# lthero-big/A-watermark-for-Diffusion-Models

Measured on AMD Instinct MI355X. Metric: watermarked images/sec (embed+extract, 512x512 SD2.1) + lossless bit-accuracy, higher is better.
Workload: dtype f16; 1 GPU; e2e: gsw_embed -> 50-step DDIM sampling (CFG 7.5, 2B-row UNet) -> 50-step DDIM inversion -> fused last step + 256-bit vote; SD2.1-base-shaped UNet (865.9 M params, synthetic weights; convolutions on the hand-written MFMA implicit GEMM), image stages per image: VAE decode -> uint8 -> ToTensor -> VAE encode (timed; synthetic VAE, inversion consumes the latent); batch_per_gpu=64, global_batch=64, message_bits=256, ddim_steps=50, parallelism=dp1 (images sharded, UNet replicated, no data-path collective)

## Files before the change

a-watermark-for-diffusion-models_amd/_native.py:

```python
from __future__ import annotations

import ctypes as C
import os

_HERE = os.path.dirname(os.path.abspath(__file__))
LIB_PATH = os.environ.get("GSWM_LIB", os.path.join(_HERE, "libgswm.so"))

GSW_F32, GSW_F16, GSW_BF16, GSW_F64 = 0, 1, 2, 3
GSW_OK, GSW_ERR_BAD_ARG, GSW_ERR_UNSUPPORTED, GSW_ERR_RAGGED, GSW_ERR_HIP, GSW_WARN_NO_RECORDS = 0, 1, 2, 3, 4, 5
GSW_EMBED_EXACT_F64, GSW_EMBED_FAST_F32 = 0, 1
GSW_MM_GN_ONLY = 1
GSW_FLAG_SATURATED, GSW_FLAG_NAN = 1, 2
GSW_MSG_INLINE_MAX = 256
GSW_IMG_U8_HWC, GSW_IMG_F16_CHW, GSW_IMG_F32_CHW = 0, 1, 2
GSW_PW_BRIGHTNESS, GSW_PW_CONTRAST, GSW_PW_INVERT, GSW_PW_GRAY, GSW_PW_HFLIP, GSW_PW_VFLIP, GSW_PW_NOISE = range(7)
GSW_RESAMPLE_LANCZOS, GSW_RESAMPLE_BILINEAR = 1, 2
GSW_TRACE_SOFT, GSW_TRACE_HARD = 0, 1

_u8p = C.POINTER(C.c_uint8)


class GswMmExtras(C.Structure):
    _fields_ = [("colstats_dev", C.c_void_p), ("colstats_capacity", C.c_int64), ("rowstats_dev", C.c_void_p), ("rowstats_capacity", C.c_int64),
                ("workspace_dev", C.c_void_p), ("workspace_bytes", C.c_int64), ("max_splits", C.c_int),
                ("colstats_rows_per_block", C.c_int), ("colstats_blocks", C.c_int), ("rowstats_slots", C.c_int), ("splits", C.c_int), ("flags", C.c_int)]


_PROTOTYPES = {
    "gsw_version": (C.c_int, []),
    "gsw_build_flags": (C.c_int, []),
    "gsw_strerror": (C.c_char_p, [C.c_int]),
    "gsw_last_hip_error": (C.c_int, []),
    "gsw_keystream": (C.c_int, [C.c_char_p, C.c_char_p, C.c_void_p, C.c_size_t, C.c_void_p]),
    "gsw_embed": (C.c_int, [C.c_char_p, C.c_char_p, C.c_char_p, C.c_int, C.c_void_p, C.c_uint64, C.c_uint64, C.c_void_p,
                            C.c_int, C.c_int, C.c_int64, C.c_uint32, C.c_void_p]),
    "gsw_philox_uniform": (C.c_int, [C.c_uint64, C.c_uint64, C.c_void_p, C.c_int, C.c_int64, C.c_void_p]),
    "gsw_extract": (C.c_int, [C.c_void_p, C.c_int, C.c_char_p, C.c_char_p, C.c_int, C.c_void_p, C.c_void_p, C.c_void_p,
                              C.c_int, C.c_int64, C.c_void_p]),
    "gsw_bit_matches": (C.c_int, [C.c_void_p, C.c_int, C.c_char_p, C.c_int, C.c_void_p, C.c_int, C.c_void_p]),
    "gsw_ddim_step": (C.c_int, [C.c_void_p, C.c_void_p, C.c_void_p, C.c_float, C.c_float, C.c_int, C.c_int64, C.c_void_p]),
    "gsw_ddim_step_cfg": (C.c_int, [C.c_void_p, C.c_void_p, C.c_void_p, C.c_void_p, C.c_float, C.c_float, C.c_float,
                                    C.c_int, C.c_int64, C.c_void_p]),
    "gsw_dpm_step": (C.c_int, [C.c_void_p, C.c_void_p, C.c_void_p, C.c_void_p, C.c_void_p, C.c_void_p, C.c_float, C.c_float, C.c_float,
                               C.c_float, C.c_float, C.c_float, C.c_int, C.c_int64, C.c_void_p]),
    "gsw_ddim_step_extract": (C.c_int, [C.c_void_p, C.c_void_p, C.c_void_p, C.c_float, C.c_float, C.c_int, C.c_char_p,
                                        C.c_char_p, C.c_int, C.c_void_p, C.c_void_p, C.c_void_p, C.c_int, C.c_int64,
                                        C.c_void_p]),
    "gsw_groupnorm_silu": (C.c_int, [C.c_void_p, C.c_void_p, C.c_void_p, C.c_void_p, C.c_void_p, C.c_int, C.c_int, C.c_int, C.c_int,
                                     C.c_float, C.c_int, C.c_int, C.c_void_p]),
    "gsw_geglu": (C.c_int, [C.c_void_p, C.c_void_p, C.c_int64, C.c_int, C.c_int, C.c_void_p]),
    "gsw_conv_pf": (C.c_int, [C.c_void_p, C.c_void_p, C.c_void_p, C.c_void_p, C.c_int, C.c_void_p, C.c_void_p, C.c_int, C.c_int, C.c_int, C.c_int,
                              C.c_int, C.c_int, C.c_int, C.c_int, C.c_int, C.c_void_p]),
    "gsw_groupnorm_pf": (C.c_int, [C.c_void_p, C.c_void_p, C.c_void_p, C.c_void_p, C.c_void_p, C.c_int, C.c_int, C.c_int, C.c_int, C.c_int,
                                   C.c_float, C.c_int, C.c_int, C.c_int, C.c_void_p]),
    "gsw_add_layernorm": (C.c_int, [C.c_void_p, C.c_void_p, C.c_void_p, C.c_void_p, C.c_void_p, C.c_void_p, C.c_int64, C.c_int, C.c_float,
                                    C.c_int, C.c_void_p]),
    "gsw_groupnorm_pf2": (C.c_int, [C.c_void_p, C.c_void_p, C.c_int, C.c_void_p, C.c_void_p, C.c_void_p, C.c_void_p, C.c_int, C.c_int, C.c_int,
                                    C.c_int, C.c_int, C.c_float, C.c_int, C.c_int, C.c_int, C.c_void_p]),
    "gsw_conv3x3_res_pf": (C.c_int, [C.c_void_p, C.c_void_p, C.c_void_p, C.c_void_p, C.c_int, C.c_void_p, C.c_void_p, C.c_int, C.c_int, C.c_int, C.c_int,
                                     C.c_int, C.c_void_p, C.c_int, C.c_void_p, C.c_int, C.c_int, C.c_void_p]),
    "gsw_conv_up2x_pf": (C.c_int, [C.c_void_p, C.c_void_p, C.c_void_p, C.c_void_p, C.c_int, C.c_int, C.c_int, C.c_int, C.c_int, C.c_int, C.c_void_p]),
    "gsw_attention": (C.c_int, [C.c_void_p, C.c_void_p, C.c_void_p, C.c_void_p, C.c_int, C.c_int, C.c_int, C.c_int, C.c_int, C.c_int, C.c_int, C.c_int,
                                C.c_int, C.c_float, C.c_int, C.c_void_p]),
    "gsw_attention_ws": (C.c_int, [C.c_void_p, C.c_void_p, C.c_void_p, C.c_void_p, C.c_int, C.c_int, C.c_int, C.c_int, C.c_int, C.c_int, C.c_int, C.c_int,
                                   C.c_int, C.c_float, C.c_int, C.c_void_p, C.c_int64, C.c_void_p]),
    "gsw_xattn_fused": (C.c_int, [C.c_void_p, C.c_void_p, C.c_void_p, C.c_int64, C.c_void_p, C.c_int64, C.c_void_p, C.c_void_p, C.c_void_p, C.c_float, C.c_int, C.c_int,
                                  C.c_int, C.c_int, C.c_int, C.c_int, C.c_void_p]),
    "gsw_xattn_fused_pre": (C.c_int, [C.c_void_p, C.c_void_p, C.c_void_p, C.c_float, C.c_void_p, C.c_int64, C.c_void_p, C.c_int64, C.c_void_p, C.c_void_p, C.c_void_p,
                                      C.c_float, C.c_int, C.c_int, C.c_int, C.c_int, C.c_int, C.c_int, C.c_void_p]),
    "gsw_gn_colstats_pairs": (C.c_int, [C.c_void_p, C.c_int, C.c_int, C.c_int, C.c_void_p, C.c_int, C.c_int, C.c_int, C.c_int, C.c_void_p]),
    "gsw_gn_proj_tokens": (C.c_int, [C.c_void_p, C.c_void_p, C.c_void_p, C.c_void_p, C.c_float, C.c_int, C.c_void_p, C.c_void_p, C.c_void_p, C.c_float, C.c_int, C.c_int,
                                     C.c_int, C.c_int, C.c_int, C.c_void_p]),
    "gsw_mt19937_seed": (None, [C.c_uint32, C.c_void_p]),
    "gsw_mt19937_uniform": (C.c_int, [C.c_void_p, C.c_int, C.c_void_p, C.c_int64, C.c_void_p, C.c_void_p]),
    "gsw_lanczos_plan": (C.c_int, [C.c_int, C.c_int, C.c_void_p, C.c_void_p, C.c_int]),
    "gsw_resize_lanczos": (C.c_int, [C.c_void_p, C.c_int, C.c_int, C.c_int, C.c_void_p, C.c_int, C.c_int, C.c_int, C.c_void_p, C.c_void_p, C.c_void_p,
                                     C.c_int, C.c_void_p, C.c_void_p, C.c_int, C.c_void_p]),
    "gsw_tensor_to_image": (C.c_int, [C.c_void_p, C.c_int, C.c_int, C.c_int, C.c_int, C.c_int, C.c_void_p, C.c_void_p]),
    "gsw_jpeg_quant_tables": (C.c_int, [C.c_int, C.c_void_p, C.c_void_p]),
    "gsw_jpeg_workspace_bytes": (C.c_size_t, [C.c_int, C.c_int, C.c_int]),
    "gsw_jpeg_roundtrip": (C.c_int, [C.c_void_p, C.c_int, C.c_int, C.c_int, C.c_int, C.c_void_p, C.c_int, C.c_void_p, C.c_void_p]),
    "gsw_gaussian_blur_params": (C.c_int, [C.c_float, C.c_int, C.c_void_p, C.c_void_p, C.c_void_p]),
    "gsw_gaussian_blur": (C.c_int, [C.c_void_p, C.c_int, C.c_int, C.c_int, C.c_float, C.c_void_p, C.c_void_p, C.c_void_p]),
    "gsw_image_pointwise": (C.c_int, [C.c_void_p, C.c_int, C.c_int, C.c_int, C.c_int, C.c_float, C.c_uint64, C.c_uint64, C.c_void_p, C.c_int,
                                      C.c_void_p, C.c_void_p]),
    "gsw_resample_plan": (C.c_int, [C.c_int, C.c_int, C.c_int, C.c_void_p, C.c_void_p, C.c_int]),
    "gsw_affine_nearest": (C.c_int, [C.c_void_p, C.c_int, C.c_int, C.c_int, C.c_void_p, C.c_void_p, C.c_int, C.c_void_p]),
    "gsw_box_mask": (C.c_int, [C.c_void_p, C.c_int, C.c_int, C.c_int, C.c_void_p, C.c_int, C.c_void_p, C.c_int, C.c_void_p]),
    "gsw_crop_resize": (C.c_int, [C.c_void_p, C.c_int, C.c_int, C.c_int, C.c_void_p, C.c_int, C.c_int, C.c_void_p, C.c_int, C.c_int, C.c_int,
                                  C.c_void_p, C.c_void_p, C.c_void_p, C.c_int, C.c_void_p, C.c_void_p, C.c_int, C.c_void_p]),
    "gsw_gemm": (C.c_int, [C.c_void_p, C.c_void_p, C.c_void_p, C.c_void_p, C.c_void_p, C.c_int64, C.c_int, C.c_int, C.c_int, C.c_int, C.c_int,
                           C.c_int, C.c_void_p]),
    "gsw_gemm_qkv": (C.c_int, [C.c_void_p, C.c_void_p, C.c_void_p, C.c_void_p, C.c_void_p, C.c_int64, C.c_int, C.c_int, C.c_int, C.c_int, C.c_int, C.c_void_p]),
    "gsw_ln_rowstats_finish": (C.c_int, [C.c_void_p, C.c_int, C.c_int64, C.c_int, C.c_float, C.c_void_p, C.c_void_p]),
    "gsw_gemm_ln": (C.c_int, [C.c_void_p, C.c_void_p, C.c_void_p, C.c_void_p, C.c_void_p, C.c_void_p, C.c_int64, C.c_int, C.c_int, C.c_int, C.c_int, C.c_int, C.c_void_p]),
    "gsw_gemm_strided": (C.c_int, [C.c_void_p, C.c_int64, C.c_void_p, C.c_int64, C.c_void_p, C.c_void_p, C.c_int64, C.c_void_p, C.c_int64, C.c_int64,
                                   C.c_int, C.c_int, C.c_int, C.c_int, C.c_int, C.c_int, C.c_void_p]),
    "gsw_softmax_rows": (C.c_int, [C.c_void_p, C.c_int64, C.c_int, C.c_int64, C.c_float, C.c_int, C.c_void_p]),
    "gsw_mm_config": (C.c_int, [C.c_int, C.c_int]),
    "gsw_mm_get_config": (C.c_int, [C.POINTER(C.c_int), C.POINTER(C.c_int)]),
    "gsw_groupnorm_pf_cs": (C.c_int, [C.c_void_p, C.c_void_p, C.c_int, C.c_void_p, C.c_int, C.c_int, C.c_int, C.c_void_p, C.c_int, C.c_int, C.c_int,
                                      C.c_void_p, C.c_void_p, C.c_void_p, C.c_void_p, C.c_int, C.c_int, C.c_int, C.c_int, C.c_int, C.c_float, C.c_int, C.c_int,
                                      C.c_int, C.c_void_p]),
    "gsw_groupnorm_pf_fused": (C.c_int, [C.c_void_p, C.c_void_p, C.c_int, C.c_void_p, C.c_void_p, C.c_void_p, C.c_int, C.c_int, C.c_int, C.c_int, C.c_int, C.c_float,
                                         C.c_int, C.c_int, C.c_int, C.c_void_p]),
    "gsw_gather_rows": (C.c_int, [C.c_void_p, C.c_int64, C.c_int64, C.c_void_p, C.c_int, C.c_void_p, C.c_int64, C.c_int, C.c_int64, C.c_void_p]),
    "gsw_nchw_to_pf": (C.c_int, [C.c_void_p, C.c_void_p, C.c_int, C.c_int, C.c_int, C.c_int, C.c_int, C.c_int, C.c_void_p]),
    "gsw_conv3x3_pf_nchw": (C.c_int, [C.c_void_p, C.c_void_p, C.c_void_p, C.c_void_p, C.c_int, C.c_int, C.c_int, C.c_int, C.c_int, C.c_int, C.c_void_p]),
    "gsw_gemm_small_config": (C.c_int, [C.c_int64, C.c_int, C.c_int, C.c_int]),
    "gsw_gemm_small": (C.c_int, [C.c_void_p, C.c_int64, C.c_void_p, C.c_int64, C.c_void_p, C.c_void_p, C.c_int64, C.c_void_p, C.c_int64, C.c_int64, C.c_int, C.c_int,
                                 C.c_int, C.c_int, C.c_int, C.c_void_p, C.c_int, C.c_float, C.c_void_p, C.c_void_p, C.c_void_p, C.c_int64, C.POINTER(C.c_int), C.c_int,
                                 C.c_int, C.c_void_p]),
    "gsw_gemm_ex": (C.c_int, [C.c_void_p, C.c_int64, C.c_void_p, C.c_int64, C.c_void_p, C.c_void_p, C.c_int64, C.c_void_p, C.c_int64, C.c_int64, C.c_int, C.c_int,
                              C.c_int, C.c_int, C.c_int, C.c_int, C.c_void_p, C.c_void_p]),
    "gsw_gemm2_ex": (C.c_int, [C.c_void_p, C.c_int64, C.c_int, C.c_void_p, C.c_int64, C.c_int, C.c_void_p, C.c_int64, C.c_void_p, C.c_void_p, C.c_int64, C.c_void_p,
                               C.c_int64, C.c_int64, C.c_int, C.c_int, C.c_int, C.c_int, C.c_int, C.c_void_p, C.c_void_p]),
    "gsw_gemm_ln_ex": (C.c_int, [C.c_void_p, C.c_void_p, C.c_void_p, C.c_void_p, C.c_void_p, C.c_void_p, C.c_int64, C.c_int, C.c_int, C.c_int, C.c_int, C.c_int,
                                 C.c_void_p, C.c_void_p]),
    "gsw_conv_pf_ex": (C.c_int, [C.c_void_p, C.c_void_p, C.c_void_p, C.c_void_p, C.c_int, C.c_void_p, C.c_void_p, C.c_int, C.c_int, C.c_int, C.c_int,
                                 C.c_int, C.c_int, C.c_int, C.c_int, C.c_int, C.c_void_p, C.c_void_p]),
    "gsw_conv3x3_res_pf_ex": (C.c_int, [C.c_void_p, C.c_void_p, C.c_void_p, C.c_void_p, C.c_int, C.c_void_p, C.c_void_p, C.c_int, C.c_int, C.c_int, C.c_int,
                                        C.c_int, C.c_void_p, C.c_int, C.c_void_p, C.c_int, C.c_int, C.c_void_p, C.c_void_p]),
    "gsw_conv_up2x_pf_ex": (C.c_int, [C.c_void_p, C.c_void_p, C.c_void_p, C.c_void_p, C.c_int, C.c_int, C.c_int, C.c_int, C.c_int, C.c_int, C.c_void_p, C.c_void_p]),
    "gsw_trace_workspace_bytes": (C.c_size_t, [C.c_int, C.c_int64, C.c_int]),
    "gsw_trace_topk": (C.c_int, [C.c_void_p, C.c_int, C.c_int, C.c_int, C.c_int, C.c_void_p, C.c_int64, C.c_int, C.c_void_p, C.c_void_p, C.c_void_p, C.c_void_p]),
    "gsw_sign_pack": (C.c_int, [C.c_void_p, C.c_int, C.c_void_p, C.c_void_p, C.c_int, C.c_int64, C.c_void_p]),
    "gsw_trace_keyed_workspace_bytes": (C.c_size_t, [C.c_int, C.c_int64, C.c_int]),
    "gsw_trace_keyed_topk": (C.c_int, [C.c_void_p, C.c_int, C.c_int64, C.c_void_p, C.c_int64, C.c_int, C.c_int64, C.c_int, C.c_void_p, C.c_void_p, C.c_void_p, C.c_void_p]),
    "gsw_embed_l": (C.c_int, [C.c_char_p, C.c_char_p, C.c_char_p, C.c_int, C.c_void_p, C.c_uint64, C.c_uint64, C.c_void_p,
                              C.c_int, C.c_int, C.c_int64, C.c_uint32, C.c_int, C.c_void_p]),
    "gsw_extract_l": (C.c_int, [C.c_void_p, C.c_int, C.c_char_p, C.c_char_p, C.c_int, C.c_void_p, C.c_void_p, C.c_void_p,
                                C.c_int, C.c_int64, C.c_int, C.c_void_p]),
    "gsw_quant_pack": (C.c_int, [C.c_void_p, C.c_int, C.c_void_p, C.c_void_p, C.c_int, C.c_int64, C.c_int, C.c_void_p]),
    "gsw_tile_agree": (C.c_int, [C.c_void_p, C.c_int, C.c_int, C.c_int, C.c_int, C.c_int, C.c_int, C.c_void_p, C.c_void_p, C.c_int, C.c_void_p, C.c_void_p]),
    "gsw_vote_tiled": (C.c_int, [C.c_void_p, C.c_int, C.c_int, C.c_int, C.c_int, C.c_int, C.c_int, C.c_void_p, C.c_void_p, C.c_int, C.c_void_p, C.c_void_p,
                                 C.c_void_p, C.c_void_p]),
    "gsw_embed_keyed": (C.c_int, [C.c_void_p, C.c_int64, C.c_int, C.c_void_p, C.c_uint64, C.c_uint64, C.c_void_p, C.c_int, C.c_int, C.c_int64,
                                  C.c_uint32, C.c_int, C.c_void_p]),
    "gsw_extract_keyed": (C.c_int, [C.c_void_p, C.c_int, C.c_void_p, C.c_int64, C.c_int, C.c_void_p, C.c_void_p, C.c_void_p, C.c_void_p,
                                    C.c_int, C.c_int64, C.c_int, C.c_void_p]),
    "gsw_extract_soft": (C.c_int, [C.c_void_p, C.c_int, C.c_void_p, C.c_int64, C.c_int, C.c_void_p, C.c_int64, C.c_int, C.c_void_p, C.c_void_p,
                                   C.c_void_p, C.c_void_p, C.c_void_p, C.c_void_p, C.c_int, C.c_int64, C.c_void_p]),
    "gsw_level_pack": (C.c_int, [C.c_void_p, C.c_int, C.c_void_p, C.c_int64, C.c_int, C.c_void_p, C.c_void_p, C.c_void_p, C.c_void_p, C.c_void_p,
                                 C.c_int, C.c_int64, C.c_void_p]),
    "gsw_trace_keyed_soft_topk": (C.c_int, [C.c_void_p, C.c_void_p, C.c_void_p, C.c_int, C.c_int, C.c_int64, C.c_void_p, C.c_int64, C.c_int, C.c_int64,
                                            C.c_int, C.c_void_p, C.c_void_p, C.c_void_p, C.c_void_p]),
    "gsw_key_search_workspace_bytes": (C.c_size_t, [C.c_int, C.c_int64, C.c_int]),
    "gsw_key_search_topk": (C.c_int, [C.c_void_p, C.c_int, C.c_int64, C.c_void_p, C.c_int64, C.c_int, C.c_int64, C.c_int, C.c_void_p, C.c_void_p, C.c_void_p, C.c_void_p]),
    "gsw_rows_align": (C.c_int, [C.c_void_p, C.c_int, C.c_int, C.c_int, C.c_int, C.c_int, C.c_void_p, C.c_int, C.c_void_p, C.c_void_p]),
    "gsw_key_search_soft_workspace_bytes": (C.c_size_t, [C.c_int, C.c_int64, C.c_int]),
    "gsw_key_search_soft_topk": (C.c_int, [C.c_void_p, C.c_void_p, C.c_int, C.c_int, C.c_int64, C.c_void_p, C.c_int64, C.c_int, C.c_int64, C.c_int,
                                           C.c_void_p, C.c_void_p, C.c_void_p, C.c_void_p]),
}

_lib = None


class GswError(RuntimeError):
    def __init__(self, status: int, what: str):
        super().__init__(f"libgswm: {what} (status {status})")
        self.status = status


def lib() -> C.CDLL:
    global _lib
    if _lib is None:
        if not os.path.exists(LIB_PATH):
            raise ImportError(
                f"{LIB_PATH} is missing: the HIP library has not been built. Run __graft_entry__.build() "
                "(hipcc --offload-arch=gfx950). There is no CPU fallback for the watermark hot path.")
        l = C.CDLL(LIB_PATH)
        for name, (res, args) in _PROTOTYPES.items():
            fn = getattr(l, name)
            fn.restype = res
            fn.argtypes = args
        flags = l.gsw_build_flags()
        if flags != 0 and os.environ.get("GSWM_LIB") is None:
            raise ImportError(f"{LIB_PATH} was compiled with measurement switches (gsw_build_flags() = {flags:#x}): not a production build; rebuild it "
                              "(__graft_entry__.build()) or select the side build explicitly with GSWM_LIB")
        _lib = l
    return _lib


def exported_symbols():
    return sorted(_PROTOTYPES)


def check(status: int):
    if status == GSW_OK:
        return
    what = lib().gsw_strerror(status).decode()
    if status == GSW_ERR_RAGGED:
        raise IndexError("string index out of range")
    if status == GSW_ERR_BAD_ARG:
        raise ValueError(f"libgswm: {what}")
    if status == GSW_ERR_HIP:
        what += f" (hipError_t {lib().gsw_last_hip_error()})"
    raise GswError(status, what)
```

a-watermark-for-diffusion-models_amd/csrc/gswm_attn.hip:

```cpp
#include <hip/hip_runtime.h>

#include <algorithm>
#include <cstdint>
#include <cstdlib>

#include "../../include/gswm.h"

extern __attribute__((visibility("hidden"))) thread_local int g_last_hip_error;

namespace {

typedef _Float16 f16x8 __attribute__((ext_vector_type(8)));
typedef _Float16 f16x4 __attribute__((ext_vector_type(4)));
typedef _Float16 f16x2 __attribute__((ext_vector_type(2)));
typedef __bf16 bf16x8 __attribute__((ext_vector_type(8)));
typedef __bf16 bf16x4 __attribute__((ext_vector_type(4)));
typedef float f32x16 __attribute__((ext_vector_type(16)));
typedef float f32x4 __attribute__((ext_vector_type(4)));
typedef float f32x2 __attribute__((ext_vector_type(2)));

__device__ __forceinline__ float xhalf_max(float v) {
    const uint32_t u = __float_as_uint(v);
    const auto r = __builtin_amdgcn_permlane32_swap(u, u, false, false);
    return fmaxf(__uint_as_float(r[0]), __uint_as_float(r[1]));
}
__device__ __forceinline__ void rows16_split(float x, float& lo16, float& hi16) {
    const uint32_t u = __float_as_uint(x);
    const auto r = __builtin_amdgcn_permlane16_swap(u, u, false, false);
    lo16 = __uint_as_float(r[0]);
    hi16 = __uint_as_float(r[1]);
}
__device__ __forceinline__ float xhalf_sum(float v) {
    const uint32_t u = __float_as_uint(v);
    const auto r = __builtin_amdgcn_permlane32_swap(u, u, false, false);
    return __uint_as_float(r[0]) + __uint_as_float(r[1]);
}

template <typename T> struct AT;
template <> struct AT<_Float16> {
    using v8 = f16x8;
    using v4 = f16x4;
    static __device__ __forceinline__ f32x16 mfma(v8 a, v8 b, f32x16 c) { return __builtin_amdgcn_mfma_f32_32x32x16_f16(a, b, c, 0, 0, 0); }
    static __device__ __forceinline__ f32x4 mfma16(v8 a, v8 b, f32x4 c) { return __builtin_amdgcn_mfma_f32_16x16x32_f16(a, b, c, 0, 0, 0); }
    static __device__ __forceinline__ f32x4 mfma4(v4 a, v4 b, f32x4 c) { return __builtin_amdgcn_mfma_f32_4x4x4f16(a, b, c, 0, 0, 0); }
};
template <> struct AT<__bf16> {
    using v8 = bf16x8;
    using v4 = bf16x4;
    static __device__ __forceinline__ f32x16 mfma(v8 a, v8 b, f32x16 c) { return __builtin_amdgcn_mfma_f32_32x32x16_bf16(a, b, c, 0, 0, 0); }
    static __device__ __forceinline__ f32x4 mfma16(v8 a, v8 b, f32x4 c) { return __builtin_amdgcn_mfma_f32_16x16x32_bf16(a, b, c, 0, 0, 0); }
    static __device__ __forceinline__ f32x4 mfma4(v4 a, v4 b, f32x4 c) {
        typedef short s16x4 __attribute__((ext_vector_type(4)));
        return __builtin_amdgcn_mfma_f32_4x4x4bf16_1k(__builtin_bit_cast(s16x4, a), __builtin_bit_cast(s16x4, b), c, 0, 0, 0);
    }
};

struct AttnArgs {
    const void* q;
    const void* k;
    const void* vt;
    void* o;
    int32_t H, Sq, Sk, ldq, ldk, ldo;
    int32_t Sk_valid;
    float scale_log2;
    uint32_t nqt;
    uint32_t total;
    uint32_t ksplit;
    float* part;
};

constexpr uint32_t VP = 144;

template <typename T, int QB, int DU, bool PAIR, bool RAGGED, bool KVS = false, bool DMA = false>
__global__ __launch_bounds__(256, (DU > 10 ? 1 : 2)) void gsw_attn_fwd_kernel(AttnArgs p) {
    using v8 = typename AT<T>::v8;
    using v4 = typename AT<T>::v4;
    constexpr int D = DU * 8, KC = (DU + 1) / 2, DBF = D / 32, TR = D % 32;
    constexpr bool TAIL = TR != 0;
    static_assert(TR == 0 || TR == 8 || TR == 16, "head_dim % 32 must be 0, 8 or 16");
    constexpr int DB = DBF > 0 ? DBF : 1, VROWS = DBF * 32 + (TAIL ? 16 : 0), NACC = DBF * 16 + (TAIL ? 8 : 0);
    constexpr uint32_t KP = KC * 32 + 16;
    constexpr uint32_t STAGE = 64 * KP + VROWS * VP;
    constexpr int NU = (64 * DU + 255) / 256;
    constexpr uint32_t NSTG = PAIR ? 4 : 2;
    constexpr bool LM = TR == 8 && !KVS;
    constexpr bool L4 = !LM;
    static_assert(!KVS || (QB == 1 && !RAGGED && !PAIR), "key-split form: 32 queries per wave, whole tiles, the plain two-stage loop");
    static_assert(!DMA || (DU == 8 && PAIR && !RAGGED && !KVS), "DMA staging: head_dim 64, four stages, whole tiles");
    extern __shared__ __attribute__((aligned(16))) uint8_t lds[];
    const uint32_t tid = threadIdx.x, wave = tid >> 6, lane = tid & 63u, h = lane >> 5, c32 = lane & 31u;
    constexpr uint32_t QW = 32u * QB, QWG = 4u * QW;

    uint32_t logical = blockIdx.x;
    const uint32_t total_wg = KVS ? p.total * p.ksplit : p.total;
    if ((total_wg & 7u) == 0) logical = (blockIdx.x & 7u) * (total_wg >> 3) + (blockIdx.x >> 3);
    uint32_t ks = 0;
    if constexpr (KVS) { const uint32_t lq = logical / p.ksplit; ks = logical - lq * p.ksplit; logical = lq; }
    const uint32_t bh = logical / p.nqt, qt = logical - bh * p.nqt;
    const uint32_t b = bh / (uint32_t)p.H, hh = bh - b * (uint32_t)p.H;

    const uint32_t q0 = qt * QWG + wave * QW + c32;
    const T* Qb = reinterpret_cast<const T*>(p.q) + (int64_t)b * p.Sq * p.ldq + hh * (uint32_t)D;
    const T* K = reinterpret_cast<const T*>(p.k) + (int64_t)b * p.Sk * p.ldk + hh * (uint32_t)D;
    const T* VT = reinterpret_cast<const T*>(p.vt) + ((int64_t)b * p.H + hh) * D * (int64_t)p.Sk;

    if (DU & 1 || D & 31) {
        for (uint32_t i = tid; i < NSTG * STAGE / 16; i += 256) reinterpret_cast<uint4*>(lds)[i] = make_uint4(0, 0, 0, 0);
        __syncthreads();
        if constexpr (LM) {
            const T one = (T)1.0f;
            if (tid < NSTG * 64u) *reinterpret_cast<T*>(lds + (tid >> 6) * STAGE + 64u * KP + (uint32_t)D * VP + (tid & 63u) * 2u) = one;
        }
        __syncthreads();
    }

    v8 qreg[QB][KC];
#pragma unroll
    for (int qb = 0; qb < QB; ++qb)
#pragma unroll
        for (int kc = 0; kc < KC; ++kc) {
            typedef uint32_t u32x4 __attribute__((ext_vector_type(4)));
            u32x4 w = u32x4{0u, 0u, 0u, 0u};
            const uint32_t qi = q0 + 32u * qb;
            const T* Q = Qb + (int64_t)((!RAGGED || qi < (uint32_t)p.Sq) ? qi : 0u) * p.ldq;
            if (2 * kc + 1 < DU || h == 0) w = *reinterpret_cast<const u32x4*>(Q + kc * 16 + h * 8);
#pragma unroll
            for (int j = 0; j < 4; ++j) { uint32_t e = w[j]; asm volatile("v_mov_b32 %0, %0" : "+v"(e)); w[j] = e; }
            qreg[qb][kc] = __builtin_bit_cast(v8, w);
        }

    constexpr bool ALLV = NU * 256 == 64 * DU;
#define GSW_ATTN_UNIT_DECL(i)                                                                           \
    uint4 kreg##i = make_uint4(0, 0, 0, 0), vreg##i = make_uint4(0, 0, 0, 0);                           \
    const uint32_t u##i = tid + 256u * i;                                                               \
    const bool uv##i = u##i < 64u * DU;                                                                 \
    const uint32_t uu##i = uv##i ? u##i : 0u;                                                           \
    const uint32_t kr##i = uu##i / (uint32_t)DU, kcol##i = uu##i - kr##i * (uint32_t)DU;                \
    const T* kg##i = K + (int64_t)kr##i * p.ldk + kcol##i * 8u;                                         \
    const uint32_t kst##i = kr##i * KP + kcol##i * 16u;                                                 \
    const T* vg##i = VT + (int64_t)(uu##i >> 3) * p.Sk + (uu##i & 7u) * 8u;                             \
    const uint32_t vst##i = 64u * KP + (uu##i >> 3) * VP + ((uu##i & 7u) >> 1) * 32u + (uu##i & 1u) * 8u;
    GSW_ATTN_UNIT_DECL(0)
    GSW_ATTN_UNIT_DECL(1)
    GSW_ATTN_UNIT_DECL(2)
    GSW_ATTN_UNIT_DECL(3)
    GSW_ATTN_UNIT_DECL(4)
#define GSW_ATTN_GLOAD1(i, key0)                                                                        \
    if (NU > i && (ALLV || uv##i)) {                                                                    \
        if (RAGGED) {                                                                                   \
            const int32_t row_ = min((int32_t)(key0) + (int32_t)kr##i, p.Sk - 1);                       \
            const int32_t col_ = (int32_t)(key0) + (int32_t)(uu##i & 7u) * 8;                           \
            kreg##i = *reinterpret_cast<const uint4*>(K + (int64_t)row_ * p.ldk + kcol##i * 8u);        \
            vreg##i = *reinterpret_cast<const uint4*>(VT + (int64_t)(uu##i >> 3) * p.Sk + (col_ + 8 <= p.Sk ? col_ : 0)); \
        } else {                                                                                        \
            kreg##i = *reinterpret_cast<const uint4*>(kg##i + (int64_t)(key0) * p.ldk);                 \
            vreg##i = *reinterpret_cast<const uint4*>(vg##i + (key0));                                  \
        }                                                                                               \
    }
#define GSW_ATTN_GLOAD(key0) GSW_ATTN_GLOAD1(0, key0) GSW_ATTN_GLOAD1(1, key0) GSW_ATTN_GLOAD1(2, key0) GSW_ATTN_GLOAD1(3, key0) GSW_ATTN_GLOAD1(4, key0)
#define GSW_ATTN_LSTORE1(i, st)                                                                         \
    if (NU > i && (ALLV || uv##i)) {                                                                    \
        uint8_t* base_ = lds + (st) * STAGE;                                                            \
        *reinterpret_cast<uint4*>(base_ + kst##i) = kreg##i;                                            \
        *reinterpret_cast<uint2*>(base_ + vst##i) = make_uint2(vreg##i.x, vreg##i.y);        \
        *reinterpret_cast<uint2*>(base_ + vst##i + 16u) = make_uint2(vreg##i.z, vreg##i.w);  \
    }
#define GSW_ATTN_LSTORE(st) GSW_ATTN_LSTORE1(0, st) GSW_ATTN_LSTORE1(1, st) GSW_ATTN_LSTORE1(2, st) GSW_ATTN_LSTORE1(3, st) GSW_ATTN_LSTORE1(4, st)
    static_assert(NU <= 5, "staging code covers up to 5 units per thread");

    f32x16 o[QB][DB];
    f32x4 ot[QB][2];
    float m_i[QB], l_i[QB];
    f32x4 l4[QB][2];
#pragma unroll
    for (int qb = 0; qb < QB; ++qb) {
        ot[qb][0] = f32x4{0.f, 0.f, 0.f, 0.f}; ot[qb][1] = f32x4{0.f, 0.f, 0.f, 0.f};
#pragma unroll
        for (int db = 0; db < DB; ++db)
#pragma unroll
            for (int i = 0; i < 16; ++i) o[qb][db][i] = 0.f;
        m_i[qb] = -INFINITY;
        l_i[qb] = 0.f;
        l4[qb][0] = f32x4{0.f, 0.f, 0.f, 0.f}; l4[qb][1] = f32x4{0.f, 0.f, 0.f, 0.f};
    }
    const float cs = p.scale_log2;

    const int32_t nt = (p.Sk + 63) >> 6;
    uint32_t swo[8];
#pragma unroll
    for (int k = 0; k < 8; ++k) swo[k] = DMA ? c32 * 128u + (((uint32_t)k ^ ((c32 >> 1) & 7u)) << 4) : 0u;
    auto tile = [&](const uint8_t* Kl, const uint8_t* Vl, int32_t t) __attribute__((always_inline)) {

        f32x16 s[QB][2];
#pragma unroll
        for (int qb = 0; qb < QB; ++qb)
#pragma unroll
            for (int i = 0; i < 16; ++i) { s[qb][0][i] = 0.f; s[qb][1][i] = 0.f; }
#pragma unroll
        for (int kc = 0; kc < KC; ++kc) {
#pragma unroll
            for (int kb = 0; kb < 2; ++kb) {
                const v8 a = DMA ? *reinterpret_cast<const v8*>(Kl + (uint32_t)(kb * 32 * 128) + (h ? swo[(2 * kc + 1) & 7] : swo[(2 * kc) & 7]))
                                 : *reinterpret_cast<const v8*>(Kl + (uint32_t)(kb * 32 + (int)c32) * KP + (uint32_t)kc * 32u + h * 16u);
#pragma unroll
                for (int qb = 0; qb < QB; ++qb) s[qb][kb] = AT<T>::mfma(a, qreg[qb][kc], s[qb][kb]);
            }
        }
        if ((t + 1) * 64 > p.Sk_valid) {
            asm volatile("; masked tile");
#pragma unroll
            for (int kb = 0; kb < 2; ++kb)
#pragma unroll
                for (int i = 0; i < 16; ++i) {
                    const int32_t key = DMA ? t * 64 + kb * 32 + (i >> 3) * 16 + (int32_t)h * 8 + ((i >> 2) & 1) * 4 + (i & 3)
                                            : t * 64 + kb * 32 + (i >> 2) * 8 + (int32_t)h * 4 + (i & 3);
                    if (key >= p.Sk_valid) {
#pragma unroll
                        for (int qb = 0; qb < QB; ++qb) s[qb][kb][i] = -INFINITY;
                    }
                }
        }

        v8 pb[QB][2][2];
#pragma unroll
        for (int qb = 0; qb < QB; ++qb) {
            float mx = s[qb][0][0];
#pragma unroll
            for (int i = 1; i < 16; ++i) mx = fmaxf(mx, s[qb][0][i]);
#pragma unroll
            for (int i = 0; i < 16; ++i) mx = fmaxf(mx, s[qb][1][i]);
            mx = xhalf_max(mx);
            const float m_new = fmaxf(m_i[qb], mx * cs);
            const float alpha = __builtin_amdgcn_exp2f(m_i[qb] - m_new);
            m_i[qb] = m_new;
#pragma unroll
            for (int kb = 0; kb < 2; ++kb) {
#pragma unroll
                for (int i = 0; i < 16; ++i) {
                    const float e = __builtin_amdgcn_exp2f(fmaf(s[qb][kb][i], cs, -m_new));
                    pb[qb][kb][i >> 3][i & 7] = (T)e;
                }
            }
            if (__any(alpha != 1.0f)) {
                if constexpr (L4) { l4[qb][0] *= alpha; l4[qb][1] *= alpha; }
#pragma unroll
                for (int db = 0; db < DBF; ++db)
#pragma unroll
                    for (int i = 0; i < 16; ++i) o[qb][db][i] *= alpha;
                if constexpr (TAIL) {
                    float a0, a1;
                    rows16_split(alpha, a0, a1);
                    ot[qb][0] *= a0; ot[qb][1] *= a1;
                }
            }
        }

        if constexpr (L4) {
            const v4 ones = v4{(T)1.0f, (T)1.0f, (T)1.0f, (T)1.0f};
#pragma unroll
            for (int kb = 0; kb < 2; ++kb)
#pragma unroll
                for (int tt = 0; tt < 2; ++tt)
#pragma unroll
                    for (int qb = 0; qb < QB; ++qb) {
                        const v8 pv = pb[qb][kb][tt];
                        l4[qb][0] = AT<T>::mfma4(ones, v4{pv[0], pv[1], pv[2], pv[3]}, l4[qb][0]);
                        l4[qb][1] = AT<T>::mfma4(ones, v4{pv[4], pv[5], pv[6], pv[7]}, l4[qb][1]);
                    }
        }
#pragma unroll
        for (int kb = 0; kb < 2; ++kb) {
#pragma unroll
            for (int tt = 0; tt < 2; ++tt) {
#pragma unroll
                for (int db = 0; db < DBF; ++db) {
                    const v8 a = DMA ? *reinterpret_cast<const v8*>(Vl + (uint32_t)(db * 32 * 128) + (h ? swo[(4 * kb + 2 * tt + 1) & 7] : swo[(4 * kb + 2 * tt) & 7]))
                                     : *reinterpret_cast<const v8*>(Vl + (uint32_t)(db * 32 + (int)c32) * VP + (uint32_t)(kb * 32 + tt * 16) * 2u + h * 16u);
#pragma unroll
                    for (int qb = 0; qb < QB; ++qb) o[qb][db] = AT<T>::mfma(a, pb[qb][kb][tt], o[qb][db]);
                }
            }
            if constexpr (TAIL) {
                const uint32_t r16 = lane >> 4, m16 = lane & 15u;
                const v8 a = *reinterpret_cast<const v8*>(Vl + (uint32_t)(DBF * 32 + (int)m16) * VP + (uint32_t)(kb * 32 + (int)((r16 & 1u) * 16u)) * 2u + (r16 >> 1) * 16u);
#pragma unroll
                for (int qb = 0; qb < QB; ++qb) {
                    typedef uint32_t u32x4 __attribute__((ext_vector_type(4)));
                    u32x4 b0 = __builtin_bit_cast(u32x4, pb[qb][kb][0]), b1 = __builtin_bit_cast(u32x4, pb[qb][kb][1]);
#pragma unroll
                    for (int w = 0; w < 4; ++w) {
                        const auto sw = __builtin_amdgcn_permlane16_swap(b0[w], b1[w], false, false);
                        b0[w] = sw[0]; b1[w] = sw[1];
                    }
                    ot[qb][0] = AT<T>::mfma16(a, __builtin_bit_cast(v8, b0), ot[qb][0]);
                    ot[qb][1] = AT<T>::mfma16(a, __builtin_bit_cast(v8, b1), ot[qb][1]);
                }
            }
        }
    };
    if constexpr (DMA) {
        __shared__ __attribute__((aligned(16))) uint8_t sg0[16384], sg1[16384], sg2[16384], sg3[16384];
        const T* kp[2];
        const T* vp[2];
#pragma unroll
        for (int j = 0; j < 2; ++j) {
            const uint32_t pc = wave + 4u * j, row = 8u * pc + (lane >> 3);
            const uint32_t chunk = (lane & 7u) ^ ((row >> 1) & 7u);
            const uint32_t key = 16u * (pc >> 1) + 8u * (lane >> 5) + 4u * (pc & 1u) + ((lane >> 3) & 3u);
            kp[j] = K + (int64_t)key * p.ldk + chunk * 8u;
            vp[j] = VT + (int64_t)row * p.Sk + chunk * 8u;
        }
        const uint32_t wv = __builtin_amdgcn_readfirstlane(wave);
        const int64_t kstep = (int64_t)64 * p.ldk;
        auto dma = [&](uint8_t* sg, int32_t t) __attribute__((always_inline)) {
#pragma unroll
            for (int j = 0; j < 2; ++j) {
                __builtin_amdgcn_global_load_lds((const __attribute__((address_space(1))) void*)(kp[j] + (int64_t)t * kstep),
                                                 (__attribute__((address_space(3))) void*)(sg + (wv + 4u * j) * 1024u), 16, 0, 0);
                __builtin_amdgcn_global_load_lds((const __attribute__((address_space(1))) void*)(vp[j] + (int64_t)t * 64),
                                                 (__attribute__((address_space(3))) void*)(sg + 8192u + (wv + 4u * j) * 1024u), 16, 0, 0);
            }
        };
        dma(sg0, 0);
        dma(sg1, 1);
        __builtin_amdgcn_s_waitcnt(0x0F70);
        __syncthreads();
        for (int32_t t = 0; t < nt; t += 4) {
            dma(sg2, t + 2);
            __builtin_amdgcn_sched_barrier(0);
            tile(sg0, sg0 + 8192, t);
            dma(sg3, t + 3);
            __builtin_amdgcn_sched_barrier(0);
            tile(sg1, sg1 + 8192, t + 1);
            __builtin_amdgcn_s_waitcnt(0x0F70);
            __syncthreads();
            const int32_t tn = t + 4 < nt ? t + 4 : t;
            dma(sg0, tn);
            __builtin_amdgcn_sched_barrier(0);
            tile(sg2, sg2 + 8192, t + 2);
            dma(sg1, tn + 1);
            __builtin_amdgcn_sched_barrier(0);
            tile(sg3, sg3 + 8192, t + 3);
            __builtin_amdgcn_s_waitcnt(0x0F70);
            __syncthreads();
        }
    } else if (PAIR) {
        GSW_ATTN_GLOAD(0)
        GSW_ATTN_LSTORE(0u)
        GSW_ATTN_GLOAD((nt > 1 ? 1 : 0) << 6)
        GSW_ATTN_LSTORE(1u)
        __syncthreads();
        for (int32_t t = 0; t < nt; t += 2) {
            GSW_ATTN_GLOAD((t + 2 < nt ? t + 2 : nt - 1) << 6)
            __builtin_amdgcn_sched_barrier(0);
            tile(lds + (uint32_t)(t & 3) * STAGE, lds + (uint32_t)(t & 3) * STAGE + 64u * KP, t);
            GSW_ATTN_LSTORE((uint32_t)((t + 2) & 3))
            if (t + 1 < nt) {
                GSW_ATTN_GLOAD((t + 3 < nt ? t + 3 : nt - 1) << 6)
                __builtin_amdgcn_sched_barrier(0);
                tile(lds + (uint32_t)((t + 1) & 3) * STAGE, lds + (uint32_t)((t + 1) & 3) * STAGE + 64u * KP, t + 1);
                GSW_ATTN_LSTORE((uint32_t)((t + 3) & 3))
            }
            __syncthreads();
        }
    } else {
        const int32_t t_lo = KVS ? (int32_t)(((int64_t)ks * nt) / (int32_t)p.ksplit) : 0;
        const int32_t t_hi = KVS ? (int32_t)(((int64_t)(ks + 1u) * nt) / (int32_t)p.ksplit) : nt;
        GSW_ATTN_GLOAD(t_lo << 6)
        GSW_ATTN_LSTORE(0u)
        __syncthreads();
        for (int32_t t = t_lo; t < t_hi; ++t) {
            const int32_t tn = t + 1 < t_hi ? t + 1 : t;
            GSW_ATTN_GLOAD(tn << 6)
            __builtin_amdgcn_sched_barrier(0);
            tile(lds + (uint32_t)((t - t_lo) & 1) * STAGE, lds + (uint32_t)((t - t_lo) & 1) * STAGE + 64u * KP, t);
            GSW_ATTN_LSTORE((uint32_t)((t - t_lo + 1) & 1))
            __syncthreads();
        }
    }

    if constexpr (KVS) {
        float* base = p.part + (((size_t)logical * p.ksplit + ks) * 4u + wave) * (size_t)((NACC + 2) * 64) + lane;
#pragma unroll
        for (int db = 0; db < DBF; ++db)
#pragma unroll
            for (int i = 0; i < 16; ++i) base[(db * 16 + i) * 64] = o[0][db][i];
        if constexpr (TAIL) {
#pragma unroll
            for (int i = 0; i < 8; ++i) base[(DBF * 16 + i) * 64] = ot[0][i >> 2][i & 3];
        }
        base[NACC * 64] = m_i[0];
        base[(NACC + 1) * 64] = l4[0][0][0] + l4[0][1][0];
        return;
    }

#pragma unroll
    for (int qb = 0; qb < QB; ++qb) {
        float l;
        if constexpr (LM) {
            const int idx = (int)(4u * (32u + (lane & 15u)));
            const float l0 = __int_as_float(__builtin_amdgcn_ds_bpermute(idx, __float_as_int(ot[qb][0][0])));
            const float l1 = __int_as_float(__builtin_amdgcn_ds_bpermute(idx, __float_as_int(ot[qb][1][0])));
            l = (c32 & 16u) ? l1 : l0;
            l_i[qb] = 0.5f * l;
        } else {
            if constexpr (L4) l_i[qb] = l4[qb][0][0] + l4[qb][1][0];
            l = xhalf_sum(l_i[qb]);
        }
        const float inv = 1.0f / l;
        const uint32_t qi = q0 + 32u * qb;
        if (RAGGED && qi >= (uint32_t)p.Sq) continue;
        T* O = reinterpret_cast<T*>(p.o) + ((int64_t)b * p.Sq + qi) * p.ldo + hh * (uint32_t)D;
#pragma unroll
        for (int db = 0; db < DBF; ++db) {
#pragma unroll
            for (int g = 0; g < 4; ++g) {
                const int d0 = db * 32 + g * 8 + (int)h * 4;
                v4 w;
#pragma unroll
                for (int j = 0; j < 4; ++j) w[j] = (T)(o[qb][db][g * 4 + j] * inv);
                *reinterpret_cast<v4*>(O + d0) = w;
            }
        }
    }
    if constexpr (TAIL) {
#pragma unroll
        for (int qb = 0; qb < QB; ++qb) {
            float inv2[2];
            rows16_split(1.0f / xhalf_sum(l_i[qb]), inv2[0], inv2[1]);
            const int d0 = DBF * 32 + (int)(lane >> 4) * 4;
#pragma unroll
            for (int hq = 0; hq < 2; ++hq) {
                const uint32_t qi = qt * QWG + wave * QW + 32u * qb + 16u * hq + (lane & 15u);
                if ((RAGGED && qi >= (uint32_t)p.Sq) || d0 >= D) continue;
                T* O = reinterpret_cast<T*>(p.o) + ((int64_t)b * p.Sq + qi) * p.ldo + hh * (uint32_t)D;
                v4 w;
#pragma unroll
                for (int j = 0; j < 4; ++j) w[j] = (T)(ot[qb][hq][j] * inv2[hq]);
                *reinterpret_cast<v4*>(O + d0) = w;
            }
        }
    }
#undef GSW_ATTN_GLOAD
#undef GSW_ATTN_LSTORE
#undef GSW_ATTN_GLOAD1
#undef GSW_ATTN_LSTORE1
#undef GSW_ATTN_UNIT_DECL
}

template <typename T, int DU>
__global__ __launch_bounds__(256) void gsw_attn_combine_kernel(AttnArgs p) {
    using v4 = typename AT<T>::v4;
    constexpr int D = DU * 8, DBF = D / 32, TR = D % 32, DB = DBF > 0 ? DBF : 1, NACC = DBF * 16 + (TR ? 8 : 0);
    constexpr bool TAIL = TR != 0;
    const uint32_t tid = threadIdx.x, wave = tid >> 6, lane = tid & 63u, h = lane >> 5, c32 = lane & 31u;
    const uint32_t logical = blockIdx.x;
    const uint32_t bh = logical / p.nqt, qt = logical - bh * p.nqt;
    const uint32_t b = bh / (uint32_t)p.H, hh = bh - b * (uint32_t)p.H;
    const uint32_t qi = qt * 128u + wave * 32u + c32;
    constexpr size_t REC = (size_t)(NACC + 2) * 64;
    const float* base = p.part + ((size_t)logical * p.ksplit * 4u + wave) * REC + lane;
    float m = -INFINITY;
    for (uint32_t s = 0; s < p.ksplit; ++s) m = fmaxf(m, base[(size_t)s * 4u * REC + NACC * 64]);
    f32x16 o[DB];
    f32x4 ot[2] = {f32x4{0.f, 0.f, 0.f, 0.f}, f32x4{0.f, 0.f, 0.f, 0.f}};
#pragma unroll
    for (int db = 0; db < DB; ++db)
#pragma unroll
        for (int i = 0; i < 16; ++i) o[db][i] = 0.f;
    float l = 0.f;
    for (uint32_t s = 0; s < p.ksplit; ++s) {
        const float* r = base + (size_t)s * 4u * REC;
        const float sc = __builtin_amdgcn_exp2f(r[NACC * 64] - m);
        l = fmaf(r[(NACC + 1) * 64], sc, l);
#pragma unroll
        for (int db = 0; db < DBF; ++db)
#pragma unroll
            for (int i = 0; i < 16; ++i) o[db][i] = fmaf(r[(db * 16 + i) * 64], sc, o[db][i]);
        if constexpr (TAIL) {
            float s2[2];
            rows16_split(sc, s2[0], s2[1]);
#pragma unroll
            for (int i = 0; i < 8; ++i) ot[i >> 2][i & 3] = fmaf(r[(DBF * 16 + i) * 64], s2[i >> 2], ot[i >> 2][i & 3]);
        }
    }
    const float inv = 1.0f / xhalf_sum(l);
    T* O = reinterpret_cast<T*>(p.o) + ((int64_t)b * p.Sq + qi) * p.ldo + hh * (uint32_t)D;
#pragma unroll
    for (int db = 0; db < DBF; ++db) {
#pragma unroll
        for (int g = 0; g < 4; ++g) {
            const int d0 = db * 32 + g * 8 + (int)h * 4;
            v4 w;
#pragma unroll
            for (int j = 0; j < 4; ++j) w[j] = (T)(o[db][g * 4 + j] * inv);
            *reinterpret_cast<v4*>(O + d0) = w;
        }
    }
    if constexpr (TAIL) {
        float inv2[2];
        rows16_split(inv, inv2[0], inv2[1]);
        const int d0 = DBF * 32 + (int)(lane >> 4) * 4;
#pragma unroll
        for (int hq = 0; hq < 2; ++hq) {
            const uint32_t qh = qt * 128u + wave * 32u + 16u * hq + (lane & 15u);
            if (d0 >= D) continue;
            T* Oh = reinterpret_cast<T*>(p.o) + ((int64_t)b * p.Sq + qh) * p.ldo + hh * (uint32_t)D;
            v4 w;
#pragma unroll
            for (int j = 0; j < 4; ++j) w[j] = (T)(ot[hq][j] * inv2[hq]);
            *reinterpret_cast<v4*>(Oh + d0) = w;
        }
    }
}

}

template <typename T, int QB, int DU>
static int launch_attn_cfg(const AttnArgs& a, uint32_t grid, bool ragged, float* ws, int64_t ws_bytes, hipStream_t st) {
    constexpr int KC = (DU + 1) / 2, DBF = DU * 8 / 32, TR = DU * 8 % 32, NACC = DBF * 16 + (TR ? 8 : 0);
    constexpr uint32_t stage = 64 * (KC * 32 + 16) + (DBF * 32 + (TR ? 16 : 0)) * VP;
    if constexpr (QB == 1 && (DU == 8 || DU == 5)) {
        static const int kvs_env = getenv("GSW_ATTN_KVS") ? atoi(getenv("GSW_ATTN_KVS")) : 1;
        const int32_t nt = a.Sk >> 6;
        if (!ragged && kvs_env && ws && a.Sk_valid == a.Sk && a.total <= 256u && nt >= (kvs_env > 1 ? 8 : 32)) {
            uint32_t ksplit = (uint32_t)std::min<int64_t>(std::min<int64_t>(512 / a.total, nt / 4), 8);
            if (kvs_env > 1) ksplit = (uint32_t)std::min<int>(kvs_env, nt);
            const int64_t need = (int64_t)a.total * ksplit * 4 * (NACC + 2) * 64 * (int64_t)sizeof(float);
            if (ksplit >= 2 && need <= ws_bytes) {
                AttnArgs k = a;
                k.ksplit = ksplit; k.part = ws;
                hipLaunchKernelGGL((gsw_attn_fwd_kernel<T, 1, DU, false, false, true>), dim3(a.total * ksplit), dim3(256), 2 * stage, st, k);
                hipLaunchKernelGGL((gsw_attn_combine_kernel<T, DU>), dim3(a.total), dim3(256), 0, st, k);
                return GSW_OK;
            }
        }
    }
    static const int pair_env = getenv("GSW_ATTN_PAIR") ? atoi(getenv("GSW_ATTN_PAIR")) : 1;
    const bool pair = !ragged && pair_env && 4 * stage <= 80 * 1024 && (a.Sk >> 6) >= 16;
    const uint32_t lds = (pair ? 4 : 2) * stage;
    const void* fn = pair ? (const void*)gsw_attn_fwd_kernel<T, QB, DU, true, false>
                          : (ragged ? (const void*)gsw_attn_fwd_kernel<T, 1, DU, false, true> : (const void*)gsw_attn_fwd_kernel<T, QB, DU, false, false>);
    if (lds > 64 * 1024) {
        hipError_t e = hipFuncSetAttribute(fn, hipFuncAttributeMaxDynamicSharedMemorySize, (int)lds);
        if (e != hipSuccess) { g_last_hip_error = (int)e; return GSW_ERR_HIP; }
    }
    if constexpr (DU == 8) {
        static const int dma_env = getenv("GSW_ATTN_DMA") ? atoi(getenv("GSW_ATTN_DMA")) : 1;
        if (pair && dma_env && ((a.Sk >> 6) & 3) == 0) {
            hipLaunchKernelGGL((gsw_attn_fwd_kernel<T, QB, DU, true, false, false, true>), dim3(grid), dim3(256), 0, st, a);
            return GSW_OK;
        }
    }
    if (pair) hipLaunchKernelGGL((gsw_attn_fwd_kernel<T, QB, DU, true, false>), dim3(grid), dim3(256), lds, st, a);
    else if (ragged) hipLaunchKernelGGL((gsw_attn_fwd_kernel<T, 1, DU, false, true>), dim3(grid), dim3(256), lds, st, a);
    else hipLaunchKernelGGL((gsw_attn_fwd_kernel<T, QB, DU, false, false>), dim3(grid), dim3(256), lds, st, a);
    return GSW_OK;
}

template <typename T>
static int launch_attn(const AttnArgs& a, int head_dim, int QB, uint32_t grid, bool ragged, float* ws, int64_t wsb, hipStream_t st) {
    if (head_dim == 64) return QB == 2 ? launch_attn_cfg<T, 2, 8>(a, grid, ragged, ws, wsb, st) : launch_attn_cfg<T, 1, 8>(a, grid, ragged, ws, wsb, st);
    if (head_dim == 40) return QB == 2 ? launch_attn_cfg<T, 2, 5>(a, grid, ragged, ws, wsb, st) : launch_attn_cfg<T, 1, 5>(a, grid, ragged, ws, wsb, st);
    if (head_dim == 80) return launch_attn_cfg<T, 1, 10>(a, grid, ragged, ws, wsb, st);
    return launch_attn_cfg<T, 1, 20>(a, grid, ragged, ws, wsb, st);
}

int gsw_attention(const void* q_dev, const void* k_dev, const void* vt_dev, void* out_dev, int B, int H, int head_dim, int Sq, int Sk, int Sk_valid,
                  int ldq, int ldk, int ldo, float scale, int dtype, void* stream) {
    return gsw_attention_ws(q_dev, k_dev, vt_dev, out_dev, B, H, head_dim, Sq, Sk, Sk_valid, ldq, ldk, ldo, scale, dtype, nullptr, 0, stream);
}

int gsw_attention_ws(const void* q_dev, const void* k_dev, const void* vt_dev, void* out_dev, int B, int H, int head_dim, int Sq, int Sk, int Sk_valid,
                     int ldq, int ldk, int ldo, float scale, int dtype, void* workspace_dev, int64_t workspace_bytes, void* stream) {
    if (workspace_bytes < 0 || (workspace_bytes > 0 && !workspace_dev) || ((uintptr_t)workspace_dev & 15)) return GSW_ERR_BAD_ARG;
    if (!q_dev || !k_dev || !vt_dev || !out_dev || B <= 0 || H <= 0 || Sq <= 0 || Sk <= 0 || Sk_valid <= 0 || Sk_valid > Sk) return GSW_ERR_BAD_ARG;
    if (dtype != GSW_F16 && dtype != GSW_BF16) return GSW_ERR_BAD_ARG;
    if (head_dim != 40 && head_dim != 64 && head_dim != 80 && head_dim != 160) return GSW_ERR_UNSUPPORTED;
    const int inner = H * head_dim;
    if ((Sk & 7) || ldq < inner || ldk < inner || ldo < inner || ((ldq | ldk | ldo) & 7)) return GSW_ERR_UNSUPPORTED;
    static const int qb_env = getenv("GSW_ATTN_QB") ? atoi(getenv("GSW_ATTN_QB")) : 2;
    const bool ragged = (Sq & 127) || (Sk & 63);
    const int64_t wg256 = (int64_t)(Sq / 256) * B * H;
    const int QB = ((Sq & 255) == 0 && Sq >= 512 && qb_env >= 2 && head_dim < 80 && !ragged && (wg256 > 400 || qb_env == 3)) ? 2 : 1;
    const int64_t total = (int64_t)((Sq + 128 * QB - 1) / (128 * QB)) * B * H;
    if (total > 0x7FFFFFFF) return GSW_ERR_UNSUPPORTED;
    AttnArgs a;
    a.q = q_dev; a.k = k_dev; a.vt = vt_dev; a.o = out_dev;
    a.H = H; a.Sq = Sq; a.Sk = Sk; a.ldq = ldq; a.ldk = ldk; a.ldo = ldo; a.Sk_valid = Sk_valid;
    a.scale_log2 = scale * 1.4426950408889634f;
    a.nqt = (uint32_t)((Sq + 128 * QB - 1) / (128 * QB));
    a.total = (uint32_t)total;
    a.ksplit = 1; a.part = nullptr;
    float* const ws = workspace_bytes > 0 ? (float*)workspace_dev : nullptr;
    const int rc = dtype == GSW_F16 ? launch_attn<_Float16>(a, head_dim, QB, (uint32_t)total, ragged, ws, workspace_bytes, (hipStream_t)stream)
                                    : launch_attn<__bf16>(a, head_dim, QB, (uint32_t)total, ragged, ws, workspace_bytes, (hipStream_t)stream);
    if (rc != GSW_OK) return rc;
    hipError_t e = hipGetLastError();
    if (e != hipSuccess) { g_last_hip_error = (int)e; return GSW_ERR_HIP; }
    return GSW_OK;
}

template <typename T>
__global__ __launch_bounds__(256) void gsw_softmax_rows_kernel(T* __restrict__ x, int64_t ld, int32_t cols, float scale_log2) {
    __shared__ float red[4];
    T* row = x + (int64_t)blockIdx.x * ld;
    const uint32_t tid = threadIdx.x, lane = tid & 63u, wave = tid >> 6;
    const int32_t nv = cols >> 3;
    auto load8 = [&](int32_t v, float (&f)[8]) {
        const uint4 u = reinterpret_cast<const uint4*>(row)[v];
        const uint32_t w[4] = {u.x, u.y, u.z, u.w};
#pragma unroll
        for (int k = 0; k < 4; ++k) {
            T lo, hi;
            const uint16_t a = (uint16_t)w[k], b = (uint16_t)(w[k] >> 16);
            __builtin_memcpy(&lo, &a, 2); __builtin_memcpy(&hi, &b, 2);
            f[2 * k] = (float)lo; f[2 * k + 1] = (float)hi;
        }
    };
    auto wg_reduce = [&](float v, bool is_max) -> float {
#pragma unroll
        for (int o = 32; o > 0; o >>= 1) { const float t = __shfl_xor(v, o); v = is_max ? fmaxf(v, t) : v + t; }
        __syncthreads();
        if (lane == 0) red[wave] = v;
        __syncthreads();
        const float a = red[0], b = red[1], c = red[2], d = red[3];
        return is_max ? fmaxf(fmaxf(a, b), fmaxf(c, d)) : (a + b) + (c + d);
    };
    float mx = -INFINITY;
    for (int32_t v = tid; v < nv; v += 256) {
        float f[8];
        load8(v, f);
#pragma unroll
        for (int k = 0; k < 8; ++k) mx = fmaxf(mx, f[k]);
    }
    mx = wg_reduce(mx, true) * scale_log2;
    float sum = 0.f;
    for (int32_t v = tid; v < nv; v += 256) {
        float f[8];
        load8(v, f);
#pragma unroll
        for (int k = 0; k < 8; ++k) sum += __builtin_amdgcn_exp2f(fmaf(f[k], scale_log2, -mx));
    }
    const float inv = 1.0f / wg_reduce(sum, false);
    for (int32_t v = tid; v < nv; v += 256) {
        float f[8];
        load8(v, f);
        uint32_t w[4];
#pragma unroll
        for (int k = 0; k < 4; ++k) {
            const T lo = (T)(__builtin_amdgcn_exp2f(fmaf(f[2 * k], scale_log2, -mx)) * inv), hi = (T)(__builtin_amdgcn_exp2f(fmaf(f[2 * k + 1], scale_log2, -mx)) * inv);
            uint16_t a, b;
            __builtin_memcpy(&a, &lo, 2); __builtin_memcpy(&b, &hi, 2);
            w[k] = (uint32_t)a | ((uint32_t)b << 16);
        }
        reinterpret_cast<uint4*>(row)[v] = make_uint4(w[0], w[1], w[2], w[3]);
    }
}

int gsw_softmax_rows(void* x_dev, int64_t rows, int cols, int64_t ld, float scale, int dtype, void* stream) {
    if (!x_dev || rows < 0 || cols <= 0 || ld < cols) return GSW_ERR_BAD_ARG;
    if (dtype != GSW_F16 && dtype != GSW_BF16) return GSW_ERR_BAD_ARG;
    if ((cols & 7) || (ld & 7) || rows > 0x7FFFFFFF) return GSW_ERR_UNSUPPORTED;
    if (rows == 0) return GSW_OK;
    const float sl2 = scale * 1.4426950408889634f;
    if (dtype == GSW_F16) hipLaunchKernelGGL(gsw_softmax_rows_kernel<_Float16>, dim3((uint32_t)rows), dim3(256), 0, (hipStream_t)stream, (_Float16*)x_dev, ld, cols, sl2);
    else hipLaunchKernelGGL(gsw_softmax_rows_kernel<__bf16>, dim3((uint32_t)rows), dim3(256), 0, (hipStream_t)stream, (__bf16*)x_dev, ld, cols, sl2);
    hipError_t e = hipGetLastError();
    if (e != hipSuccess) { g_last_hip_error = (int)e; return GSW_ERR_HIP; }
    return GSW_OK;
}
```

a-watermark-for-diffusion-models_amd/graph.py:

```python
from __future__ import annotations

import os
import warnings
from collections import OrderedDict
from typing import Dict, Optional, Tuple

import torch


def _env_mode() -> str:
    return os.environ.get("GSW_GRAPH", "auto").lower()


AUTO_MAX_ROWS = 32
CHECK_EVERY = 32
_WEIGHTS_EPOCH = [0]


def weights_changed() -> None:
    _WEIGHTS_EPOCH[0] += 1

MAX_ENTRIES = 8


def _switches():
    from . import pf, unet as U, xattn as X, _native as N
    import ctypes as C
    tr, sm = C.c_int(0), C.c_int(0)
    N.lib().gsw_mm_get_config(C.byref(tr), C.byref(sm))
    return (U.FUSED_KERNELS, U.USE_PF, U.UPSAMPLE_SUBPIXEL, U.CACHE_CONTEXT_KV, U.FUSED_QK, U.FUSED_QKV, U.OWN_ATTENTION, U.OWN_GEMM, U.TEMB_TABLE,
            U.CONV_OUT_DIRECT_MAX_PIXELS, U.CFG_SHARED_PREFIX, pf.FUSE_GN_STATS, pf.GN_FUSED_MAX_WGS, pf.GN_FUSED_MAX_PIXELS, pf.FOLD_LN, pf.FOLD_LN_MIN_ROWS, pf.SPLITK_MAX,
            pf.SPLITK_BYTES, pf.SMALL_GEMM_MAX_ROWS, pf.ATTN_KEY_SPLIT, U.FOLD_FF_OUT, X.ENABLED, X.PRE_ENABLED, X.GNPROJ_ENABLED,
            tr.value, sm.value)


class _Entry:
    __slots__ = ("graph", "x_s", "t_s", "ctx_s", "out", "ctx_id", "replays", "ws")


def _ctx_identity(ctx: torch.Tensor):
    base = ctx._base if ctx._base is not None else ctx
    return (base, ctx._version, ctx.storage_offset(), tuple(ctx.shape), tuple(ctx.stride()))


def _same_ctx(a, b) -> bool:
    return a[0] is b[0] and a[1:] == b[1:]


class GraphedEpsModel:

    def __init__(self, model, mode: Optional[str] = None, max_rows: int = AUTO_MAX_ROWS, clone_output: bool = True):
        self.model = model
        m = (mode or _env_mode()).lower()
        self.mode = {"1": "always", "0": "never", "on": "always", "off": "never"}.get(m, m)
        if self.mode not in ("auto", "always", "never"):
            raise ValueError(f"GSW_GRAPH / mode must be auto | always | never (got {m!r})")
        self.max_rows = max_rows
        self.clone_output = clone_output
        self.capture_fallbacks: Dict[str, int] = {}
        self._entries: "OrderedDict[Tuple, _Entry]" = OrderedDict()
        self._weights_key = None
        self._epoch = _WEIGHTS_EPOCH[0]
        if hasattr(model, "register_load_state_dict_post_hook"):
            model.register_load_state_dict_post_hook(lambda _m, _keys: weights_changed())
        self._failed: Dict[Tuple, str] = {}
        self.stats = {"captures": 0, "replays": 0, "eager": 0, "context_refreshes": 0}

    def __getattr__(self, name):
        return getattr(self.__dict__["model"], name)

    def _wants_graph(self, x: torch.Tensor) -> bool:
        if self.mode == "never" or not x.is_cuda:
            return False
        if torch.cuda.is_current_stream_capturing():
            return False
        return self.mode == "always" or x.shape[0] <= self.max_rows

    def _params_key(self):
        return tuple((p.data_ptr(), p._version) for p in self.model.parameters())

    def reset(self):
        self._entries.clear()
        self._failed.clear()

    def _capture(self, key, x, t, ctx, kw) -> Optional[_Entry]:
        e = _Entry()
        e.x_s = torch.empty_like(x, memory_format=torch.contiguous_format).copy_(x)
        e.t_s = torch.empty_like(t).copy_(t)
        e.ctx_s = torch.empty(ctx.shape, dtype=ctx.dtype, device=ctx.device).copy_(ctx)
        e.ctx_id, e.replays = _ctx_identity(ctx), 0
        from . import pf
        e.ws = torch.empty(pf.SPLITK_BYTES, dtype=torch.uint8, device=x.device)
        from . import unet as U
        fb_before = dict(U.FALLBACKS)
        try:
            side = torch.cuda.Stream(device=x.device)
            side.wait_stream(torch.cuda.current_stream(x.device))
            with torch.cuda.stream(side), torch.no_grad(), pf.splitk_workspace(e.ws):
                self.model(e.x_s, e.t_s, e.ctx_s, **kw)
                self.model(e.x_s, e.t_s, e.ctx_s, **kw)
            torch.cuda.current_stream(x.device).wait_stream(side)
            g = torch.cuda.CUDAGraph()
            with torch.no_grad(), pf.splitk_workspace(e.ws), torch.cuda.graph(g):
                e.out = self.model(e.x_s, e.t_s, e.ctx_s, **kw)
            e.graph = g
            for k_, v_ in U.FALLBACKS.items():
                if v_ != fb_before.get(k_, 0):
                    self.capture_fallbacks[k_] = self.capture_fallbacks.get(k_, 0) + 1
        except Exception as exc:
            self._failed[key] = f"{type(exc).__name__}: {exc}"
            warnings.warn(f"gswm graph: capture of the eps model for {key} failed ({self._failed[key]}); running it eagerly", RuntimeWarning, stacklevel=3)
            return None
        self.stats["captures"] += 1
        return e

    @torch.no_grad()
    def __call__(self, x: torch.Tensor, t: torch.Tensor, ctx: torch.Tensor, cfg_dup: bool = False) -> torch.Tensor:
        kw = {"cfg_dup": True} if cfg_dup else {}
        if not self._wants_graph(ctx if cfg_dup else x):
            self.stats["eager"] += 1
            return self.model(x, t, ctx, **kw)
        if not torch.is_tensor(t):
            t = torch.as_tensor(t, device=x.device)
        key = (tuple(x.shape), x.dtype, str(x.device), tuple(t.shape), t.dtype, tuple(ctx.shape), ctx.dtype, bool(cfg_dup), _switches())
        if key in self._failed:
            self.stats["eager"] += 1
            return self.model(x, t, ctx, **kw)
        e = self._entries.get(key)
        cid = _ctx_identity(ctx)
        if e is None or not _same_ctx(cid, e.ctx_id) or e.replays % CHECK_EVERY == 0 or self._epoch != _WEIGHTS_EPOCH[0]:
            self._epoch = _WEIGHTS_EPOCH[0]
            wk = self._params_key()
            if wk != self._weights_key:
                self._entries.clear()
                self._weights_key = wk
                e = None
        if e is None:
            e = self._capture(key, x, t, ctx, kw)
            if e is None:
                self.stats["eager"] += 1
                return self.model(x, t, ctx, **kw)
            self._entries[key] = e
            while len(self._entries) > MAX_ENTRIES:
                self._entries.popitem(last=False)
        elif not _same_ctx(cid, e.ctx_id):
            e.ctx_s.copy_(ctx)
            e.ctx_id = cid
            self.model.prepare_context(e.ctx_s)
            self.stats["context_refreshes"] += 1
        e.x_s.copy_(x)
        e.t_s.copy_(t)
        e.graph.replay()
        e.replays += 1
        self.stats["replays"] += 1
        self._entries.move_to_end(key)
        return e.out.clone() if self.clone_output else e.out


def graphed(model, mode: Optional[str] = None, clone_output: bool = True):
    return model if isinstance(model, GraphedEpsModel) else GraphedEpsModel(model, mode, clone_output=clone_output)
```

a-watermark-for-diffusion-models_amd/pf.py:

```python
from __future__ import annotations

import ctypes as _C
import os
from typing import Optional

import torch

from . import _native as N
from .codec import _dt, _stream_ptr


class PF:
    __slots__ = ("buf", "B", "H", "W", "C", "stats", "border_valid")

    def __init__(self, buf: torch.Tensor, B: int, H: int, W: int, C: int):
        self.buf, self.B, self.H, self.W, self.C = buf, B, H, W, C
        self.stats: Optional["ColStats"] = None
        self.border_valid = True

    @property
    def G(self) -> int:
        return self.W + 3

    @property
    def M(self) -> int:
        return self.B * (self.H + 2) * (self.W + 2)

    @property
    def rows(self) -> torch.Tensor:
        return self.buf[self.G:self.G + self.M]

    @property
    def grid(self) -> torch.Tensor:
        return self.rows.view(self.B, self.H + 2, self.W + 2, self.C)

    @property
    def interior(self) -> torch.Tensor:
        return self.grid[:, 1:-1, 1:-1, :]

    @staticmethod
    def empty(B, H, W, C, dtype, device) -> "PF":
        G = W + 3
        M = B * (H + 2) * (W + 2)
        return PF(torch.empty((M + 2 * G, C), dtype=dtype, device=device), B, H, W, C)

    @staticmethod
    def zeros(B, H, W, C, dtype, device) -> "PF":
        G = W + 3
        return PF(torch.zeros((B * (H + 2) * (W + 2) + 2 * G, C), dtype=dtype, device=device), B, H, W, C)

    @staticmethod
    def from_nchw(x: torch.Tensor) -> "PF":
        B, C, H, W = x.shape
        p = PF.zeros(B, H, W, C, x.dtype, x.device)
        p.interior.copy_(x.permute(0, 2, 3, 1))
        return p

    def to_nchw(self) -> torch.Tensor:
        return self.interior.permute(0, 3, 1, 2).contiguous()

    def tokens(self) -> torch.Tensor:
        return self.interior.reshape(self.B, self.H * self.W, self.C)


SPLITK_BYTES = 40 << 20
GN_ONLY_SKIPS_BORDER = True
ATTN_KEY_SPLIT = True
LAUNCH_LOG = None
SPLITK_MAX = 0
_WS = {}
_WS_OVERRIDE: Optional[torch.Tensor] = None


def _workspace(device) -> torch.Tensor:
    ov = _WS_OVERRIDE
    if ov is not None:
        return ov
    dev = torch.device(device)
    key = (dev.index, torch.cuda.current_stream(dev).cuda_stream)
    ws = _WS.get(key)
    if ws is None:
        ws = _WS[key] = torch.empty(SPLITK_BYTES, dtype=torch.uint8, device=dev)
    return ws


def _extras(device, colstats: Optional[torch.Tensor] = None, rowstats: Optional[torch.Tensor] = None) -> "N.GswMmExtras":
    ws = _workspace(device)
    ex = N.GswMmExtras()
    if colstats is not None:
        ex.colstats_dev, ex.colstats_capacity = colstats.data_ptr(), colstats.numel()
    if rowstats is not None:
        ex.rowstats_dev, ex.rowstats_capacity = rowstats.data_ptr(), rowstats.numel()
    ex.workspace_dev, ex.workspace_bytes, ex.max_splits = ws.data_ptr(), ws.numel(), int(SPLITK_MAX)
    if LAUNCH_LOG is not None:
        LAUNCH_LOG.append(ex)
    return ex


class splitk_workspace:

    def __init__(self, buf: Optional[torch.Tensor]):
        self.buf = buf

    def __enter__(self):
        global _WS_OVERRIDE
        self.prev, _WS_OVERRIDE = _WS_OVERRIDE, self.buf
        return self

    def __exit__(self, *exc):
        global _WS_OVERRIDE
        _WS_OVERRIDE = self.prev
        return False



FUSE_GN_STATS = True


class ColStats:
    __slots__ = ("buf", "rows", "npar", "blocks")

    def __init__(self, buf: torch.Tensor, rows: int, npar: int, blocks: int):
        self.buf, self.rows, self.npar, self.blocks = buf, rows, npar, blocks


def _colstats_arm(M: int, Nn: int, device, npar: int = 1, geom=None):
    if not FUSE_GN_STATS or (geom is not None and _gn_fused_ok(geom[0], geom[1], geom[2], Nn, 32)):
        return None
    cap_blocks = (M + 127) // 128 * 4
    buf = torch.empty(npar * cap_blocks * Nn, dtype=torch.float32, device=device)
    return buf, cap_blocks


def _colstats_collect(armed, ex, npar: int = 1) -> Optional[ColStats]:
    if armed is None or ex.colstats_rows_per_block <= 0:
        return None
    return ColStats(armed[0], int(ex.colstats_rows_per_block), npar, armed[1])


def _stats_usable(x: "PF") -> bool:
    st = x.stats
    if st is None:
        return False
    pix = x.H * x.W if st.npar == 1 else (x.H // 2) * (x.W // 2)
    return pix % st.rows == 0 and (st.npar == 1 or (x.H % 2 == 0 and x.W % 2 == 0))


def cached(owner, name: str, params, build):
    key = tuple((q.data_ptr(), q._version, str(q.device), q.dtype) for q in params)
    c = getattr(owner, name, None)
    if c is None or c[0] != key:
        c = (key, build())
        setattr(owner, name, c)
    return c[1]


class ConvTimer:

    def __init__(self, by_shape: bool = False):
        self.ev = []
        self.by_shape = by_shape

    def start(self):
        e = torch.cuda.Event(enable_timing=True)
        e.record()
        return e

    def stop(self, e0, kernel: str, flops: float, launches: int = 1, nbytes: float = 0.0):
        e1 = torch.cuda.Event(enable_timing=True)
        e1.record()
        self.ev.append((kernel, flops, e0, e1, launches, nbytes))

    def summary(self):
        out = {}
        for k, f, a, b, nl, nb in self.ev:
            d = out.setdefault(k, {"calls": 0, "flops": 0.0, "ms": 0.0, "bytes": 0.0})
            d["calls"] += nl
            d["flops"] += f
            d["bytes"] += nb
            d["ms"] += a.elapsed_time(b)
        for d in out.values():
            d["avg_us"] = d["ms"] * 1e3 / d["calls"]
            d["flops_per_launch"] = d["flops"] / d["calls"]
            d["bytes_per_launch"] = d["bytes"] / d["calls"]
            d["tflops"] = d["flops"] / (d["ms"] * 1e-3) / 1e12 if d["ms"] else 0.0
        return out


CONV_TIMER: Optional[ConvTimer] = None


def _conv_kernel_name(W: int, n_out: int, ksize: int, stride: int) -> str:
    if n_out % 8 == 0 and n_out >= 128 and (stride == 1 or ksize == 3):
        return ("gsw_mm_kernel(conv3x3)" if stride == 1 else "gsw_mm_kernel(conv3x3 s2)") if ksize == 3 else "gsw_mm_kernel(conv1x1)"
    return "gsw_conv_gemm_kernel"


def pack_conv_weight(w: torch.Tensor) -> torch.Tensor:
    return w.permute(0, 2, 3, 1).reshape(w.shape[0], -1).contiguous()


def conv_pf(x: PF, w_packed: torch.Tensor, bias: Optional[torch.Tensor], *, ksize: int = 3, stride: int = 1,
            rowbias: Optional[torch.Tensor] = None, resid: Optional[PF] = None, cin: Optional[int] = None, cin_offset: int = 0,
            pad_after_only: bool = False, gn_only: bool = False) -> PF:
    C = x.C if cin is None else cin
    Nn = w_packed.shape[0]
    Ho, Wo = x.H // stride, x.W // stride
    _same(w_packed, x.buf, "conv weight", Nn * ksize * ksize * C)
    _same(bias, x.buf, "conv bias", Nn)
    ldrb = _rowbias_ld(rowbias, x.buf, x.B, Nn)
    if resid is not None:
        _same(resid.buf, x.buf, "resid")
        if (resid.B, resid.H, resid.W, resid.C) != (x.B, Ho, Wo, Nn):
            raise ValueError("resid geometry does not match the convolution output")
    y = PF.empty(x.B, Ho, Wo, Nn, x.buf.dtype, x.buf.device)
    xp = x.rows.data_ptr() + cin_offset * x.buf.element_size()
    if pad_after_only:
        assert stride == 2 and ksize == 3
        xp += (x.W + 2 + 1) * x.C * x.buf.element_size()
    tm = CONV_TIMER
    with torch.cuda.device(x.buf.device):
        e0 = tm.start() if tm is not None else None
        armed = _colstats_arm(x.B * Ho * Wo, Nn, x.buf.device, geom=(x.B, Ho, Wo)) if Nn >= 128 else None
        ex = _extras(x.buf.device, colstats=None if armed is None else armed[0])
        if gn_only and GN_ONLY_SKIPS_BORDER:
            ex.flags = N.GSW_MM_GN_ONLY
        N.check(N.lib().gsw_conv_pf_ex(xp, w_packed.data_ptr(), bias.data_ptr() if bias is not None else None,
                                       rowbias.data_ptr() if rowbias is not None else None, ldrb,
                                       resid.rows.data_ptr() if resid is not None else None, y.rows.data_ptr(),
                                       x.B, Ho, Wo, C, Nn, ksize, stride, x.C, _dt(x.buf.dtype), _C.byref(ex), _stream_ptr()))
        y.stats = _colstats_collect(armed, ex)
        y.border_valid = not (ex.flags & N.GSW_MM_GN_ONLY and ex.colstats_rows_per_block > 0)
        if tm is not None:
            name = _conv_kernel_name(Wo, Nn, ksize, stride)
            tm.stop(e0, (name, x.B, Ho, Wo, ksize * ksize * C, Nn, stride) if tm.by_shape else name, 2.0 * x.B * Ho * Wo * Nn * ksize * ksize * C,
                    nbytes=2.0 * (x.B * x.H * x.W * C + Nn * ksize * ksize * C + x.B * Ho * Wo * Nn * (2 if resid is not None else 1)))
    return y


def _rowbias_ld(rb: Optional[torch.Tensor], like: torch.Tensor, B: int, Nn: int) -> int:
    if rb is None:
        return 0
    if not rb.is_cuda or rb.device != like.device or rb.dtype != like.dtype:
        raise ValueError(f"rowbias must be a {like.dtype} tensor on {like.device}")
    if tuple(rb.shape) != (B, Nn) or rb.stride(1) != 1 or rb.data_ptr() % 16 or (B > 1 and (rb.stride(0) % 8 or rb.stride(0) < Nn)):
        raise ValueError(f"rowbias must be [{B}, {Nn}] with contiguous, 16-byte aligned rows a multiple of 8 elements apart")
    return rb.stride(0) if B > 1 else Nn


def _rows2d(t: torch.Tensor, like: torch.Tensor, name: str):
    if t.dim() != 2 or not t.is_cuda or t.device != like.device or t.dtype != like.dtype:
        raise ValueError(f"{name} must be a 2-D {like.dtype} tensor on {like.device}")
    if t.stride(1) != 1 or t.stride(0) % 8 or t.stride(0) < t.shape[1] or t.data_ptr() % 16:
        raise ValueError(f"{name}: rows must be contiguous, 16-byte aligned and a multiple of 8 elements apart")
    return t.stride(0)


def gemm_strided(x: torch.Tensor, w: torch.Tensor, out: torch.Tensor, bias: Optional[torch.Tensor] = None) -> torch.Tensor:
    if x.dtype not in (torch.float16, torch.bfloat16):
        raise ValueError(f"gemm_strided: fp16 / bf16 only (got {x.dtype})")
    ldx, ldw, ldy = _rows2d(x, x, "x"), _rows2d(w, x, "w"), _rows2d(out, x, "out")
    M, K = x.shape
    Nn = w.shape[0]
    if w.shape[1] != K or tuple(out.shape) != (M, Nn):
        raise ValueError("gemm_strided: shapes do not chain")
    _same(bias, x, "bias", Nn)
    tm = CONV_TIMER
    with torch.cuda.device(x.device):
        e0 = tm.start() if tm is not None else None
        ex = _extras(x.device)
        N.check(N.lib().gsw_gemm_ex(x.data_ptr(), ldx, w.data_ptr(), ldw, bias.data_ptr() if bias is not None else None, None, ldy,
                                    out.data_ptr(), ldy, M, K, Nn, 0, 0, 0, _dt(x.dtype), _C.byref(ex), _stream_ptr()))
        if tm is not None:
            tm.stop(e0, ("gsw_mm_kernel", M, K, Nn, "plain") if tm.by_shape else "gsw_mm_kernel", 2.0 * M * K * Nn, nbytes=2.0 * (M * K + Nn * K + M * Nn))
    return out


def softmax_rows_(x: torch.Tensor, scale: float) -> torch.Tensor:
    ld = _rows2d(x, x, "x")
    with torch.cuda.device(x.device):
        N.check(N.lib().gsw_softmax_rows(x.data_ptr(), x.shape[0], x.shape[1], ld, float(scale), _dt(x.dtype), _stream_ptr()))
    return x


def attention_single_head(q: torch.Tensor, k: torch.Tensor, vt: torch.Tensor) -> torch.Tensor:
    B, S, d = q.shape
    if k.shape != (B, S, d) or vt.shape != (B, d, S) or d % 64 or S % 8:
        raise ValueError("attention_single_head: q, k [B, S, d], vt [B, d, S], d % 64 == 0, S % 8 == 0")
    Sp = (S + 63) // 64 * 64
    out = torch.empty((B, S, d), dtype=q.dtype, device=q.device)
    scores = torch.empty((S, Sp), dtype=q.dtype, device=q.device)
    if Sp != S:
        scores[:, S:].zero_()
        vt = torch.cat([vt, vt.new_zeros(B, d, Sp - S)], dim=2)
    for b in range(B):
        gemm_strided(q[b], k[b], scores[:, :S])
        softmax_rows_(scores[:, :S], d ** -0.5)
        gemm_strided(scores, vt[b], out[b])
    return out


_GN_WS = {}


def _gn_workspace(device, B, groups, C=0):
    k = (str(device), max(B * 64 * groups * 2, B * C * 2))
    if k not in _GN_WS:
        _GN_WS[k] = torch.empty(k[1], dtype=torch.float32, device=device)
    return _GN_WS[k]


GN_FUSED_MAX_WGS = int(os.environ.get("GSW_GN_FUSED_MAX_WGS", "512"))
GN_FUSED_MAX_PIXELS = int(os.environ.get("GSW_GN_FUSED_MAX_PIXELS", "1024"))


def _gn_fused_ok(B: int, H: int, W: int, C: int, groups: int) -> bool:
    if B * groups > GN_FUSED_MAX_WGS or H * W > GN_FUSED_MAX_PIXELS or C % groups or (C // groups) % 2 or C % 8:
        return False
    npair = C // groups // 2
    if npair * W > 1024 or B * (H + 2) * (W + 2) * C >= 1 << 31:
        return False
    rl = min(1024 // (npair * W), H)
    while H % rl:
        rl -= 1
    return (H + rl - 1) // rl <= 32


def _groupnorm_fused(x: PF, x2: Optional[PF], gamma, beta, groups, eps, act, tokens):
    dev = x.buf.device
    C = x.C + (x2.C if x2 is not None else 0)
    if tokens:
        res = torch.empty((x.B, x.H * x.W, C), dtype=x.buf.dtype, device=dev)
        optr = res.data_ptr()
    else:
        res = PF.empty(x.B, x.H, x.W, C, x.buf.dtype, dev)
        optr = res.rows.data_ptr()
    with torch.cuda.device(dev):
        N.check(N.lib().gsw_groupnorm_pf_fused(x.rows.data_ptr(), x2.rows.data_ptr() if x2 is not None else None, x.C if x2 is not None else 0,
                                               gamma.data_ptr(), beta.data_ptr(), optr, x.B, x.H, x.W, C, groups, eps, 1 if act else 0,
                                               1 if tokens else 0, _dt(x.buf.dtype), _stream_ptr()))
    return res


def _ensure_border(x: PF) -> None:
    if not x.border_valid:
        g = x.grid
        g[:, 0].zero_(); g[:, -1].zero_(); g[:, :, 0].zero_(); g[:, :, -1].zero_()
        x.border_valid = True


def groupnorm_pf(x: PF, gamma: torch.Tensor, beta: torch.Tensor, groups: int, eps: float, *, act: bool = True, tokens: bool = False):
    dev = x.buf.device
    _same(gamma, x.buf, "gamma", x.C)
    _same(beta, x.buf, "beta", x.C)
    if _gn_fused_ok(x.B, x.H, x.W, x.C, groups):
        _ensure_border(x)
        return _groupnorm_fused(x, None, gamma, beta, groups, eps, act, tokens)
    ws = _gn_workspace(dev, x.B, groups, x.C)
    if tokens:
        out = torch.empty((x.B, x.H * x.W, x.C), dtype=x.buf.dtype, device=dev)
        optr, res = out.data_ptr(), out
    else:
        y = PF.empty(x.B, x.H, x.W, x.C, x.buf.dtype, dev)
        optr, res = y.rows.data_ptr(), y
    if FUSE_GN_STATS and _stats_usable(x) and x.C <= 4096 and (x.C // groups) % 2 == 0:
        st = x.stats
        with torch.cuda.device(dev):
            N.check(N.lib().gsw_groupnorm_pf_cs(x.rows.data_ptr(), None, 0, st.buf.data_ptr(), st.rows, st.npar, st.blocks, None, 0, 0, 0,
                                                gamma.data_ptr(), beta.data_ptr(), optr, ws.data_ptr(), x.B, x.H, x.W, x.C, groups, eps,
                                                1 if act else 0, 1 if tokens else 0, _dt(x.buf.dtype), _stream_ptr()))
        return res
    _ensure_border(x)
    with torch.cuda.device(dev):
        N.check(N.lib().gsw_groupnorm_pf(x.rows.data_ptr(), gamma.data_ptr(), beta.data_ptr(), optr, ws.data_ptr(), x.B, x.H, x.W, x.C, groups,
                                         eps, 1 if act else 0, 1 if tokens else 0, _dt(x.buf.dtype), _stream_ptr()))
    return res


def gn_pf(x: PF, norm, act: bool = True, tokens: bool = False):
    return groupnorm_pf(x, norm.weight, norm.bias, norm.num_groups, norm.eps, act=act, tokens=tokens)


def pack_geglu_weight(w: torch.Tensor, b: Optional[torch.Tensor]):
    I = w.shape[0] // 2
    v = w[:I].reshape(I // 8, 8, -1)
    g = w[I:].reshape(I // 8, 8, -1)
    wp = torch.cat([v, g], dim=1).reshape(2 * I, -1).contiguous()
    bp = None
    if b is not None:
        bp = torch.cat([b[:I].reshape(I // 8, 8), b[I:].reshape(I // 8, 8)], dim=1).reshape(2 * I).contiguous()
    return wp, bp


def linear(x: torch.Tensor, w: torch.Tensor, bias: Optional[torch.Tensor], *, resid: Optional[torch.Tensor] = None, geglu: bool = False) -> torch.Tensor:
    return gemm(x, w, bias, resid=resid, mode="geglu" if geglu else "plain")


GEMM_MODES = {"plain": 0, "geglu": 1, "trans": 2, "tok2pf": 3}
SMALL_GEMM_MAX_ROWS = int(os.environ.get("GSW_SMALL_GEMM_MAX_ROWS", "128"))
SMALL_GEMM_MAX_K = 2560


def _same(t: Optional[torch.Tensor], like: torch.Tensor, name: str, numel: Optional[int] = None):
    if t is None:
        return
    if not t.is_cuda or t.device != like.device:
        raise RuntimeError(f"{name} must live on {like.device} (got {t.device}); there is no CPU fallback")
    if t.dtype != like.dtype:
        raise ValueError(f"{name} must be {like.dtype} like the activations (got {t.dtype})")
    if not t.is_contiguous() or t.data_ptr() % 16:
        raise ValueError(f"{name} must be contiguous and 16-byte aligned")
    if numel is not None and t.numel() != numel:
        raise ValueError(f"{name} has {t.numel()} elements, expected {numel}")


def gemm(x: torch.Tensor, w: torch.Tensor, bias: Optional[torch.Tensor] = None, *, resid: Optional[torch.Tensor] = None, mode: str = "plain",
         tokens: int = 0, width: int = 0, out: Optional[torch.Tensor] = None, stats_for: Optional["PF"] = None,
         rowstats: bool = False) -> torch.Tensor:
    if x.dtype not in (torch.float16, torch.bfloat16):
        raise ValueError(f"gemm: fp16 / bf16 only (got {x.dtype})")
    _same(x, x, "x")
    K = x.shape[-1]
    M = x.numel() // K
    Nn = w.shape[0]
    _same(w, x, "w", Nn * K)
    _same(bias, x, "bias", Nn)
    m = GEMM_MODES[mode]
    if mode == "plain":
        _same(resid, x, "resid", M * Nn)
        y = torch.empty((*x.shape[:-1], Nn), dtype=x.dtype, device=x.device) if out is None else out
        _same(y, x, "out", M * Nn)
    elif mode == "geglu":
        if resid is not None:
            raise ValueError("gemm: geglu takes no residual")
        y = torch.empty((*x.shape[:-1], Nn // 2), dtype=x.dtype, device=x.device) if out is None else out
        _same(y, x, "out", M * Nn // 2)
    elif mode == "trans":
        if resid is not None or tokens <= 0 or M % tokens:
            raise ValueError("gemm: trans needs tokens = rows per image and no residual")
        y = torch.empty((M // tokens, Nn, tokens), dtype=x.dtype, device=x.device) if out is None else out
        _same(y, x, "out", M * Nn)
    else:
        if out is None or tokens <= 0 or width <= 0 or tokens % width or M % tokens:
            raise ValueError("gemm: tok2pf needs out (PF rows), tokens = H*W and width = W")
        y = out
        rows = (M // tokens) * (tokens // width + 2) * (width + 2)
        _same(y, x, "out", rows * Nn)
        _same(resid, x, "resid", rows * Nn)
    tm = CONV_TIMER
    if (SMALL_GEMM_MAX_ROWS and M <= SMALL_GEMM_MAX_ROWS and mode in ("plain", "trans", "tok2pf") and K <= SMALL_GEMM_MAX_K and M % 16 == 0 and Nn % 16 == 0
            and K % 32 == 0 and K >= 128 and (mode != "trans" or tokens % 4 == 0)):
        rs_buf = torch.empty(M * ((Nn + 31) // 32) * 2, dtype=torch.float32, device=x.device) if (rowstats and mode == "plain" and FOLD_LN and M >= FOLD_LN_MIN_ROWS and M % 8 == 0) else None
        slots = _C.c_int(0)
        with torch.cuda.device(x.device):
            e0 = tm.start() if tm is not None else None
            N.check(N.lib().gsw_gemm_small(x.data_ptr(), K, w.data_ptr(), K, bias.data_ptr() if bias is not None else None,
                                           resid.data_ptr() if resid is not None else None, Nn, y.data_ptr(), Nn, M, K, Nn, m, tokens, width, None, 0, 0.0, None, None,
                                           rs_buf.data_ptr() if rs_buf is not None else None, rs_buf.numel() if rs_buf is not None else 0, _C.byref(slots), -1,
                                           _dt(x.dtype), _stream_ptr()))
            if tm is not None:
                tm.stop(e0, ("gsw_mm_small_kernel", M, K, Nn, mode) if tm.by_shape else "gsw_mm_small_kernel", 2.0 * M * K * Nn, nbytes=2.0 * (M * K + Nn * K + M * Nn * (2 if resid is not None else 1)))
        if stats_for is not None:
            stats_for.stats = None
        if rs_buf is not None and slots.value > 0:
            y._gsw_rowstats = (rs_buf, int(slots.value))
        return y
    with torch.cuda.device(x.device):
        e0 = tm.start() if tm is not None else None
        armed = _colstats_arm(M, Nn, x.device, geom=(M // tokens, tokens // width, width)) if (stats_for is not None and mode == "tok2pf") else None
        rs_buf = None
        if rowstats and mode == "plain" and FOLD_LN and M >= FOLD_LN_MIN_ROWS and M % 8 == 0:
            rs_buf = torch.empty(M * 2 * ((Nn + 159) // 160) * 2, dtype=torch.float32, device=x.device)
        ex = _extras(x.device, colstats=None if armed is None else armed[0], rowstats=rs_buf)
        ncols = Nn // 2 if mode == "geglu" else Nn
        N.check(N.lib().gsw_gemm_ex(x.data_ptr(), K, w.data_ptr(), K, bias.data_ptr() if bias is not None else None,
                                    resid.data_ptr() if resid is not None else None, Nn, y.data_ptr(), ncols, M, K, Nn, m, tokens, width,
                                    _dt(x.dtype), _C.byref(ex), _stream_ptr()))
        if stats_for is not None:
            stats_for.stats = _colstats_collect(armed, ex)
        if rs_buf is not None and ex.rowstats_slots > 0:
            y._gsw_rowstats = (rs_buf, int(ex.rowstats_slots))
        if tm is not None:
            tm.stop(e0, ("gsw_mm_kernel", M, K, Nn, mode + ("+res" if resid is not None and mode == "plain" else "")) if tm.by_shape else "gsw_mm_kernel", 2.0 * M * K * Nn,
                    nbytes=2.0 * (M * K + Nn * K + M * ncols * (2 if resid is not None else 1)))
    return y


def gemm2(x0: torch.Tensor, x1: torch.Tensor, w: torch.Tensor, bias: Optional[torch.Tensor] = None, *, resid: Optional[torch.Tensor] = None, mode: str = "tok2pf",
          tokens: int = 0, width: int = 0, out: Optional[torch.Tensor] = None, stats_for: Optional["PF"] = None) -> torch.Tensor:
    if x0.dtype not in (torch.float16, torch.bfloat16):
        raise ValueError(f"gemm2: fp16 / bf16 only (got {x0.dtype})")
    if mode not in ("plain", "tok2pf"):
        raise ValueError(f"gemm2: mode plain | tok2pf (got {mode!r})")
    _same(x0, x0, "x0")
    K0, K1 = x0.shape[-1], x1.shape[-1]
    M = x0.numel() // K0
    _same(x1, x0, "x1", M * K1)
    Nn = w.shape[0]
    _same(w, x0, "w", Nn * (K0 + K1))
    _same(bias, x0, "bias", Nn)
    if mode == "plain":
        _same(resid, x0, "resid", M * Nn)
        y = torch.empty((*x0.shape[:-1], Nn), dtype=x0.dtype, device=x0.device) if out is None else out
        _same(y, x0, "out", M * Nn)
    else:
        if out is None or tokens <= 0 or width <= 0 or tokens % width or M % tokens:
            raise ValueError("gemm2: tok2pf needs out (PF rows), tokens = H*W and width = W")
        y = out
        rows = (M // tokens) * (tokens // width + 2) * (width + 2)
        _same(y, x0, "out", rows * Nn)
        _same(resid, x0, "resid", rows * Nn)
    tm = CONV_TIMER
    with torch.cuda.device(x0.device):
        e0 = tm.start() if tm is not None else None
        armed = _colstats_arm(M, Nn, x0.device, geom=(M // tokens, tokens // width, width)) if (stats_for is not None and mode == "tok2pf") else None
        ex = _extras(x0.device, colstats=None if armed is None else armed[0])
        N.check(N.lib().gsw_gemm2_ex(x0.data_ptr(), K0, K0, x1.data_ptr(), K1, K1, w.data_ptr(), K0 + K1, bias.data_ptr() if bias is not None else None,
                                     resid.data_ptr() if resid is not None else None, Nn, y.data_ptr(), Nn, M, Nn, GEMM_MODES[mode], tokens, width,
                                     _dt(x0.dtype), _C.byref(ex), _stream_ptr()))
        if stats_for is not None:
            stats_for.stats = _colstats_collect(armed, ex)
        if tm is not None:
            K = K0 + K1
            tm.stop(e0, ("gsw_mm_kernel", M, K, Nn, mode + "2" + ("+res" if resid is not None else "")) if tm.by_shape else "gsw_mm_kernel", 2.0 * M * K * Nn,
                    nbytes=2.0 * (M * K + Nn * K + M * Nn * (2 if resid is not None else 1)))
    return y


FOLD_LN = True
FOLD_LN_MIN_ROWS = int(os.environ.get("GSW_FOLD_LN_MIN_ROWS", "1024"))


def ln_stat(x: torch.Tensor, eps: float) -> Optional[torch.Tensor]:
    done = getattr(x, "_gsw_lnstat", None)
    if done is not None and FOLD_LN and done[1] == float(eps):
        return done[0]
    rs = getattr(x, "_gsw_rowstats", None)
    if rs is None or not FOLD_LN:
        return None
    C = x.shape[-1]
    M = x.numel() // C
    if M % 8 or M < FOLD_LN_MIN_ROWS:
        return None
    out = torch.empty((M, 2), dtype=torch.float32, device=x.device)
    with torch.cuda.device(x.device):
        N.check(N.lib().gsw_ln_rowstats_finish(rs[0].data_ptr(), rs[1], M, C, float(eps), out.data_ptr(), _stream_ptr()))
    return out


def fold_ln_weights(w: torch.Tensor, b: Optional[torch.Tensor], gamma: torch.Tensor, beta: torch.Tensor, geglu: bool = False):
    wf = w.detach().float()
    wp = (wf * gamma.detach().float()[None, :]).to(w.dtype)
    u = wp.float().sum(dim=1)
    v = wf @ beta.detach().float()
    if b is not None:
        v = v + b.detach().float()
    if geglu:
        wp, u = pack_geglu_weight(wp, u)
        _, v = pack_geglu_weight(wp, v)
    return wp.contiguous(), u.contiguous(), v.contiguous()


def gemm_ln(x: torch.Tensor, stat: torch.Tensor, wp: torch.Tensor, u: torch.Tensor, v: torch.Tensor, *, mode: str = "plain", tokens: int = 0) -> torch.Tensor:
    K = x.shape[-1]
    M = x.numel() // K
    Nn = wp.shape[0]
    _same(x, x, "x")
    _same(wp, x, "w", Nn * K)
    for t_, nm in ((stat, "stat"), (u, "u"), (v, "v")):
        if t_.dtype != torch.float32 or t_.device != x.device or not t_.is_contiguous() or t_.data_ptr() % 16:
            raise ValueError(f"gemm_ln: {nm} must be a contiguous, 16-byte aligned fp32 tensor on {x.device}")
    if stat.numel() != 2 * M or u.numel() != Nn or v.numel() != Nn:
        raise ValueError("gemm_ln: stat [M, 2], u [N], v [N]")
    if mode == "plain":
        y = torch.empty((*x.shape[:-1], Nn), dtype=x.dtype, device=x.device)
    elif mode == "geglu":
        y = torch.empty((*x.shape[:-1], Nn // 2), dtype=x.dtype, device=x.device)
    elif mode == "trans":
        if tokens <= 0 or M % tokens:
            raise ValueError("gemm_ln: trans needs tokens = rows per image")
        y = torch.empty((M // tokens, Nn, tokens), dtype=x.dtype, device=x.device)
    else:
        raise ValueError(mode)
    tm = CONV_TIMER
    with torch.cuda.device(x.device):
        e0 = tm.start() if tm is not None else None
        ex = _extras(x.device)
        N.check(N.lib().gsw_gemm_ln_ex(x.data_ptr(), stat.data_ptr(), wp.data_ptr(), u.data_ptr(), v.data_ptr(), y.data_ptr(), M, K, Nn,
                                       GEMM_MODES[mode], tokens, _dt(x.dtype), _C.byref(ex), _stream_ptr()))
        if tm is not None:
            tm.stop(e0, ("gsw_mm_kernel", M, K, Nn, mode + "+ln") if tm.by_shape else "gsw_mm_kernel", 2.0 * M * K * Nn, nbytes=2.0 * (M * K + Nn * K) + y.numel() * 2.0 + M * 8.0)
    return y


def gemm_qkv(x: torch.Tensor, w: torch.Tensor, n_rows: int, bias: Optional[torch.Tensor] = None):
    if x.dtype not in (torch.float16, torch.bfloat16) or x.dim() != 3:
        raise ValueError("gemm_qkv: fp16 / bf16 tokens [B, S, K]")
    B, S, K = x.shape
    Nn = w.shape[0]
    _same(x, x, "x")
    _same(w, x, "w", Nn * K)
    _same(bias, x, "bias", Nn)
    if n_rows <= 0 or n_rows >= Nn or n_rows % 160 or S % 8:
        raise ValueError("gemm_qkv: n_rows must be a multiple of 160 inside (0, N), S a multiple of 8")
    rows = torch.empty((B, S, n_rows), dtype=x.dtype, device=x.device)
    vt = torch.empty((B, Nn - n_rows, S), dtype=x.dtype, device=x.device)
    tm = CONV_TIMER
    with torch.cuda.device(x.device):
        e0 = tm.start() if tm is not None else None
        N.check(N.lib().gsw_gemm_qkv(x.data_ptr(), w.data_ptr(), bias.data_ptr() if bias is not None else None, rows.data_ptr(), vt.data_ptr(),
                                     B * S, K, n_rows, Nn, S, _dt(x.dtype), _stream_ptr()))
        if tm is not None:
            tm.stop(e0, ("gsw_mm_kernel", B * S, K, Nn, "qkv") if tm.by_shape else "gsw_mm_kernel", 2.0 * B * S * K * Nn, nbytes=2.0 * (B * S * K + Nn * K + B * S * Nn))
    return rows, vt


def groupnorm_pf2(x: PF, x2: Optional[PF], gamma: torch.Tensor, beta: torch.Tensor, groups: int, eps: float, *, act: bool = True) -> PF:
    if x2 is None:
        return groupnorm_pf(x, gamma, beta, groups, eps, act=act)
    dev = x.buf.device
    C = x.C + x2.C
    _same(x2.buf, x.buf, "x2")
    _same(gamma, x.buf, "gamma", C)
    _same(beta, x.buf, "beta", C)
    if (x2.B, x2.H, x2.W) != (x.B, x.H, x.W):
        raise ValueError("groupnorm_pf2: the two sources differ in geometry")
    if x.C % 8 == 0 and _gn_fused_ok(x.B, x.H, x.W, C, groups):
        _ensure_border(x); _ensure_border(x2)
        return _groupnorm_fused(x, x2, gamma, beta, groups, eps, act, False)
    ws = _gn_workspace(dev, x.B, groups, C)
    y = PF.empty(x.B, x.H, x.W, C, x.buf.dtype, dev)
    if FUSE_GN_STATS and _stats_usable(x) and _stats_usable(x2) and C <= 4096 and (C // groups) % 2 == 0 and x.C % 2 == 0:
        s1, s2 = x.stats, x2.stats
        with torch.cuda.device(dev):
            N.check(N.lib().gsw_groupnorm_pf_cs(x.rows.data_ptr(), x2.rows.data_ptr(), x.C, s1.buf.data_ptr(), s1.rows, s1.npar, s1.blocks,
                                                s2.buf.data_ptr(), s2.rows, s2.npar, s2.blocks, gamma.data_ptr(), beta.data_ptr(), y.rows.data_ptr(),
                                                ws.data_ptr(), x.B, x.H, x.W, C, groups, eps, 1 if act else 0, 0, _dt(x.buf.dtype), _stream_ptr()))
        return y
    _ensure_border(x); _ensure_border(x2)
    with torch.cuda.device(dev):
        N.check(N.lib().gsw_groupnorm_pf2(x.rows.data_ptr(), x2.rows.data_ptr(), x.C, gamma.data_ptr(), beta.data_ptr(), y.rows.data_ptr(),
                                          ws.data_ptr(), x.B, x.H, x.W, C, groups, eps, 1 if act else 0, 0, _dt(x.buf.dtype), _stream_ptr()))
    return y


def conv3x3_res_fusable(x: PF, n_out: int) -> bool:
    return n_out % 8 == 0 and n_out >= 128 and x.C % 64 == 0


def conv3x3_res_pf(x: PF, w_cat: torch.Tensor, bias: Optional[torch.Tensor], *, rowbias: Optional[torch.Tensor] = None,
                   resid: Optional[PF] = None, x1: Optional[PF] = None, x2: Optional[PF] = None) -> PF:
    Nn = w_cat.shape[0]
    _same(w_cat, x.buf, "w_cat", Nn * (9 * x.C + (x1.C if x1 is not None else 0) + (x2.C if x2 is not None else 0)))
    _same(bias, x.buf, "bias", Nn)
    ldrb = _rowbias_ld(rowbias, x.buf, x.B, Nn)
    for t_, nm in ((resid, "resid"), (x1, "x1"), (x2, "x2")):
        if t_ is not None:
            _same(t_.buf, x.buf, nm)
    y = PF.empty(x.B, x.H, x.W, Nn, x.buf.dtype, x.buf.device)
    tm = CONV_TIMER
    with torch.cuda.device(x.buf.device):
        e0 = tm.start() if tm is not None else None
        armed = _colstats_arm(x.B * x.H * x.W, Nn, x.buf.device, geom=(x.B, x.H, x.W))
        ex = _extras(x.buf.device, colstats=None if armed is None else armed[0])
        N.check(N.lib().gsw_conv3x3_res_pf_ex(x.rows.data_ptr(), w_cat.data_ptr(), bias.data_ptr() if bias is not None else None,
                                              rowbias.data_ptr() if rowbias is not None else None, ldrb,
                                              resid.rows.data_ptr() if resid is not None else None, y.rows.data_ptr(),
                                              x.B, x.H, x.W, x.C, Nn,
                                              x1.rows.data_ptr() if x1 is not None else None, x1.C if x1 is not None else 0,
                                              x2.rows.data_ptr() if x2 is not None else None, x2.C if x2 is not None else 0,
                                              _dt(x.buf.dtype), _C.byref(ex), _stream_ptr()))
        y.stats = _colstats_collect(armed, ex)
        if tm is not None:
            k = 9 * x.C + (x1.C if x1 is not None else 0) + (x2.C if x2 is not None else 0)
            name = _conv_kernel_name(x.W, Nn, 3, 1)
            pix = x.B * x.H * x.W
            tm.stop(e0, (name, x.B, x.H, x.W, k, Nn, 1) if tm.by_shape else name, 2.0 * pix * Nn * k,
                    nbytes=2.0 * (pix * (k - 8 * x.C) + Nn * k + pix * Nn * (2 if resid is not None else 1)))
    return y


ATTN_HEAD_DIMS = (40, 64, 80, 160)


def half_gpu(x: torch.Tensor) -> bool:
    return x.is_cuda and x.dtype in (torch.float16, torch.bfloat16)


def attention_ok(x: torch.Tensor, heads: int, head_dim: int, n_q: int, n_k: int) -> bool:
    return half_gpu(x) and head_dim in ATTN_HEAD_DIMS and n_q >= 1 and n_k % 8 == 0


def dup_pf(x: "PF") -> "PF":
    y = PF.empty(2 * x.B, x.H, x.W, x.C, x.buf.dtype, x.buf.device)
    r = y.rows
    r[: x.M].copy_(x.rows)
    r[x.M:].copy_(x.rows)
    return y


def attention(q: torch.Tensor, k: torch.Tensor, vt: torch.Tensor, heads: int, scale: Optional[float] = None,
              valid_keys: Optional[int] = None, out: Optional[torch.Tensor] = None) -> torch.Tensor:
    B, Sq, inner = q.shape
    Sk = k.shape[1]
    d = inner // heads
    assert inner == heads * d and vt.shape == (B, inner, Sk) and k.shape[2] == inner

    def rows(t):
        if t.stride(2) == 1 and t.stride(0) == t.shape[1] * t.stride(1) and t.stride(1) % 8 == 0 and t.data_ptr() % 16 == 0:
            return t, t.stride(1)
        t = t.contiguous()
        return t, inner

    (q, ldq), (k, ldk) = rows(q), rows(k)
    vt = vt.contiguous()
    for t_, nm in ((k, "k"), (vt, "vt")):
        if t_.dtype != q.dtype or t_.device != q.device:
            raise ValueError(f"attention: {nm} is {t_.dtype} on {t_.device}, q is {q.dtype} on {q.device}")
    if out is None:
        out = torch.empty((B, Sq, inner), dtype=q.dtype, device=q.device)
    elif tuple(out.shape) != (B, Sq, inner) or out.dtype != q.dtype or out.device != q.device or not out.is_contiguous():
        raise ValueError("attention: out must be a contiguous [B, Sq, heads * d] tensor like q")
    tm = CONV_TIMER
    with torch.cuda.device(q.device):
        e0 = tm.start() if tm is not None else None
        ks_ok = (ATTN_KEY_SPLIT and d in (40, 64) and Sq % 128 == 0 and Sk % 64 == 0 and Sk // 64 >= 32 and (valid_keys is None or int(valid_keys) == Sk)
                 and (Sq // 128) * B * heads <= 256)
        ws = _workspace(q.device) if ks_ok else None
        N.check(N.lib().gsw_attention_ws(q.data_ptr(), k.data_ptr(), vt.data_ptr(), out.data_ptr(), B, heads, d, Sq, Sk,
                                         Sk if valid_keys is None else int(valid_keys), ldq, ldk, inner,
                                         float(scale if scale is not None else d ** -0.5), _dt(q.dtype), 0 if ws is None else ws.data_ptr(),
                                         0 if ws is None else ws.numel(), _stream_ptr()))
        if tm is not None:
            tm.stop(e0, ("gsw_attn_fwd_kernel", B, Sq, Sk, heads, d) if tm.by_shape else "gsw_attn_fwd_kernel", 4.0 * B * heads * Sq * (Sk if valid_keys is None else int(valid_keys)) * d,
                    nbytes=2.0 * heads * d * (2 * out.shape[0] * Sq + 2 * B * Sk))
    return out


attention_hd64 = attention


def pack_upsample_weight(w: torch.Tensor) -> torch.Tensor:
    rows = {(0, 0): (0,), (0, 1): (1, 2), (1, 0): (0, 1), (1, 1): (2,)}
    wf = w.detach().float()
    out = []
    for dy in (0, 1):
        for dx in (0, 1):
            taps = []
            for a in (0, 1):
                for b in (0, 1):
                    taps.append(sum(wf[:, :, kh, kw] for kh in rows[(dy, a)] for kw in rows[(dx, b)]))
            out.append(torch.stack(taps, dim=1).reshape(w.shape[0], -1))
    return torch.stack(out).to(w.dtype).contiguous()


def conv_up2x_fusable(x: PF, n_out: int) -> bool:
    return n_out % 8 == 0 and n_out >= 128 and x.C % 64 == 0


def conv_up2x_pf(x: PF, w4: torch.Tensor, bias: Optional[torch.Tensor]) -> PF:
    Nn = w4.shape[1]
    _same(w4, x.buf, "w4", 4 * Nn * 4 * x.C)
    _same(bias, x.buf, "bias", Nn)
    y = PF.empty(x.B, 2 * x.H, 2 * x.W, Nn, x.buf.dtype, x.buf.device)
    tm = CONV_TIMER
    with torch.cuda.device(x.buf.device):
        e0 = tm.start() if tm is not None else None
        armed = _colstats_arm(x.B * x.H * x.W, Nn, x.buf.device, npar=4, geom=(x.B, 2 * x.H, 2 * x.W))
        ex = _extras(x.buf.device, colstats=None if armed is None else armed[0])
        N.check(N.lib().gsw_conv_up2x_pf_ex(x.rows.data_ptr(), w4.data_ptr(), bias.data_ptr() if bias is not None else None, y.rows.data_ptr(),
                                            x.B, x.H, x.W, x.C, Nn, _dt(x.buf.dtype), _C.byref(ex), _stream_ptr()))
        y.stats = _colstats_collect(armed, ex, npar=4)
        if tm is not None:
            name = "gsw_mm_kernel(up2x)"
            tm.stop(e0, (name, x.B, 2 * x.H, 2 * x.W, 4 * x.C, Nn, 1) if tm.by_shape else name,
                    2.0 * x.B * 4 * x.H * x.W * Nn * 4 * x.C, launches=4, nbytes=2.0 * (4 * x.B * x.H * x.W * x.C + 16 * Nn * x.C + 4 * x.B * x.H * x.W * Nn))
    return y
```

a-watermark-for-diffusion-models_amd/unet.py:

```python
from __future__ import annotations

import math
import os
import warnings
from typing import Optional, Sequence

import torch
import torch.nn as nn
import torch.nn.functional as F

from . import _native as N
from . import checkpoint, codec, graph, pf, xattn


FUSED_KERNELS = True


def _fusable(x: torch.Tensor) -> bool:
    return FUSED_KERNELS and x.is_cuda and x.dtype in (torch.float16, torch.bfloat16, torch.float32) and x.is_contiguous() \
        and (x.shape[-1] * x.shape[-2]) % 8 == 0


def gn_act(x: torch.Tensor, norm: nn.GroupNorm, act: bool = True, pre_bias: Optional[torch.Tensor] = None) -> torch.Tensor:
    if _fusable(x):
        return codec.groupnorm_silu(x, norm.weight, norm.bias, norm.num_groups, norm.eps, act=act, pre_bias=pre_bias)
    if pre_bias is not None:
        x = x + pre_bias[:, :, None, None]
    y = norm(x)
    return F.silu(y) if act else y


USE_PF = True


def _pw(conv: nn.Conv2d) -> torch.Tensor:
    return pf.cached(conv, "_gsw_packed", (conv.weight,), lambda: pf.pack_conv_weight(conv.weight.detach()))


UPSAMPLE_SUBPIXEL = True

CACHE_CONTEXT_KV = True

FUSED_QK = True

FUSED_QKV = False

OWN_ATTENTION = True

OWN_GEMM = True

FOLD_FF_OUT = os.environ.get("GSW_FOLD_FF_OUT", "1") != "0"

FALLBACKS = {}

STRICT = os.environ.get("GSW_STRICT_KERNELS", "1") != "0"


def _note_fallback(why: str):
    if STRICT:
        raise RuntimeError("gswm unet (strict kernels): " + why + " -- this call would run a library kernel (hipBLASLt / MIOpen / SDPA); "
                           "pass --strict_kernels 0 to allow it")
    if why not in FALLBACKS:
        warnings.warn("gswm unet: " + why, RuntimeWarning, stacklevel=3)
    FALLBACKS[why] = FALLBACKS.get(why, 0) + 1


def _own_gemm_ok(x: torch.Tensor, K: int, N: int) -> bool:
    if not (OWN_GEMM and USE_PF and FUSED_KERNELS and pf.half_gpu(x)):
        return False
    if K % 64 or N % 8:
        _note_fallback(f"linear K={K} N={N}: library GEMM")
        return False
    return True


def _wb(lin: nn.Linear, x: torch.Tensor):
    if lin.weight.dtype != x.dtype or lin.weight.device != x.device or not lin.weight.is_contiguous():
        raise ValueError(f"linear weight is {lin.weight.dtype} on {lin.weight.device}, activations are {x.dtype} on {x.device}")
    return lin.weight, lin.bias


def _lin(x: torch.Tensor, lin: nn.Linear, resid: Optional[torch.Tensor] = None, out: Optional[torch.Tensor] = None, rowstats: bool = False) -> torch.Tensor:
    if _own_gemm_ok(x, lin.in_features, lin.out_features):
        w, b = _wb(lin, x)
        return pf.gemm(x.contiguous(), w, b, resid=None if resid is None else resid.contiguous(), out=out, rowstats=rowstats)
    y = lin(x)
    y = y if resid is None else y + resid
    return y if out is None else out.copy_(y)


def _lin_t(x: torch.Tensor, lin: nn.Linear, out: Optional[torch.Tensor] = None) -> torch.Tensor:
    b, n, _ = x.shape
    if _own_gemm_ok(x, lin.in_features, lin.out_features) and n % 8 == 0:
        w, bias = _wb(lin, x)
        return pf.gemm(x.contiguous(), w, bias, mode="trans", tokens=n, out=out)
    vt = torch.bmm(lin.weight.unsqueeze(0).expand(b, -1, -1), x.transpose(1, 2))
    vt = vt if lin.bias is None else vt + lin.bias[None, :, None]
    return vt if out is None else out.copy_(vt)


def timestep_embedding(t: torch.Tensor, dim: int, max_period: float = 10000.0) -> torch.Tensor:
    half = dim // 2
    freqs = torch.exp(-math.log(max_period) * torch.arange(half, dtype=torch.float32, device=t.device) / half)
    args = t.float()[:, None] * freqs[None]
    return torch.cat([torch.cos(args), torch.sin(args)], dim=-1)


class TimestepEmbedding(nn.Module):
    def __init__(self, in_dim, dim):
        super().__init__()
        self.linear_1 = nn.Linear(in_dim, dim)
        self.linear_2 = nn.Linear(dim, dim)

    def forward(self, x):
        return _lin(F.silu(_lin(x, self.linear_1)), self.linear_2)


class TembRows:
    __slots__ = ("act", "rows", "table", "widths")

    def __init__(self, act, table, widths):
        self.act, self.table, self.widths, self.rows, off = act, table, widths, {}, 0
        for key, n in widths:
            self.rows[key] = table[:, off:off + n]
            off += n

    def doubled(self) -> "TembRows":
        return TembRows(None if self.act is None else torch.cat([self.act, self.act], dim=0), torch.cat([self.table, self.table], dim=0), self.widths)


class ResnetBlock2D(nn.Module):
    def __init__(self, cin, cout, temb_dim, groups=32, eps=1e-5):
        super().__init__()
        self.norm1 = nn.GroupNorm(groups, cin, eps=eps)
        self.conv1 = nn.Conv2d(cin, cout, 3, padding=1)
        self.time_emb_proj = nn.Linear(temb_dim, cout)
        self.norm2 = nn.GroupNorm(groups, cout, eps=eps)
        self.conv2 = nn.Conv2d(cout, cout, 3, padding=1)
        self.conv_shortcut = nn.Conv2d(cin, cout, 1) if cin != cout else None

    def forward(self, x, temb_act):
        h = self.conv1(gn_act(x, self.norm1))
        h = self.conv2(gn_act(h, self.norm2, pre_bias=self.time_emb_proj(temb_act)))
        return (x if self.conv_shortcut is None else self.conv_shortcut(x)) + h

    def forward_pf(self, x, temb_act, x2=None):
        cout = self.conv2.out_channels
        fuse = self.conv_shortcut is not None and pf.conv3x3_res_fusable(x, cout) and (x2 is None or x2.C % 64 == 0)
        if x2 is not None and not fuse:
            x, x2 = pf.PF(torch.cat([x.buf, x2.buf], dim=1), x.B, x.H, x.W, x.C + x2.C), None
        n1 = pf.groupnorm_pf2(x, x2, self.norm1.weight, self.norm1.bias, self.norm1.num_groups, self.norm1.eps, act=True)
        rowbias = temb_act.rows[id(self)] if isinstance(temb_act, TembRows) else _lin(temb_act, self.time_emb_proj).contiguous()
        h = pf.conv_pf(n1, _pw(self.conv1), self.conv1.bias, rowbias=rowbias, gn_only=True)
        h = pf.gn_pf(h, self.norm2)
        if self.conv_shortcut is None:
            return pf.conv_pf(h, _pw(self.conv2), self.conv2.bias, resid=x)
        if not fuse:
            sc = pf.conv_pf(x, _pw(self.conv_shortcut), self.conv_shortcut.bias, ksize=1)
            return pf.conv_pf(h, _pw(self.conv2), self.conv2.bias, resid=sc)
        c = pf.cached(self, "_gsw_res", (self.conv2.weight, self.conv2.bias, self.conv_shortcut.weight, self.conv_shortcut.bias),
                   lambda: (torch.cat([_pw(self.conv2), self.conv_shortcut.weight.detach()[:, :, 0, 0]], dim=1).contiguous(),
                            (self.conv2.bias.detach() + self.conv_shortcut.bias.detach()).contiguous()))
        return pf.conv3x3_res_pf(h, c[0], c[1], x1=x, x2=x2)


def _padded_ctx(ctx: torch.Tensor):
    n = ctx.shape[1]
    if n % 64 == 0:
        return ctx, n
    cached = getattr(ctx, "_gsw_pad", None)
    if cached is not None and cached[1].device == ctx.device and cached[1].dtype == ctx.dtype:
        if cached[0] == ctx._version:
            return cached[1], n
        cached[1][:, :n].copy_(ctx)
        ctx._gsw_pad = (ctx._version, cached[1])
        return cached[1], n
    pad = F.pad(ctx, (0, 0, 0, (-n) % 64)).contiguous()
    ctx._gsw_pad = (ctx._version, pad)
    return pad, n


def _padded_keys(ctx: torch.Tensor) -> int:
    return (ctx.shape[1] + 63) // 64 * 64


class Attention(nn.Module):
    def __init__(self, dim, ctx_dim, heads, head_dim):
        super().__init__()
        if head_dim is None:
            head_dim = dim // heads
        inner = heads * head_dim
        self.heads = heads
        self.to_q = nn.Linear(dim, inner, bias=False)
        self.to_k = nn.Linear(ctx_dim, inner, bias=False)
        self.to_v = nn.Linear(ctx_dim, inner, bias=False)
        self.to_out = nn.ModuleList([nn.Linear(inner, dim)])

    @property
    def head_dim(self) -> int:
        return self.to_q.out_features // self.heads

    def _no_qkv_bias(self) -> bool:
        return self.to_q.bias is None and self.to_k.bias is None and self.to_v.bias is None

    def _wcat(self, which: str) -> torch.Tensor:
        ws = tuple(getattr(self, "to_" + c).weight for c in which)
        return pf.cached(self, "_gsw_w" + which, ws, lambda: torch.cat([w.detach() for w in ws], dim=0).contiguous())

    def _folded(self, which: str, norm: nn.LayerNorm):
        ws = tuple(getattr(self, "to_" + c).weight for c in which)
        return pf.cached(self, "_gsw_ln_" + which, ws + (norm.weight, norm.bias),
                         lambda: pf.fold_ln_weights(ws[0].detach() if len(ws) == 1 else torch.cat([w.detach() for w in ws], dim=0), None, norm.weight, norm.bias))

    def context_kv(self, src: torch.Tensor):
        store = getattr(src, "_gsw_kv", None)
        if store is None:
            store = {}
            src._gsw_kv = store
        ver = (src._version, self.to_k.weight._version, self.to_v.weight._version, self.to_k.weight.data_ptr(), self.to_v.weight.data_ptr())
        ent = store.get(id(self))
        if ent is None or ent[0] != ver:
            ent = (ver, _lin(src, self.to_k, out=None if ent is None else ent[1]), _lin_t(src, self.to_v, out=None if ent is None else ent[2]))
            store[id(self)] = ent
        return ent[1], ent[2]

    def forward_ln(self, x, stat, norm: nn.LayerNorm, ctx=None, resid=None, project: bool = True):
        n = x.shape[1]
        inner = self.to_q.out_features
        if ctx is None:
            qk = pf.gemm_ln(x, stat, *self._folded("qk", norm))
            vt = pf.gemm_ln(x, stat, *self._folded("v", norm), mode="trans", tokens=n)
            o = pf.attention(qk[..., :inner], qk[..., inner:], vt, self.heads)
        else:
            src, valid = _padded_ctx(ctx)
            fq = self._folded("q", norm)
            k_ctx, vt_ctx = self.context_kv(src)
            o = pf.attention(pf.gemm_ln(x, stat, *fq), k_ctx, vt_ctx, self.heads, valid_keys=valid)
        if not project:
            return o
        return _lin(o, self.to_out[0], resid, rowstats=True)

    def fused_sublayer(self, x, stat, norm: nn.LayerNorm, ctx, eps_next: Optional[float] = None, pre=None):
        blob, v, idx = xattn.context_operands(self, norm, ctx, x.dtype)
        if pre is not None:
            return xattn.fused(x, None, blob, v, idx, ctx.shape[0], self.heads, eps_out=eps_next, pre_o=pre[0], pre_w=xattn.out_projection_operand(pre[1], x.dtype),
                               pre_eps=norm.eps)
        return xattn.fused(x, stat, blob, v, idx, ctx.shape[0], self.heads, eps_out=eps_next)

    def cross_dup(self, x, ctx, *, stat=None, norm: Optional[nn.LayerNorm] = None):
        B = x.shape[0]
        src, valid = _padded_ctx(ctx)
        k_ctx, vt_ctx = self.context_kv(src)
        q = pf.gemm_ln(x, stat, *self._folded("q", norm)) if stat is not None else _lin(x, self.to_q)
        o = torch.empty((2 * B, x.shape[1], self.to_q.out_features), dtype=x.dtype, device=x.device)
        pf.attention(q, k_ctx[:B], vt_ctx[:B], self.heads, valid_keys=valid, out=o[:B])
        pf.attention(q, k_ctx[B:], vt_ctx[B:], self.heads, valid_keys=valid, out=o[B:])
        return o

    def ln_foldable(self, x, ctx=None) -> bool:
        n = x.shape[1]
        return (OWN_ATTENTION and FUSED_KERNELS and n % 8 == 0 and self._no_qkv_bias()
                and pf.attention_ok(x, self.heads, self.head_dim, n, n if ctx is None else _padded_keys(ctx)) and (ctx is None or CACHE_CONTEXT_KV)
                and _own_gemm_ok(x, self.to_q.in_features, self.to_q.out_features))

    def _qkv(self, x, src, cross: bool):
        n, inner = x.shape[1], self.to_q.out_features
        if cross and CACHE_CONTEXT_KV:
            k_ctx, vt_ctx = self.context_kv(src)
            return _lin(x, self.to_q), k_ctx, vt_ctx
        if (not cross and FUSED_QK and FUSED_QKV and self._no_qkv_bias() and (2 * inner) % 160 == 0 and n % 8 == 0
                and _own_gemm_ok(x, self.to_q.in_features, 3 * inner)):
            wqkv = self._wcat("qkv")
            if wqkv.dtype == x.dtype:
                qk, vt = pf.gemm_qkv(x.contiguous(), wqkv, 2 * inner)
                return qk[..., :inner], qk[..., inner:], vt
        vt = _lin_t(src, self.to_v)
        if not cross and FUSED_QK:
            wqk = self._wcat("qk")
            qk = pf.gemm(x.contiguous(), wqk, None) if _own_gemm_ok(x, wqk.shape[1], wqk.shape[0]) else F.linear(x, wqk)
            return qk[..., :inner], qk[..., inner:], vt
        return _lin(x, self.to_q), _lin(src, self.to_k), vt

    def forward(self, x, ctx=None, resid=None):
        b, n, _ = x.shape
        if OWN_ATTENTION and FUSED_KERNELS:
            src, valid = (x, n) if ctx is None else _padded_ctx(ctx)
            if pf.attention_ok(x, self.heads, self.head_dim, n, src.shape[1]):
                q, k, vt = self._qkv(x, src, ctx is not None)
                return _lin(pf.attention(q, k, vt, self.heads, valid_keys=valid), self.to_out[0], resid)
            if pf.half_gpu(x):
                _note_fallback(f"attention head_dim={self.head_dim} Sq={n} Sk={src.shape[1]}: torch SDPA")
        ctx = x if ctx is None else ctx
        q = _lin(x, self.to_q).view(b, n, self.heads, -1).transpose(1, 2)
        k = _lin(ctx, self.to_k).view(b, ctx.shape[1], self.heads, -1).transpose(1, 2)
        v = _lin(ctx, self.to_v).view(b, ctx.shape[1], self.heads, -1).transpose(1, 2)
        o = F.scaled_dot_product_attention(q, k, v)
        return _lin(o.transpose(1, 2).reshape(b, n, -1), self.to_out[0], resid)


class GEGLU(nn.Module):
    def __init__(self, dim, inner):
        super().__init__()
        self.proj = nn.Linear(dim, inner * 2)

    def forward(self, x):
        inner = self.proj.out_features // 2
        if _own_gemm_ok(x, self.proj.in_features, self.proj.out_features) and inner % 80 == 0:
            _wb(self.proj, x)
            c = pf.cached(self, "_gsw_geglu", (self.proj.weight, self.proj.bias), lambda: pf.pack_geglu_weight(self.proj.weight.detach(), self.proj.bias.detach()))
            return pf.gemm(x.contiguous(), c[0], c[1], mode="geglu")
        y = self.proj(x)
        if FUSED_KERNELS and y.is_cuda and y.is_contiguous() and (y.shape[-1] // 2) % 8 == 0:
            return codec.geglu(y)
        h, gate = y.chunk(2, dim=-1)
        return h * F.gelu(gate)


class FeedForward(nn.Module):
    def __init__(self, dim, mult=4):
        super().__init__()
        self.net = nn.ModuleList([GEGLU(dim, dim * mult), nn.Identity(), nn.Linear(dim * mult, dim)])

    def forward(self, x, resid=None, rowstats: bool = False):
        return _lin(self.net[0](x), self.net[2], resid, rowstats=rowstats)

    def _folded(self, norm: nn.LayerNorm):
        proj = self.net[0].proj
        return pf.cached(self, "_gsw_ln_ff1", (proj.weight, proj.bias, norm.weight, norm.bias),
                         lambda: pf.fold_ln_weights(proj.weight.detach(), proj.bias, norm.weight, norm.bias, geglu=True))

    def forward_ln(self, x, stat, norm: nn.LayerNorm, resid=None):
        return _lin(pf.gemm_ln(x, stat, *self._folded(norm), mode="geglu"), self.net[2], resid, rowstats=True)


def _fused_block_ok(like: torch.Tensor, channels: int) -> bool:
    return FUSED_KERNELS and pf.half_gpu(like) and channels % 8 == 0 and channels <= 1536


def _cached_kv_on() -> bool:
    return OWN_ATTENTION and FUSED_KERNELS and CACHE_CONTEXT_KV


class BasicTransformerBlock(nn.Module):
    def __init__(self, dim, ctx_dim, heads, head_dim):
        super().__init__()
        self.norm1 = nn.LayerNorm(dim)
        self.attn1 = Attention(dim, dim, heads, head_dim)
        self.norm2 = nn.LayerNorm(dim)
        self.attn2 = Attention(dim, ctx_dim, heads, head_dim)
        self.norm3 = nn.LayerNorm(dim)
        self.ff = FeedForward(dim)

    @staticmethod
    def fused_ok(x) -> bool:
        return _fused_block_ok(x, x.shape[-1]) and x.is_contiguous()

    def dup_ok(self, x, ctx) -> bool:
        a = self.attn2
        return (self.fused_ok(x) and _cached_kv_on() and ctx.shape[0] == 2 * x.shape[0]
                and pf.attention_ok(x, a.heads, a.head_dim, x.shape[1], _padded_keys(ctx)))

    def _cross_sublayer(self, x, ctx, dup: bool, one_launch: bool):
        st = pf.ln_stat(x, self.norm2.eps) if (one_launch or self.attn2.ln_foldable(x, ctx[: x.shape[0]] if dup else ctx)) else None
        if st is not None and one_launch:
            return self.attn2.fused_sublayer(x, st, self.norm2, ctx, eps_next=self.norm3.eps)
        if dup:
            if st is not None:
                o = self.attn2.cross_dup(x, ctx, stat=st, norm=self.norm2)
            else:
                _, n = codec.add_layernorm(x, None, self.norm2.weight, self.norm2.bias, self.norm2.eps)
                o = self.attn2.cross_dup(n, ctx)
            return _lin(o, self.attn2.to_out[0], torch.cat([x, x], dim=0), rowstats=True)
        if st is not None:
            return self.attn2.forward_ln(x, st, self.norm2, ctx, resid=x)
        _, n = codec.add_layernorm(x, None, self.norm2.weight, self.norm2.bias, self.norm2.eps)
        return self.attn2(n, ctx, resid=x)

    def forward(self, x, ctx, dup: bool = False, ff_split: bool = False):
        if dup and not self.dup_ok(x, ctx):
            x, dup = torch.cat([x, x], dim=0), False
        if not self.fused_ok(x):
            if ff_split:
                raise RuntimeError("BasicTransformerBlock: ff_split is a form of the fused path")
            x = x + self.attn1(self.norm1(x))
            x = x + self.attn2(self.norm2(x), ctx)
            return x + self.ff(self.norm3(x))
        one_launch = xattn.usable(x, self.attn2, ctx)
        st = pf.ln_stat(x, self.norm1.eps) if self.attn1.ln_foldable(x) else None
        if st is not None and one_launch and xattn.pre_usable(self.attn1.to_out[0]):
            o1 = self.attn1.forward_ln(x, st, self.norm1, project=False)
            x = self.attn2.fused_sublayer(x, None, self.norm2, ctx, eps_next=self.norm3.eps, pre=(o1, self.attn1.to_out[0]))
        else:
            if st is not None:
                x = self.attn1.forward_ln(x, st, self.norm1, resid=x)
            else:
                _, n = codec.add_layernorm(x, None, self.norm1.weight, self.norm1.bias, self.norm1.eps)
                x = self.attn1(n, resid=x)
            x = self._cross_sublayer(x, ctx, dup, one_launch)
        inner4 = self.ff.net[2].in_features
        st = pf.ln_stat(x, self.norm3.eps) if (inner4 % 80 == 0 and _own_gemm_ok(x, x.shape[-1], 2 * inner4)) else None
        if st is not None:
            if ff_split:
                return pf.gemm_ln(x, st, *self.ff._folded(self.norm3), mode="geglu"), x
            return self.ff.forward_ln(x, st, self.norm3, resid=x)
        _, n = codec.add_layernorm(x, None, self.norm3.weight, self.norm3.bias, self.norm3.eps)
        if ff_split:
            return self.ff.net[0](n), x
        return self.ff(n, resid=x)


def fold_ff_out(w2: torch.Tensor, b2: torch.Tensor, wp: torch.Tensor, bp: torch.Tensor):
    acc = torch.float64 if wp.dtype == torch.float64 else torch.float32
    wpf, w2f = wp.detach().to(acc), w2.detach().to(acc)
    w_cat = torch.cat([wpf @ w2f, wpf], dim=1).to(wp.dtype).contiguous()
    b = (wpf @ b2.detach().to(acc) + bp.detach().to(acc)).to(wp.dtype).contiguous()
    return w_cat, b


class Transformer2DModel(nn.Module):
    def __init__(self, ch, ctx_dim, heads, head_dim, layers=1, groups=32):
        super().__init__()
        self.norm = nn.GroupNorm(groups, ch, eps=1e-6)
        self.proj_in = nn.Linear(ch, ch)
        self.transformer_blocks = nn.ModuleList([BasicTransformerBlock(ch, ctx_dim, heads, head_dim) for _ in range(layers)])
        self.proj_out = nn.Linear(ch, ch)

    def forward(self, x, ctx):
        b, c, h, w = x.shape
        y = gn_act(x, self.norm, act=False).permute(0, 2, 3, 1).reshape(b, h * w, c)
        y = self.proj_in(y)
        for blk in self.transformer_blocks:
            y = blk(y, ctx)
        y = self.proj_out(y).reshape(b, h, w, c).permute(0, 3, 1, 2)
        return x + y

    def _ff_out_folded(self):
        l2, po = self.transformer_blocks[-1].ff.net[2], self.proj_out
        return pf.cached(self, "_gsw_ff_out", (l2.weight, l2.bias, po.weight, po.bias), lambda: fold_ff_out(l2.weight, l2.bias, po.weight, po.bias))

    def _ff_out_fold_ok(self, y, dup: bool) -> bool:
        C = self.proj_out.in_features
        if not (FOLD_FF_OUT and len(self.transformer_blocks) > 0 and C % 64 == 0):
            return False
        l2 = self.transformer_blocks[-1].ff.net[2]
        rows = y.shape[0] * y.shape[1] * (2 if dup else 1)
        return (BasicTransformerBlock.fused_ok(y) and l2.bias is not None and self.proj_out.bias is not None and l2.out_features == C and l2.in_features % 64 == 0
                and self.proj_out.out_features == C and rows > pf.SMALL_GEMM_MAX_ROWS and _own_gemm_ok(y, l2.in_features, C) and _own_gemm_ok(y, C, C))

    def forward_pf(self, x, ctx, dup: bool = False):
        if xattn.gn_proj_usable(x, self.norm, self.proj_in):
            y = xattn.gn_proj(x, self.norm, self.proj_in, eps_next=self.transformer_blocks[0].norm1.eps)
        else:
            y = _lin(pf.gn_pf(x, self.norm, act=False, tokens=True), self.proj_in, rowstats=True)
        last = len(self.transformer_blocks) - 1
        fold = self._ff_out_fold_ok(y, dup)
        for i, blk in enumerate(self.transformer_blocks):
            y = blk(y, ctx, dup=dup and i == 0, ff_split=fold and i == last)
        if dup:
            x = pf.dup_pf(x)
        if fold:
            h, y = y
            w, b = self._ff_out_folded()
            pf.gemm2(h.contiguous(), y.contiguous(), w, b, resid=x.rows, mode="tok2pf", tokens=x.H * x.W, width=x.W, out=x.rows, stats_for=x)
        elif _own_gemm_ok(y, self.proj_out.in_features, self.proj_out.out_features):
            w, b = _wb(self.proj_out, y)
            pf.gemm(y.contiguous(), w, b, resid=x.rows, mode="tok2pf", tokens=x.H * x.W, width=x.W, out=x.rows, stats_for=x)
        else:
            x.interior.add_(_lin(y, self.proj_out).view(x.B, x.H, x.W, x.C))
            x.stats = None
        return x


class Downsample2D(nn.Module):
    def __init__(self, ch):
        super().__init__()
        self.conv = nn.Conv2d(ch, ch, 3, stride=2, padding=1)

    def forward(self, x):
        return self.conv(x)

    def forward_pf(self, x):
        return pf.conv_pf(x, _pw(self.conv), self.conv.bias, stride=2)


class Upsample2D(nn.Module):
    def __init__(self, ch):
        super().__init__()
        self.conv = nn.Conv2d(ch, ch, 3, padding=1)

    def forward(self, x):
        return self.conv(F.interpolate(x, scale_factor=2.0, mode="nearest"))

    def forward_pf(self, x):
        if UPSAMPLE_SUBPIXEL and pf.conv_up2x_fusable(x, self.conv.out_channels):
            w4 = pf.cached(self, "_gsw_up4", (self.conv.weight,), lambda: pf.pack_upsample_weight(self.conv.weight))
            return pf.conv_up2x_pf(x, w4, self.conv.bias)
        up = pf.PF.zeros(x.B, 2 * x.H, 2 * x.W, x.C, x.buf.dtype, x.buf.device)
        xi, g = x.interior, up.grid
        for dy in (0, 1):
            for dx in (0, 1):
                g[:, 1 + dy:1 + dy + 2 * x.H:2, 1 + dx:1 + dx + 2 * x.W:2, :].copy_(xi)
        return pf.conv_pf(up, _pw(self.conv), self.conv.bias)


class DownBlock(nn.Module):
    def __init__(self, cin, cout, temb, ctx_dim, heads, head_dim, layers, attn, down):
        super().__init__()
        self.resnets = nn.ModuleList([ResnetBlock2D(cin if i == 0 else cout, cout, temb) for i in range(layers)])
        self.attentions = nn.ModuleList([Transformer2DModel(cout, ctx_dim, heads, head_dim) for _ in range(layers)]) if attn else None
        self.downsamplers = nn.ModuleList([Downsample2D(cout)]) if down else None

    def forward(self, x, temb, ctx, skips):
        for i, r in enumerate(self.resnets):
            x = r(x, temb)
            if self.attentions is not None:
                x = self.attentions[i](x, ctx)
            skips.append(x)
        if self.downsamplers is not None:
            x = self.downsamplers[0](x)
            skips.append(x)
        return x

    def forward_pf(self, x, temb, ctx, skips, dup_temb=None):
        for i, r in enumerate(self.resnets):
            x = r.forward_pf(x, temb)
            if self.attentions is not None:
                x = self.attentions[i].forward_pf(x, ctx, dup=dup_temb is not None and i == 0)
                if dup_temb is not None and i == 0:
                    temb = dup_temb
            skips.append(x)
        if self.downsamplers is not None:
            x = self.downsamplers[0].forward_pf(x)
            skips.append(x)
        return x


class UpBlock(nn.Module):
    def __init__(self, cin, cout, cprev, temb, ctx_dim, heads, head_dim, layers, attn, up):
        super().__init__()
        rs = []
        for i in range(layers):
            skip = cin if i == layers - 1 else cout
            rin = cprev if i == 0 else cout
            rs.append(ResnetBlock2D(rin + skip, cout, temb))
        self.resnets = nn.ModuleList(rs)
        self.attentions = nn.ModuleList([Transformer2DModel(cout, ctx_dim, heads, head_dim) for _ in range(layers)]) if attn else None
        self.upsamplers = nn.ModuleList([Upsample2D(cout)]) if up else None

    def forward(self, x, temb, ctx, skips):
        for i, r in enumerate(self.resnets):
            x = r(torch.cat([x, skips.pop()], dim=1), temb)
            if self.attentions is not None:
                x = self.attentions[i](x, ctx)
        if self.upsamplers is not None:
            x = self.upsamplers[0](x)
        return x

    def forward_pf(self, x, temb, ctx, skips):
        for i, r in enumerate(self.resnets):
            x = r.forward_pf(x, temb, x2=skips.pop())
            if self.attentions is not None:
                x = self.attentions[i].forward_pf(x, ctx)
        if self.upsamplers is not None:
            x = self.upsamplers[0].forward_pf(x)
        return x


class MidBlock(nn.Module):
    def __init__(self, ch, temb, ctx_dim, heads, head_dim):
        super().__init__()
        self.resnets = nn.ModuleList([ResnetBlock2D(ch, ch, temb), ResnetBlock2D(ch, ch, temb)])
        self.attentions = nn.ModuleList([Transformer2DModel(ch, ctx_dim, heads, head_dim)])

    def forward(self, x, temb, ctx):
        return self.resnets[1](self.attentions[0](self.resnets[0](x, temb), ctx), temb)

    def forward_pf(self, x, temb, ctx):
        return self.resnets[1].forward_pf(self.attentions[0].forward_pf(self.resnets[0].forward_pf(x, temb), ctx), temb)


TEMB_TABLE = True
NUM_TRAIN_TIMESTEPS = 1000

CONV_OUT_DIRECT_MAX_PIXELS = 65536

CFG_SHARED_PREFIX = os.environ.get("GSW_CFG_SHARED_PREFIX", "1") != "0"


def _edge_conv_weights(self):
    w_in, w_out = self.conv_in.weight, self.conv_out.weight

    def build():
        wi = torch.zeros((w_in.shape[0], 64, 3, 3), dtype=w_in.dtype, device=w_in.device)
        wi[:, : w_in.shape[1]] = w_in.detach()
        wo = torch.zeros((64, w_out.shape[1], 3, 3), dtype=w_out.dtype, device=w_out.device)
        wo[: w_out.shape[0]] = w_out.detach()
        bo = torch.zeros(64, dtype=w_out.dtype, device=w_out.device)
        bo[: w_out.shape[0]] = self.conv_out.bias.detach()
        return pf.pack_conv_weight(wi), pf.pack_conv_weight(wo), bo

    return pf.cached(self, "_gsw_edge", (w_in, w_out, self.conv_out.bias), build)


def _resnets(self):
    resnets = getattr(self, "_gsw_resnets", None)
    if resnets is None:
        resnets = self._gsw_resnets = [m for m in self.modules() if isinstance(m, ResnetBlock2D)]
    return resnets


def _temb_widths(resnets):
    return [(id(r), r.time_emb_proj.out_features) for r in resnets]


def _temb_rows(self, temb: torch.Tensor):
    resnets = _resnets(self)
    widths = _temb_widths(resnets)
    if not resnets or not _own_gemm_ok(temb, temb.shape[-1], sum(n for _, n in widths)) or any(n % 8 for _, n in widths):
        return temb
    params = tuple(p for r in resnets for p in (r.time_emb_proj.weight, r.time_emb_proj.bias))
    wcat, bcat = pf.cached(self, "_gsw_temb_cat", params, lambda: (torch.cat([r.time_emb_proj.weight.detach() for r in resnets], dim=0).contiguous(),
                                                                     torch.cat([r.time_emb_proj.bias.detach() for r in resnets], dim=0).contiguous()))
    if wcat.dtype != temb.dtype:
        return temb
    return TembRows(temb, pf.gemm(temb.contiguous(), wcat, bcat), widths)


def _temb_rows_from_table(self, t: torch.Tensor, x: torch.Tensor):
    if t.dtype not in (torch.int64, torch.int32) or not t.is_cuda or t.numel() not in (1, x.shape[0]):
        return None
    resnets = _resnets(self)
    if not resnets or any(r.time_emb_proj.out_features % 8 for r in resnets):
        return None
    te = self.time_embedding
    if te.linear_1.weight.dtype != x.dtype or te.linear_1.weight.device != x.device:
        return None
    params = (te.linear_1.weight, te.linear_1.bias, te.linear_2.weight, te.linear_2.bias) + tuple(p for r in resnets for p in (r.time_emb_proj.weight, r.time_emb_proj.bias))

    def build():
        with torch.no_grad():
            tt = torch.arange(int(getattr(self, "num_train_timesteps", NUM_TRAIN_TIMESTEPS)), device=x.device)
            temb = F.silu(te(timestep_embedding(tt, self.c0).to(x.dtype)))
            rows = _temb_rows(self, temb)
            if not isinstance(rows, TembRows):
                return None
            return rows.table.contiguous()

    table = pf.cached(self, "_gsw_temb_table", params, build)
    if table is not None and table.shape[0] != int(getattr(self, "num_train_timesteps", NUM_TRAIN_TIMESTEPS)):
        self._gsw_temb_table = None
        table = pf.cached(self, "_gsw_temb_table", params, build)
        graph.weights_changed()
    if table is None:
        return None
    B, n_tot = x.shape[0], table.shape[1]
    idx = t if t.dtype == torch.int64 else t.to(torch.int64)
    out = torch.empty((B, n_tot), dtype=table.dtype, device=table.device)
    with torch.cuda.device(x.device):
        N.check(N.lib().gsw_gather_rows(table.data_ptr(), n_tot * table.element_size(), table.shape[0], idx.data_ptr(), 0 if idx.numel() == 1 else 1,
                                        out.data_ptr(), n_tot * table.element_size(), B, n_tot * table.element_size(), codec._stream_ptr()))
    return TembRows(None, out, _temb_widths(resnets))


class UNet2DCondition(nn.Module):

    @classmethod
    def sd15(cls) -> "UNet2DCondition":
        return cls(cross_attention_dim=768, num_heads=(8, 8, 8, 8), head_dim=None)

    def __init__(self, in_channels=4, out_channels=4, block_out_channels: Sequence[int] = (320, 640, 1280, 1280), layers_per_block=2,
                 cross_attention_dim=1024, num_heads: Sequence[int] = (5, 10, 20, 20), head_dim=64,
                 attn_blocks: Sequence[bool] = (True, True, True, False)):
        super().__init__()
        c0 = block_out_channels[0]
        temb = c0 * 4
        self.c0 = c0
        self.conv_in = nn.Conv2d(in_channels, c0, 3, padding=1)
        self.time_embedding = TimestepEmbedding(c0, temb)
        self.down_blocks = nn.ModuleList()
        ch = c0
        n = len(block_out_channels)
        for i, co in enumerate(block_out_channels):
            self.down_blocks.append(DownBlock(ch, co, temb, cross_attention_dim, num_heads[i], co // num_heads[i] if head_dim is None else head_dim,
                                              layers_per_block, attn_blocks[i], i < n - 1))
            ch = co
        self.mid_block = MidBlock(ch, temb, cross_attention_dim, num_heads[-1], head_dim)
        self.up_blocks = nn.ModuleList()
        rev = list(reversed(block_out_channels))
        rheads = list(reversed(num_heads))
        rattn = list(reversed(attn_blocks))
        cprev = ch
        for i, co in enumerate(rev):
            cin = rev[min(i + 1, n - 1)]
            self.up_blocks.append(UpBlock(cin, co, cprev, temb, cross_attention_dim, rheads[i], head_dim, layers_per_block + 1, rattn[i], i < n - 1))
            cprev = co
        self.conv_norm_out = nn.GroupNorm(32, c0, eps=1e-5)
        self.conv_out = nn.Conv2d(c0, out_channels, 3, padding=1)

    supports_cfg_dup = True

    def forward(self, x: torch.Tensor, t: torch.Tensor, ctx: torch.Tensor, cfg_dup: bool = False) -> torch.Tensor:
        if cfg_dup:
            if ctx.shape[0] != 2 * x.shape[0] or t.numel() not in (1, x.shape[0]):
                raise ValueError("cfg_dup: ctx must hold 2B contexts for the B latents, t one timestep or B")
            if not (CFG_SHARED_PREFIX and self._pf_ok(x) and self._cfg_dup_ok(x, ctx)):
                return self.forward(torch.cat([x, x], dim=0), t if t.numel() == 1 else torch.cat([t, t]), ctx)
        if self._pf_ok(x):
            rows = _temb_rows_from_table(self, t, x) if TEMB_TABLE else None
            if rows is not None:
                return self._forward_pf(x, rows, ctx, cfg_dup)
        if t.dim() == 0:
            t = t.expand(x.shape[0])
        temb = self.time_embedding(timestep_embedding(t, self.c0).to(x.dtype))
        temb = F.silu(temb)
        if self._pf_ok(x):
            return self._forward_pf(x, _temb_rows(self, temb), ctx, cfg_dup)
        if USE_PF and FUSED_KERNELS and pf.half_gpu(x):
            _note_fallback(f"UNet forward on {tuple(x.shape)} {x.dtype}: off the padded-flat path (fp16 / bf16, conv channels % 64, lattice % {1 << (len(self.down_blocks) - 1)}): plain torch modules")
        h = self.conv_in(x)
        skips = [h]
        for blk in self.down_blocks:
            h = blk(h, temb, ctx, skips)
        h = self.mid_block(h, temb, ctx)
        for blk in self.up_blocks:
            h = blk(h, temb, ctx, skips)
        return self.conv_out(gn_act(h, self.conv_norm_out)).contiguous(memory_format=torch.contiguous_format)

    def _pf_ok(self, x: torch.Tensor) -> bool:
        if not (USE_PF and FUSED_KERNELS and pf.half_gpu(x)):
            return False
        ok = getattr(self, "_pf_shapes_ok", None)
        if ok is None:
            ok = all(m.in_channels % 64 == 0 and m.out_channels % 64 == 0 for n, m in self.named_modules()
                     if isinstance(m, nn.Conv2d) and n not in ("conv_in", "conv_out"))
            self._pf_shapes_ok = ok
        n_down = len(self.down_blocks) - 1
        return ok and x.shape[-1] % (1 << n_down) == 0 and x.shape[-2] % (1 << n_down) == 0

    def _cfg_dup_ok(self, x: torch.Tensor, ctx: torch.Tensor) -> bool:
        b0 = self.down_blocks[0]
        if b0.attentions is None or not isinstance(b0.attentions[0].transformer_blocks[0], BasicTransformerBlock):
            return False
        a = b0.attentions[0].transformer_blocks[0].attn2
        return (_fused_block_ok(x, b0.attentions[0].proj_in.out_features) and _cached_kv_on() and OWN_GEMM and a.head_dim in pf.ATTN_HEAD_DIMS
                and _own_gemm_ok(x, a.to_q.in_features, a.to_q.out_features))

    def _forward_pf(self, x: torch.Tensor, temb, ctx: torch.Tensor, cfg_dup: bool = False) -> torch.Tensor:
        w_in, w_out, b_out = _edge_conv_weights(self)
        B, cin, H, W = x.shape
        xin = pf.PF.empty(B, H, W, 64, x.dtype, x.device)
        xc = x.contiguous()
        with torch.cuda.device(x.device):
            N.check(N.lib().gsw_nchw_to_pf(xc.data_ptr(), xin.rows.data_ptr(), B, cin, H, W, 64, codec._dt(x.dtype), codec._stream_ptr()))
        h = pf.conv_pf(xin, w_in, self.conv_in.bias)
        skips = [h]
        if cfg_dup:
            temb2 = temb.doubled() if isinstance(temb, TembRows) else torch.cat([temb, temb], dim=0)
            h = self.down_blocks[0].forward_pf(h, temb, ctx, skips, dup_temb=temb2)
            skips[0] = pf.dup_pf(skips[0])
            temb, B = temb2, 2 * B
            rest = self.down_blocks[1:]
        else:
            rest = self.down_blocks
        for blk in rest:
            h = blk.forward_pf(h, temb, ctx, skips)
        h = self.mid_block.forward_pf(h, temb, ctx)
        for blk in self.up_blocks:
            h = blk.forward_pf(h, temb, ctx, skips)
        hn = pf.gn_pf(h, self.conv_norm_out, act=True)
        nout = self.conv_out.out_channels
        if B * H * W <= CONV_OUT_DIRECT_MAX_PIXELS and nout <= 16 and hn.C % 32 == 0 and self.conv_out.bias is not None:
            wo = pf.cached(self.conv_out, "_gsw_packed_direct", (self.conv_out.weight,), lambda: pf.pack_conv_weight(self.conv_out.weight.detach()))
            y = torch.empty((B, nout, H, W), dtype=x.dtype, device=x.device)
            with torch.cuda.device(x.device):
                N.check(N.lib().gsw_conv3x3_pf_nchw(hn.rows.data_ptr(), wo.data_ptr(), self.conv_out.bias.data_ptr(), y.data_ptr(), B, H, W, hn.C, nout,
                                                    codec._dt(x.dtype), codec._stream_ptr()))
            return y
        y = pf.conv_pf(hn, w_out, b_out)
        return y.interior[..., :nout].permute(0, 3, 1, 2).contiguous()

    def prepare_context(self, ctx: torch.Tensor) -> None:
        if not (_cached_kv_on() and ctx.is_cuda):
            return
        src, _ = _padded_ctx(ctx)
        for blk in self.modules():
            if isinstance(blk, BasicTransformerBlock):
                a = blk.attn2
                if pf.attention_ok(ctx, a.heads, a.head_dim, 1, src.shape[1]):
                    a.context_kv(src)
                if xattn.layer_usable(a, ctx, ctx.dtype):
                    xattn.context_operands(a, blk.norm2, ctx, ctx.dtype)
                    if xattn.pre_usable(blk.attn1.to_out[0]):
                        xattn.out_projection_operand(blk.attn1.to_out[0], ctx.dtype)


def synthetic_init_(model: nn.Module, seed: int = 0, out_scale: float = 1.0) -> nn.Module:
    g = torch.Generator().manual_seed(seed)
    n_res = 0
    for name, p in model.named_parameters():
        if p.dim() >= 2:
            fan_in = p[0].numel()
            std = (1.0 / fan_in) ** 0.5
            if name.endswith(("conv2.weight", "to_out.0.weight", "net.2.weight", "proj_out.weight")):
                std *= 0.3
                n_res += 1
            if name == "conv_out.weight":
                std *= out_scale
            with torch.no_grad():
                p.copy_(torch.randn(p.shape, generator=g) * std)
        else:
            with torch.no_grad():
                p.fill_(1.0 if name.endswith("weight") and "norm" in name else 0.0)
    return model


def load_diffusers_state_dict(model: nn.Module, weight_dir: str) -> nn.Module:
    sd = dict(checkpoint.load_component_state_dict(weight_dir, "unet"))
    own = dict(model.named_parameters())
    for k, v in list(sd.items()):
        if k in own and v.dim() == 4 and own[k].dim() == 2 and v.shape[2:] == (1, 1):
            sd[k] = v[:, :, 0, 0]
    missing, unexpected = model.load_state_dict(sd, strict=False)
    if missing or unexpected:
        raise RuntimeError(f"state dict mismatch: missing {missing[:5]}..., unexpected {unexpected[:5]}...")
    graph.weights_changed()
    return model


def count_cfg_shared_prefix_flops(model: nn.Module, h: int = 64, w: int = 64) -> int:
    from torch.utils.flop_counter import FlopCounterMode
    import copy
    m = copy.deepcopy(model).to("meta")
    dt = next(m.parameters()).dtype
    b0 = m.down_blocks[0]
    if b0.attentions is None:
        return 0
    tr = b0.attentions[0]
    blk = tr.transformer_blocks[0]
    x = torch.empty(1, m.conv_in.in_channels, h, w, device="meta", dtype=dt)
    temb = torch.empty(1, m.time_embedding.linear_2.out_features, device="meta", dtype=dt)
    with FlopCounterMode(display=False) as fc:
        hh = m.conv_in(x)
        hh = b0.resnets[0](hh, temb)
        y = tr.proj_in(tr.norm(hh).permute(0, 2, 3, 1).reshape(1, h * w, -1))
        y = y + blk.attn1(blk.norm1(y))
        blk.attn2.to_q(blk.norm2(y))
    return int(fc.get_total_flops())


def count_flops_per_image(model: nn.Module, h: int = 64, w: int = 64, ctx_len: int = 77, ctx_dim: Optional[int] = None) -> int:
    from torch.utils.flop_counter import FlopCounterMode
    import copy
    m = copy.deepcopy(model).to("meta")
    if ctx_dim is None:
        ctx_dim = next(mod for n, mod in m.named_modules() if n.endswith("attn2")).to_k.in_features
    dt = next(m.parameters()).dtype
    x = torch.empty(1, 4, h, w, device="meta", dtype=dt)
    t = torch.empty(1, device="meta")
    c = torch.empty(1, ctx_len, ctx_dim, device="meta", dtype=dt)
    with FlopCounterMode(display=False) as fc:
        m(x, t, c)
    return int(fc.get_total_flops())
```

include/gswm.h:

```cpp
#ifndef GSWM_H
#define GSWM_H

#include <stddef.h>
#include <stdint.h>

#ifdef __cplusplus
extern "C" {
#endif

#if defined(__GNUC__)
#pragma GCC visibility push(default)
#endif

#define GSW_VERSION 500

#define GSW_MSG_INLINE_MAX 256

typedef enum gsw_dtype {
    GSW_F32 = 0,
    GSW_F16 = 1,
    GSW_BF16 = 2,
    GSW_F64 = 3
} gsw_dtype;

typedef enum gsw_status {
    GSW_OK = 0,
    GSW_ERR_BAD_ARG = 1,
    GSW_ERR_UNSUPPORTED = 2,
    GSW_ERR_RAGGED = 3,
    GSW_ERR_HIP = 4,
    GSW_WARN_NO_RECORDS = 5
} gsw_status;

#define GSW_EMBED_EXACT_F64 0u
#define GSW_EMBED_FAST_F32 1u

#define GSW_FLAG_SATURATED 1u
#define GSW_FLAG_NAN 2u

int gsw_version(void);
int gsw_build_flags(void);
const char* gsw_strerror(int status);
int gsw_last_hip_error(void);

int gsw_keystream(const uint8_t key[32], const uint8_t nonce16[16], uint8_t* out_dev, size_t nbytes, void* stream);

int gsw_embed(const uint8_t key[32], const uint8_t nonce16[16], const uint8_t* msg, int msg_bytes,
              const double* u_dev, uint64_t seed, uint64_t image_index0, void* out_dev, int out_dtype, int B,
              int64_t n_elems, uint32_t flags, void* stream);

int gsw_philox_uniform(uint64_t seed, uint64_t image_index0, double* u_dev, int B, int64_t n_elems, void* stream);

int gsw_extract(const void* z_dev, int z_dtype, const uint8_t key[32], const uint8_t nonce16[16], int msg_bits,
                uint8_t* bits_dev, uint32_t* counts_dev, uint32_t* flags_dev, int B, int64_t n_elems, void* stream);

int gsw_bit_matches(const uint8_t* bits_dev, int msg_bits, const uint8_t* ref_msg, int ref_bits,
                    uint32_t* matches_dev, int B, void* stream);

int gsw_ddim_step(const void* x_dev, const void* model_out_dev, void* out_dev, float a, float b, int dtype,
                  int64_t n, void* stream);

int gsw_ddim_step_cfg(const void* x_dev, const void* e_uncond_dev, const void* e_text_dev, void* out_dev, float a,
                      float b, float guidance, int dtype, int64_t n, void* stream);

int gsw_dpm_step(const void* x_dev, const void* e_uncond_dev, const void* e_text_dev ,
                 const void* m_prev_dev , void* x_out_dev, void* m_out_dev, float P, float Q, float A,
                 float B, float C, float guidance, int dtype, int64_t n, void* stream);

int gsw_ddim_step_extract(const void* x_dev, const void* model_out_dev, void* z_out_dev, float a, float b, int dtype,
                          const uint8_t key[32], const uint8_t nonce16[16], int msg_bits, uint8_t* bits_dev,
                          uint32_t* counts_dev, uint32_t* flags_dev, int B, int64_t n_elems, void* stream);

int gsw_groupnorm_silu(const void* x_dev, const void* pre_bias_dev, const void* gamma_dev, const void* beta_dev, void* out_dev, int B, int C,
                       int HW, int groups, float eps, int act, int dtype, void* stream);
int gsw_geglu(const void* in_dev, void* out_dev, int64_t rows, int inner, int dtype, void* stream);

int gsw_conv_pf(const void* x_dev, const void* w_dev, const void* bias_dev, const void* rowbias_dev, int ld_rowbias, const void* resid_dev, void* y_dev,
                int B, int H, int W, int C, int N, int ksize, int stride, int ldx, int dtype, void* stream);

int gsw_groupnorm_pf(const void* x_dev, const void* gamma_dev, const void* beta_dev, void* out_dev, float* workspace_dev, int B, int H, int W,
                     int C, int groups, float eps, int act, int out_tokens, int dtype, void* stream);

int gsw_groupnorm_pf2(const void* x_dev, const void* x2_dev, int Ca, const void* gamma_dev, const void* beta_dev, void* out_dev, float* workspace_dev,
                      int B, int H, int W, int C, int groups, float eps, int act, int out_tokens, int dtype, void* stream);

#define GSW_MM_GN_ONLY 1
typedef struct GswMmExtras {
    float* colstats_dev;
    int64_t colstats_capacity;
    float* rowstats_dev;
    int64_t rowstats_capacity;
    void* workspace_dev;
    int64_t workspace_bytes;
    int max_splits;
    int colstats_rows_per_block, colstats_blocks, rowstats_slots, splits;
    int flags;
} GswMmExtras;

int gsw_gemm_ex(const void* x_dev, int64_t ldx, const void* w_dev, int64_t ldw, const void* bias_dev, const void* resid_dev, int64_t ldr, void* y_dev, int64_t ldy,
                int64_t M, int K, int N, int mode, int S, int Wimg, int dtype, GswMmExtras* ex, void* stream);
int gsw_gemm2_ex(const void* x0_dev, int64_t ld0, int K0, const void* x1_dev, int64_t ld1, int K1, const void* w_dev, int64_t ldw, const void* bias_dev,
                 const void* resid_dev, int64_t ldr, void* y_dev, int64_t ldy, int64_t M, int N, int mode, int S, int Wimg, int dtype, GswMmExtras* ex, void* stream);
int gsw_gemm_ln_ex(const void* x_dev, const float* ln_stat_dev, const void* w_dev, const float* u_dev, const float* v_dev, void* y_dev, int64_t M, int K, int N,
                   int mode, int S, int dtype, GswMmExtras* ex, void* stream);
int gsw_conv_pf_ex(const void* x_dev, const void* w_dev, const void* bias_dev, const void* rowbias_dev, int ld_rowbias, const void* resid_dev, void* y_dev,
                   int B, int H, int W, int C, int N, int ksize, int stride, int ldx, int dtype, GswMmExtras* ex, void* stream);
int gsw_conv3x3_res_pf_ex(const void* x_dev, const void* w_dev, const void* bias_dev, const void* rowbias_dev, int ld_rowbias, const void* resid_dev, void* y_dev,
                          int B, int H, int W, int C, int N, const void* x1_dev, int C1, const void* x2_dev, int C2, int dtype, GswMmExtras* ex, void* stream);
int gsw_conv_up2x_pf_ex(const void* x_dev, const void* w4_dev, const void* bias_dev, void* y_dev, int B, int H, int W, int C, int N, int dtype, GswMmExtras* ex,
                        void* stream);

int gsw_groupnorm_pf_cs(const void* x_dev, const void* x2_dev, int Ca, const float* cs1_dev, int cs1_rows, int cs1_npar, int cs1_blocks,
                        const float* cs2_dev, int cs2_rows, int cs2_npar, int cs2_blocks, const void* gamma_dev, const void* beta_dev, void* out_dev,
                        float* workspace_dev, int B, int H, int W, int C, int groups, float eps, int act, int out_tokens, int dtype, void* stream);

int gsw_conv3x3_res_pf(const void* x_dev, const void* w_dev, const void* bias_dev, const void* rowbias_dev, int ld_rowbias, const void* resid_dev, void* y_dev,
                       int B, int H, int W, int C, int N, const void* x1_dev, int C1, const void* x2_dev, int C2, int dtype, void* stream);

int gsw_add_layernorm(const void* x_dev, const void* delta_dev, const void* gamma_dev, const void* beta_dev, void* xnew_dev, void* y_dev,
                      int64_t rows, int C, float eps, int dtype, void* stream);


#define GSW_GEMM_PLAIN 0
#define GSW_GEMM_GEGLU 1
#define GSW_GEMM_TRANS 2
#define GSW_GEMM_TOK2PF 3
int gsw_gemm(const void* x_dev, const void* w_dev, const void* bias_dev, const void* resid_dev, void* y_dev, int64_t M, int K, int N,
             int mode, int S, int Wimg, int dtype, void* stream);
int gsw_gemm_qkv(const void* x_dev, const void* w_dev, const void* bias_dev, void* rows_dev, void* trans_dev, int64_t M, int K, int N_rows, int N,
                 int S, int dtype, void* stream);

int gsw_ln_rowstats_finish(const float* records_dev, int slots, int64_t M, int C, float eps, float* stat_dev, void* stream);
int gsw_gemm_ln(const void* x_dev, const float* ln_stat_dev, const void* w_dev, const float* u_dev, const float* v_dev, void* y_dev, int64_t M, int K, int N,
                int mode, int S, int dtype, void* stream);

int gsw_gemm_strided(const void* x_dev, int64_t ldx, const void* w_dev, int64_t ldw, const void* bias_dev, const void* resid_dev, int64_t ldr,
                     void* y_dev, int64_t ldy, int64_t M, int K, int N, int mode, int S, int Wimg, int dtype, void* stream);

int gsw_mm_config(int tile_rows, int split_mask);
int gsw_mm_get_config(int* tile_rows, int* split_mask);

int gsw_softmax_rows(void* x_dev, int64_t rows, int cols, int64_t ld, float scale, int dtype, void* stream);

int gsw_groupnorm_pf_fused(const void* x_dev, const void* x2_dev, int Ca, const void* gamma_dev, const void* beta_dev, void* out_dev, int B, int H, int W,
                           int C, int groups, float eps, int act, int out_tokens, int dtype, void* stream);
int gsw_gather_rows(const void* table_dev, int64_t ld_bytes, int64_t nrows, const int64_t* index_dev, int index_stride, void* out_dev, int64_t out_ld_bytes,
                    int B, int64_t row_bytes, void* stream);
int gsw_nchw_to_pf(const void* x_dev, void* y_dev, int B, int Cin, int H, int W, int Cp, int dtype, void* stream);
int gsw_conv3x3_pf_nchw(const void* x_dev, const void* w_dev, const void* bias_dev, void* y_dev, int B, int H, int W, int C, int Nout, int dtype, void* stream);

int gsw_gemm_small_config(int64_t M, int K, int N, int mode);
int gsw_gemm_small(const void* x_dev, int64_t ldx, const void* w_dev, int64_t ldw, const void* bias_dev, const void* resid_dev, int64_t ldr, void* y_dev, int64_t ldy,
                   int64_t M, int K, int N, int mode, int S, int Wimg, const float* ln_records_dev, int ln_slots, float ln_eps, const float* ln_u_dev,
                   const float* ln_v_dev, float* rowstats_dev, int64_t rowstats_capacity, int* rowstats_slots, int config, int dtype, void* stream);

int gsw_conv_up2x_pf(const void* x_dev, const void* w4_dev, const void* bias_dev, void* y_dev, int B, int H, int W, int C, int N, int dtype,
                     void* stream);

int gsw_attention(const void* q_dev, const void* k_dev, const void* vt_dev, void* out_dev, int B, int H, int head_dim, int Sq, int Sk,
                  int Sk_valid, int ldq, int ldk, int ldo, float scale, int dtype, void* stream);
int gsw_attention_ws(const void* q_dev, const void* k_dev, const void* vt_dev, void* out_dev, int B, int H, int head_dim, int Sq, int Sk,
                     int Sk_valid, int ldq, int ldk, int ldo, float scale, int dtype, void* workspace_dev, int64_t workspace_bytes, void* stream);
int gsw_xattn_fused(const void* x_dev, const float* ln_stat_dev, const void* blob_dev, int64_t blob_stride_bytes, const float* v_dev, int64_t v_stride_floats,
                    const int32_t* ctx_index_dev, void* out_dev, float* out_stat_dev, float out_eps, int x_images, int out_images, int tokens, int C, int heads,
                    int dtype, void* stream);
int gsw_xattn_fused_pre(const void* resid_dev, const void* o_dev, const void* w_frag_dev, float ln_eps, const void* blob_dev, int64_t blob_stride_bytes,
                        const float* v_dev, int64_t v_stride_floats, const int32_t* ctx_index_dev, void* out_dev, float* out_stat_dev, float out_eps, int x_images,
                        int out_images, int tokens, int C, int heads, int dtype, void* stream);

int gsw_gn_colstats_pairs(const float* cs_dev, int cs_rows, int cs_npar, int cs_blocks, float* pairsum_dev, int B, int H, int W, int C, void* stream);
int gsw_gn_proj_tokens(const void* x_pf_dev, const float* pairsum_dev, const void* gamma_dev, const void* beta_dev, float gn_eps, int groups, const void* w_frag_dev,
                       void* out_dev, float* out_stat_dev, float out_eps, int B, int H, int W, int C, int dtype, void* stream);

void gsw_mt19937_seed(uint32_t seed, uint32_t key[624]);
int gsw_mt19937_uniform(const uint32_t key[624], int pos, double* u_dev, int64_t n, uint32_t* state_out_dev, void* stream);

typedef enum gsw_image_mode {
    GSW_IMG_U8_HWC = 0,
    GSW_IMG_F16_CHW = 1,
    GSW_IMG_F32_CHW = 2
} gsw_image_mode;

int gsw_lanczos_plan(int in_size, int out_size, int32_t* bounds, int32_t* kk, int kk_capacity);

int gsw_resize_lanczos(const uint8_t* in_dev, int B, int Hin, int Win, void* out_dev, int Hout, int Wout, int out_mode, uint8_t* tmp_dev,
                       const int32_t* hbounds_dev, const int32_t* hkk_dev, int hksize, const int32_t* vbounds_dev, const int32_t* vkk_dev,
                       int vksize, void* stream);

int gsw_tensor_to_image(const void* in_dev, int dtype, int B, int H, int W, int denormalise, uint8_t* out_dev, void* stream);

int gsw_jpeg_quant_tables(int quality, uint8_t luma[64], uint8_t chroma[64]);
size_t gsw_jpeg_workspace_bytes(int B, int H, int W);
int gsw_jpeg_roundtrip(const uint8_t* rgb_dev, int B, int H, int W, int quality, void* out_dev, int out_mode, uint8_t* workspace_dev,
                       void* stream);

int gsw_gaussian_blur_params(float radius, int passes, int* box_radius, uint32_t* ww, uint32_t* fw);
int gsw_gaussian_blur(const uint8_t* rgb_dev, int B, int H, int W, float radius, uint8_t* out_dev, uint8_t* tmp_dev, void* stream);

typedef enum gsw_pointwise_op {
    GSW_PW_BRIGHTNESS = 0,
    GSW_PW_CONTRAST = 1,
    GSW_PW_INVERT = 2,
    GSW_PW_GRAY = 3,
    GSW_PW_HFLIP = 4,
    GSW_PW_VFLIP = 5,
    GSW_PW_NOISE = 6
} gsw_pointwise_op;
int gsw_image_pointwise(const uint8_t* rgb_dev, int B, int H, int W, int op, float strength, uint64_t seed, uint64_t image_index0,
                        void* out_dev, int out_mode, uint64_t* workspace_dev, void* stream);


typedef enum gsw_resample_filter {
    GSW_RESAMPLE_LANCZOS = 1,
    GSW_RESAMPLE_BILINEAR = 2
} gsw_resample_filter;

int gsw_resample_plan(int filter, int in_size, int out_size, int32_t* bounds, int32_t* kk, int kk_capacity);

int gsw_affine_nearest(const uint8_t* in_dev, int B, int H, int W, const int32_t* coeffs_dev, void* out_dev, int out_mode, void* stream);

int gsw_box_mask(const uint8_t* in_dev, int B, int H, int W, const int32_t* boxes_dev, int keep_inside, void* out_dev, int out_mode, void* stream);

int gsw_crop_resize(const uint8_t* in_dev, int B, int H, int W, const int32_t* origins_dev, int crop_h, int crop_w, void* out_dev, int Hout,
                    int Wout, int out_mode, uint8_t* tmp_dev, const int32_t* hbounds_dev, const int32_t* hkk_dev, int hksize,
                    const int32_t* vbounds_dev, const int32_t* vkk_dev, int vksize, void* stream);

#define GSW_TRACE_SOFT 0
#define GSW_TRACE_HARD 1
size_t gsw_trace_workspace_bytes(int B, int64_t n_users, int k);
int gsw_trace_topk(const uint32_t* counts_dev, int B, int msg_bits, int copies, int mode, const uint8_t* registry_dev, int64_t n_users, int k,
                   int32_t* idx_dev, int32_t* score_dev, void* workspace_dev, void* stream);

int gsw_sign_pack(const void* z_dev, int z_dtype, uint8_t* signs_dev, uint32_t* flags_dev, int B, int64_t n_elems, void* stream);

size_t gsw_trace_keyed_workspace_bytes(int B, int64_t n_records, int k);
int gsw_trace_keyed_topk(const uint8_t* signs_dev, int B, int64_t n_bits, const uint8_t* records_dev, int64_t record_stride, int msg_bytes,
                         int64_t n_records, int k, int32_t* idx_dev, int32_t* score_dev, void* workspace_dev, void* stream);

int gsw_embed_l(const uint8_t key[32], const uint8_t nonce16[16], const uint8_t* msg, int msg_bytes, const double* u_dev, uint64_t seed,
                uint64_t image_index0, void* out_dev, int out_dtype, int B, int64_t n_elems, uint32_t flags, int l, void* stream);
int gsw_extract_l(const void* z_dev, int z_dtype, const uint8_t key[32], const uint8_t nonce16[16], int msg_bits, uint8_t* bits_dev,
                  uint32_t* counts_dev, uint32_t* flags_dev, int B, int64_t n_elems, int l, void* stream);
int gsw_quant_pack(const void* z_dev, int z_dtype, uint8_t* packed_dev, uint32_t* flags_dev, int B, int64_t n_elems, int l, void* stream);

int gsw_tile_agree(const uint8_t* packed_dev, int B, int C, int h, int w, int l, int tile, const uint8_t* keys_dev, const uint8_t* msg_dev,
                   int msg_bits, int32_t* agree_dev, void* stream);
int gsw_vote_tiled(const uint8_t* packed_dev, int B, int C, int h, int w, int l, int tile, const uint8_t* keys_dev, const uint16_t* weights_dev,
                   int msg_bits, uint8_t* bits_dev, int32_t* score_dev, int32_t* wsum_dev, void* stream);

int gsw_embed_keyed(const uint8_t* records_dev, int64_t record_stride, int msg_bytes, const double* u_dev, uint64_t seed,
                    uint64_t image_index0, void* out_dev, int out_dtype, int B, int64_t n_elems, uint32_t flags, int l, void* stream);
int gsw_extract_keyed(const void* z_dev, int z_dtype, const uint8_t* records_dev, int64_t record_stride, int msg_bytes,
                      uint8_t* bits_dev, uint32_t* counts_dev , uint32_t* flags_dev, uint32_t* matches_dev ,
                      int B, int64_t n_elems, int l, void* stream);

int gsw_extract_soft(const void* z_dev, int z_dtype, const uint8_t* records_dev, int64_t record_stride, int msg_bytes,
                     const float* thr_dev, int64_t thr_stride , int levels,
                     uint8_t* bits_dev, int32_t* score_dev , int32_t* wsum_dev , int32_t* wsq_dev ,
                     uint32_t* flags_dev, uint32_t* matches_dev , int B, int64_t n_elems, void* stream);

int gsw_level_pack(const void* z_dev, int z_dtype, const float* thr_dev, int64_t thr_stride , int levels,
                   uint8_t* signs_dev, uint8_t* planes_dev, int32_t* wsum_dev, int32_t* wsq_dev, uint32_t* flags_dev, int B, int64_t n_elems,
                   void* stream);
int gsw_trace_keyed_soft_topk(const uint8_t* signs_dev, const uint8_t* planes_dev, const int32_t* wsum_dev, int levels, int B, int64_t n_bits,
                              const uint8_t* records_dev, int64_t record_stride, int msg_bytes, int64_t n_records, int k, int32_t* idx_dev,
                              int32_t* score_dev, void* workspace_dev, void* stream);

size_t gsw_key_search_workspace_bytes(int B, int64_t n_keys, int k);
int gsw_key_search_topk(const uint8_t* signs_dev, int B, int64_t n_bits, const uint8_t* keys_dev, int64_t key_stride, int msg_bytes, int64_t n_keys,
                        int k, int32_t* idx_dev, int32_t* stat_dev, void* workspace_dev, void* stream);

int gsw_rows_align(const uint8_t* rows_dev, int B, int C, int H, int W, int l, const int32_t* aligns_dev, int A, uint8_t* out_dev, void* stream);

size_t gsw_key_search_soft_workspace_bytes(int B, int64_t n_keys, int k);
int gsw_key_search_soft_topk(const uint8_t* signs_dev, const uint8_t* planes_dev, int P, int B, int64_t n_bits, const uint8_t* keys_dev,
                             int64_t key_stride, int msg_bytes, int64_t n_keys, int k, int32_t* idx_dev, int32_t* stat_dev, void* workspace_dev,
                             void* stream);

#if defined(__GNUC__)
#pragma GCC visibility pop
#endif

#ifdef __cplusplus
}
#endif
#endif
```

Baseline: 8.140 images/s.

## Add row-major V attention path using LDS transpose reads and fused QKV GEMM

Adds a ROWV variant of the attention kernel that reads V in row-major token layout, the same layout as Q and K. It stages V into LDS with an XOR swizzle and feeds the MFMA through ds_read_tr16_b64 transpose reads. Self-attention in the UNet can then use one fused QKV GEMM instead of a QK GEMM plus a separate transposed-V GEMM. This removes a projection launch and the transposed write of V, at the cost of new LDS addressing that must stay correct and free of bank conflicts. The path is limited to head_dim 64 and at least 256 tokens, excludes the key-split cases, and is on by default through an environment variable.

```diff
diff --git a/a-watermark-for-diffusion-models_amd/_native.py b/a-watermark-for-diffusion-models_amd/_native.py
--- a/a-watermark-for-diffusion-models_amd/_native.py
+++ b/a-watermark-for-diffusion-models_amd/_native.py
@@ -64,6 +64,8 @@
                                 C.c_int, C.c_float, C.c_int, C.c_void_p]),
     "gsw_attention_ws": (C.c_int, [C.c_void_p, C.c_void_p, C.c_void_p, C.c_void_p, C.c_int, C.c_int, C.c_int, C.c_int, C.c_int, C.c_int, C.c_int, C.c_int,
                                    C.c_int, C.c_float, C.c_int, C.c_void_p, C.c_int64, C.c_void_p]),
+    "gsw_attention_rowv_ws": (C.c_int, [C.c_void_p, C.c_void_p, C.c_void_p, C.c_void_p, C.c_int, C.c_int, C.c_int, C.c_int, C.c_int, C.c_int, C.c_int, C.c_int,
+                                        C.c_int, C.c_int, C.c_float, C.c_int, C.c_void_p, C.c_int64, C.c_void_p]),
     "gsw_xattn_fused": (C.c_int, [C.c_void_p, C.c_void_p, C.c_void_p, C.c_int64, C.c_void_p, C.c_int64, C.c_void_p, C.c_void_p, C.c_void_p, C.c_float, C.c_int, C.c_int,
                                   C.c_int, C.c_int, C.c_int, C.c_int, C.c_void_p]),
     "gsw_xattn_fused_pre": (C.c_int, [C.c_void_p, C.c_void_p, C.c_void_p, C.c_float, C.c_void_p, C.c_int64, C.c_void_p, C.c_int64, C.c_void_p, C.c_void_p, C.c_void_p,
diff --git a/a-watermark-for-diffusion-models_amd/csrc/gswm_attn.hip b/a-watermark-for-diffusion-models_amd/csrc/gswm_attn.hip
--- a/a-watermark-for-diffusion-models_amd/csrc/gswm_attn.hip
+++ b/a-watermark-for-diffusion-models_amd/csrc/gswm_attn.hip
@@ -67,11 +67,12 @@
     uint32_t total;
     uint32_t ksplit;
     float* part;
+    int32_t ldv;
 };
 
 constexpr uint32_t VP = 144;
 
-template <typename T, int QB, int DU, bool PAIR, bool RAGGED, bool KVS = false, bool DMA = false>
+template <typename T, int QB, int DU, bool PAIR, bool RAGGED, bool KVS = false, bool DMA = false, bool ROWV = false>
 __global__ __launch_bounds__(256, (DU > 10 ? 1 : 2)) void gsw_attn_fwd_kernel(AttnArgs p) {
     using v8 = typename AT<T>::v8;
     using v4 = typename AT<T>::v4;
@@ -80,13 +81,14 @@
     static_assert(TR == 0 || TR == 8 || TR == 16, "head_dim % 32 must be 0, 8 or 16");
     constexpr int DB = DBF > 0 ? DBF : 1, VROWS = DBF * 32 + (TAIL ? 16 : 0), NACC = DBF * 16 + (TAIL ? 8 : 0);
     constexpr uint32_t KP = KC * 32 + 16;
-    constexpr uint32_t STAGE = 64 * KP + VROWS * VP;
+    constexpr uint32_t STAGE = 64 * KP + (ROWV ? 64 * 128 : VROWS * VP);
     constexpr int NU = (64 * DU + 255) / 256;
     constexpr uint32_t NSTG = PAIR ? 4 : 2;
     constexpr bool LM = TR == 8 && !KVS;
     constexpr bool L4 = !LM;
     static_assert(!KVS || (QB == 1 && !RAGGED && !PAIR), "key-split form: 32 queries per wave, whole tiles, the plain two-stage loop");
     static_assert(!DMA || (DU == 8 && PAIR && !RAGGED && !KVS), "DMA staging: head_dim 64, four stages, whole tiles");
+    static_assert(!ROWV || (DU == 8 && !KVS), "row-major V: head_dim 64, not the key-split form");
     extern __shared__ __attribute__((aligned(16))) uint8_t lds[];
     const uint32_t tid = threadIdx.x, wave = tid >> 6, lane = tid & 63u, h = lane >> 5, c32 = lane & 31u;
     constexpr uint32_t QW = 32u * QB, QWG = 4u * QW;
@@ -102,7 +104,8 @@
     const uint32_t q0 = qt * QWG + wave * QW + c32;
     const T* Qb = reinterpret_cast<const T*>(p.q) + (int64_t)b * p.Sq * p.ldq + hh * (uint32_t)D;
     const T* K = reinterpret_cast<const T*>(p.k) + (int64_t)b * p.Sk * p.ldk + hh * (uint32_t)D;
-    const T* VT = reinterpret_cast<const T*>(p.vt) + ((int64_t)b * p.H + hh) * D * (int64_t)p.Sk;
+    const T* VT = ROWV ? reinterpret_cast<const T*>(p.vt) + (int64_t)b * p.Sk * p.ldv + hh * (uint32_t)D
+                       : reinterpret_cast<const T*>(p.vt) + ((int64_t)b * p.H + hh) * D * (int64_t)p.Sk;
 
     if (DU & 1 || D & 31) {
         for (uint32_t i = tid; i < NSTG * STAGE / 16; i += 256) reinterpret_cast<uint4*>(lds)[i] = make_uint4(0, 0, 0, 0);
@@ -138,8 +141,9 @@
     const uint32_t kr##i = uu##i / (uint32_t)DU, kcol##i = uu##i - kr##i * (uint32_t)DU;                \
     const T* kg##i = K + (int64_t)kr##i * p.ldk + kcol##i * 8u;                                         \
     const uint32_t kst##i = kr##i * KP + kcol##i * 16u;                                                 \
-    const T* vg##i = VT + (int64_t)(uu##i >> 3) * p.Sk + (uu##i & 7u) * 8u;                             \
-    const uint32_t vst##i = 64u * KP + (uu##i >> 3) * VP + ((uu##i & 7u) >> 1) * 32u + (uu##i & 1u) * 8u;
+    const T* vg##i = ROWV ? VT + (int64_t)kr##i * p.ldv + kcol##i * 8u : VT + (int64_t)(uu##i >> 3) * p.Sk + (uu##i & 7u) * 8u;      \
+    const uint32_t vst##i = ROWV ? 64u * KP + kr##i * 128u + ((kcol##i ^ (((kr##i >> 1) & 1u) << 2)) << 4)      \
+                                 : 64u * KP + (uu##i >> 3) * VP + ((uu##i & 7u) >> 1) * 32u + (uu##i & 1u) * 8u;
     GSW_ATTN_UNIT_DECL(0)
     GSW_ATTN_UNIT_DECL(1)
     GSW_ATTN_UNIT_DECL(2)
@@ -151,10 +155,11 @@
             const int32_t row_ = min((int32_t)(key0) + (int32_t)kr##i, p.Sk - 1);                       \
             const int32_t col_ = (int32_t)(key0) + (int32_t)(uu##i & 7u) * 8;                           \
             kreg##i = *reinterpret_cast<const uint4*>(K + (int64_t)row_ * p.ldk + kcol##i * 8u);        \
-            vreg##i = *reinterpret_cast<const uint4*>(VT + (int64_t)(uu##i >> 3) * p.Sk + (col_ + 8 <= p.Sk ? col_ : 0)); \
+            vreg##i = ROWV ? *reinterpret_cast<const uint4*>(VT + (int64_t)row_ * p.ldv + kcol##i * 8u)      \
+                           : *reinterpret_cast<const uint4*>(VT + (int64_t)(uu##i >> 3) * p.Sk + (col_ + 8 <= p.Sk ? col_ : 0)); \
         } else {                                                                                        \
             kreg##i = *reinterpret_cast<const uint4*>(kg##i + (int64_t)(key0) * p.ldk);                 \
-            vreg##i = *reinterpret_cast<const uint4*>(vg##i + (key0));                                  \
+            vreg##i = *reinterpret_cast<const uint4*>(vg##i + (ROWV ? (int64_t)(key0) * p.ldv : (int64_t)(key0)));      \
         }                                                                                               \
     }
 #define GSW_ATTN_GLOAD(key0) GSW_ATTN_GLOAD1(0, key0) GSW_ATTN_GLOAD1(1, key0) GSW_ATTN_GLOAD1(2, key0) GSW_ATTN_GLOAD1(3, key0) GSW_ATTN_GLOAD1(4, key0)
@@ -162,8 +167,11 @@
     if (NU > i && (ALLV || uv##i)) {                                                                    \
         uint8_t* base_ = lds + (st) * STAGE;                                                            \
         *reinterpret_cast<uint4*>(base_ + kst##i) = kreg##i;                                            \
+        if (ROWV) *reinterpret_cast<uint4*>(base_ + vst##i) = vreg##i;                       \
+        else {                                                                              \
         *reinterpret_cast<uint2*>(base_ + vst##i) = make_uint2(vreg##i.x, vreg##i.y);        \
         *reinterpret_cast<uint2*>(base_ + vst##i + 16u) = make_uint2(vreg##i.z, vreg##i.w);  \
+        }                                                                                   \
     }
 #define GSW_ATTN_LSTORE(st) GSW_ATTN_LSTORE1(0, st) GSW_ATTN_LSTORE1(1, st) GSW_ATTN_LSTORE1(2, st) GSW_ATTN_LSTORE1(3, st) GSW_ATTN_LSTORE1(4, st)
     static_assert(NU <= 5, "staging code covers up to 5 units per thread");
@@ -189,6 +197,12 @@
     uint32_t swo[8];
 #pragma unroll
     for (int k = 0; k < 8; ++k) swo[k] = DMA ? c32 * 128u + (((uint32_t)k ^ ((c32 >> 1) & 7u)) << 4) : 0u;
+    uint32_t vtr[DB];
+#pragma unroll
+    for (int db = 0; db < DB; ++db) {
+        const uint32_t q4 = (lane >> 2) & 3u, p4 = lane & 3u;
+        vtr[db] = ROWV ? (4u * h + q4) * 128u + (((((uint32_t)db ^ (q4 >> 1)) << 2) | (((lane >> 4) & 1u) << 1) | (p4 >> 1)) << 4) + 8u * (p4 & 1u) : 0u;
+    }
     auto tile = [&](const uint8_t* Kl, const uint8_t* Vl, int32_t t) __attribute__((always_inline)) {
 
         f32x16 s[QB][2];
@@ -274,8 +288,18 @@
             for (int tt = 0; tt < 2; ++tt) {
 #pragma unroll
                 for (int db = 0; db < DBF; ++db) {
-                    const v8 a = DMA ? *reinterpret_cast<const v8*>(Vl + (uint32_t)(db * 32 * 128) + (h ? swo[(4 * kb + 2 * tt + 1) & 7] : swo[(4 * kb + 2 * tt) & 7]))
-                                     : *reinterpret_cast<const v8*>(Vl + (uint32_t)(db * 32 + (int)c32) * VP + (uint32_t)(kb * 32 + tt * 16) * 2u + h * 16u);
+                    v8 a;
+                    if constexpr (ROWV) {
+                        typedef short s16x4 __attribute__((ext_vector_type(4)));
+                        typedef __attribute__((address_space(3))) s16x4* lds_s16x4;
+                        const uint8_t* va = Vl + (uint32_t)((2 * kb + tt) * 2048) + vtr[db];
+                        const s16x4 lo = __builtin_amdgcn_ds_read_tr16_b64_v4i16((lds_s16x4)va);
+                        const s16x4 hi = __builtin_amdgcn_ds_read_tr16_b64_v4i16((lds_s16x4)(va + 1024));
+                        a = __builtin_bit_cast(v8, __builtin_shufflevector(lo, hi, 0, 1, 2, 3, 4, 5, 6, 7));
+                    } else {
+                        a = DMA ? *reinterpret_cast<const v8*>(Vl + (uint32_t)(db * 32 * 128) + (h ? swo[(4 * kb + 2 * tt + 1) & 7] : swo[(4 * kb + 2 * tt) & 7]))
+                                : *reinterpret_cast<const v8*>(Vl + (uint32_t)(db * 32 + (int)c32) * VP + (uint32_t)(kb * 32 + tt * 16) * 2u + h * 16u);
+                    }
 #pragma unroll
                     for (int qb = 0; qb < QB; ++qb) o[qb][db] = AT<T>::mfma(a, pb[qb][kb][tt], o[qb][db]);
                 }
@@ -308,16 +332,16 @@
             const uint32_t chunk = (lane & 7u) ^ ((row >> 1) & 7u);
             const uint32_t key = 16u * (pc >> 1) + 8u * (lane >> 5) + 4u * (pc & 1u) + ((lane >> 3) & 3u);
             kp[j] = K + (int64_t)key * p.ldk + chunk * 8u;
-            vp[j] = VT + (int64_t)row * p.Sk + chunk * 8u;
+            vp[j] = ROWV ? VT + (int64_t)key * p.ldv + ((lane & 7u) ^ (((row >> 1) & 1u) << 2)) * 8u : VT + (int64_t)row * p.Sk + chunk * 8u;
         }
         const uint32_t wv = __builtin_amdgcn_readfirstlane(wave);
-        const int64_t kstep = (int64_t)64 * p.ldk;
+        const int64_t kstep = (int64_t)64 * p.ldk, vstep = ROWV ? (int64_t)64 * p.ldv : (int64_t)64;
         auto dma = [&](uint8_t* sg, int32_t t) __attribute__((always_inline)) {
 #pragma unroll
             for (int j = 0; j < 2; ++j) {
                 __builtin_amdgcn_global_load_lds((const __attribute__((address_space(1))) void*)(kp[j] + (int64_t)t * kstep),
                                                  (__attribute__((address_space(3))) void*)(sg + (wv + 4u * j) * 1024u), 16, 0, 0);
-                __builtin_amdgcn_global_load_lds((const __attribute__((address_space(1))) void*)(vp[j] + (int64_t)t * 64),
+                __builtin_amdgcn_global_load_lds((const __attribute__((address_space(1))) void*)(vp[j] + (int64_t)t * vstep),
                                                  (__attribute__((address_space(3))) void*)(sg + 8192u + (wv + 4u * j) * 1024u), 16, 0, 0);
             }
         };
@@ -516,24 +540,27 @@
 
 }
 
+static uint32_t attn_key_splits(const AttnArgs& a, bool ragged, const float* ws, int64_t ws_bytes, int nacc) {
+    static const int kvs_env = getenv("GSW_ATTN_KVS") ? atoi(getenv("GSW_ATTN_KVS")) : 1;
+    const int32_t nt = a.Sk >> 6;
+    if (ragged || !kvs_env || !ws || a.Sk_valid != a.Sk || a.total > 256u || nt < (kvs_env > 1 ? 8 : 32)) return 0;
+    uint32_t ksplit = (uint32_t)std::min<int64_t>(std::min<int64_t>(512 / a.total, nt / 4), 8);
+    if (kvs_env > 1) ksplit = (uint32_t)std::min<int>(kvs_env, nt);
+    const int64_t need = (int64_t)a.total * ksplit * 4 * (nacc + 2) * 64 * (int64_t)sizeof(float);
+    return ksplit >= 2 && need <= ws_bytes ? ksplit : 0;
+}
+
 template <typename T, int QB, int DU>
 static int launch_attn_cfg(const AttnArgs& a, uint32_t grid, bool ragged, float* ws, int64_t ws_bytes, hipStream_t st) {
     constexpr int KC = (DU + 1) / 2, DBF = DU * 8 / 32, TR = DU * 8 % 32, NACC = DBF * 16 + (TR ? 8 : 0);
     constexpr uint32_t stage = 64 * (KC * 32 + 16) + (DBF * 32 + (TR ? 16 : 0)) * VP;
     if constexpr (QB == 1 && (DU == 8 || DU == 5)) {
-        static const int kvs_env = getenv("GSW_ATTN_KVS") ? atoi(getenv("GSW_ATTN_KVS")) : 1;
-        const int32_t nt = a.Sk >> 6;
-        if (!ragged && kvs_env && ws && a.Sk_valid == a.Sk && a.total <= 256u && nt >= (kvs_env > 1 ? 8 : 32)) {
-            uint32_t ksplit = (uint32_t)std::min<int64_t>(std::min<int64_t>(512 / a.total, nt / 4), 8);
-            if (kvs_env > 1) ksplit = (uint32_t)std::min<int>(kvs_env, nt);
-            const int64_t need = (int64_t)a.total * ksplit * 4 * (NACC + 2) * 64 * (int64_t)sizeof(float);
-            if (ksplit >= 2 && need <= ws_bytes) {
-                AttnArgs k = a;
-                k.ksplit = ksplit; k.part = ws;
-                hipLaunchKernelGGL((gsw_attn_fwd_kernel<T, 1, DU, false, false, true>), dim3(a.total * ksplit), dim3(256), 2 * stage, st, k);
-                hipLaunchKernelGGL((gsw_attn_combine_kernel<T, DU>), dim3(a.total), dim3(256), 0, st, k);
-                return GSW_OK;
-            }
+        if (const uint32_t ksplit = attn_key_splits(a, ragged, ws, ws_bytes, NACC)) {
+            AttnArgs k = a;
+            k.ksplit = ksplit; k.part = ws;
+            hipLaunchKernelGGL((gsw_attn_fwd_kernel<T, 1, DU, false, false, true>), dim3(a.total * ksplit), dim3(256), 2 * stage, st, k);
+            hipLaunchKernelGGL((gsw_attn_combine_kernel<T, DU>), dim3(a.total), dim3(256), 0, st, k);
+            return GSW_OK;
         }
     }
     static const int pair_env = getenv("GSW_ATTN_PAIR") ? atoi(getenv("GSW_ATTN_PAIR")) : 1;
@@ -566,19 +593,30 @@
     return launch_attn_cfg<T, 1, 20>(a, grid, ragged, ws, wsb, st);
 }
 
-int gsw_attention(const void* q_dev, const void* k_dev, const void* vt_dev, void* out_dev, int B, int H, int head_dim, int Sq, int Sk, int Sk_valid,
-                  int ldq, int ldk, int ldo, float scale, int dtype, void* stream) {
-    return gsw_attention_ws(q_dev, k_dev, vt_dev, out_dev, B, H, head_dim, Sq, Sk, Sk_valid, ldq, ldk, ldo, scale, dtype, nullptr, 0, stream);
-}
-
-int gsw_attention_ws(const void* q_dev, const void* k_dev, const void* vt_dev, void* out_dev, int B, int H, int head_dim, int Sq, int Sk, int Sk_valid,
-                     int ldq, int ldk, int ldo, float scale, int dtype, void* workspace_dev, int64_t workspace_bytes, void* stream) {
+template <typename T>
+static int launch_attn_rowv(const AttnArgs& a, int QB, uint32_t grid, bool ragged, const float* ws, int64_t ws_bytes, hipStream_t st) {
+    constexpr uint32_t stage = 64 * 144 + 64 * 128;
+    const int32_t nt = (a.Sk + 63) >> 6;
+    if (QB == 1 && attn_key_splits(a, ragged, ws, ws_bytes, 32)) return GSW_ERR_UNSUPPORTED;
+    if (!ragged && nt >= 16) {
+        if (nt & 3) return GSW_ERR_UNSUPPORTED;
+        if (QB == 2) hipLaunchKernelGGL((gsw_attn_fwd_kernel<T, 2, 8, true, false, false, true, true>), dim3(grid), dim3(256), 0, st, a);
+        else hipLaunchKernelGGL((gsw_attn_fwd_kernel<T, 1, 8, true, false, false, true, true>), dim3(grid), dim3(256), 0, st, a);
+    } else if (ragged) hipLaunchKernelGGL((gsw_attn_fwd_kernel<T, 1, 8, false, true, false, false, true>), dim3(grid), dim3(256), 2 * stage, st, a);
+    else if (QB == 2) hipLaunchKernelGGL((gsw_attn_fwd_kernel<T, 2, 8, false, false, false, false, true>), dim3(grid), dim3(256), 2 * stage, st, a);
+    else hipLaunchKernelGGL((gsw_attn_fwd_kernel<T, 1, 8, false, false, false, false, true>), dim3(grid), dim3(256), 2 * stage, st, a);
+    return GSW_OK;
+}
+
+static int attention_launch(const void* q_dev, const void* k_dev, const void* v_dev, void* out_dev, int B, int H, int head_dim, int Sq, int Sk, int Sk_valid,
+                            int ldq, int ldk, int ldv, int ldo, float scale, int dtype, void* workspace_dev, int64_t workspace_bytes, void* stream, bool rowv) {
     if (workspace_bytes < 0 || (workspace_bytes > 0 && !workspace_dev) || ((uintptr_t)workspace_dev & 15)) return GSW_ERR_BAD_ARG;
-    if (!q_dev || !k_dev || !vt_dev || !out_dev || B <= 0 || H <= 0 || Sq <= 0 || Sk <= 0 || Sk_valid <= 0 || Sk_valid > Sk) return GSW_ERR_BAD_ARG;
+    if (!q_dev || !k_dev || !v_dev || !out_dev || B <= 0 || H <= 0 || Sq <= 0 || Sk <= 0 || Sk_valid <= 0 || Sk_valid > Sk) return GSW_ERR_BAD_ARG;
     if (dtype != GSW_F16 && dtype != GSW_BF16) return GSW_ERR_BAD_ARG;
     if (head_dim != 40 && head_dim != 64 && head_dim != 80 && head_dim != 160) return GSW_ERR_UNSUPPORTED;
     const int inner = H * head_dim;
     if ((Sk & 7) || ldq < inner || ldk < inner || ldo < inner || ((ldq | ldk | ldo) & 7)) return GSW_ERR_UNSUPPORTED;
+    if (rowv && (head_dim != 64 || ldv < inner || (ldv & 7))) return GSW_ERR_UNSUPPORTED;
     static const int qb_env = getenv("GSW_ATTN_QB") ? atoi(getenv("GSW_ATTN_QB")) : 2;
     const bool ragged = (Sq & 127) || (Sk & 63);
     const int64_t wg256 = (int64_t)(Sq / 256) * B * H;
@@ -586,19 +624,38 @@
     const int64_t total = (int64_t)((Sq + 128 * QB - 1) / (128 * QB)) * B * H;
     if (total > 0x7FFFFFFF) return GSW_ERR_UNSUPPORTED;
     AttnArgs a;
-    a.q = q_dev; a.k = k_dev; a.vt = vt_dev; a.o = out_dev;
+    a.q = q_dev; a.k = k_dev; a.vt = v_dev; a.o = out_dev;
     a.H = H; a.Sq = Sq; a.Sk = Sk; a.ldq = ldq; a.ldk = ldk; a.ldo = ldo; a.Sk_valid = Sk_valid;
     a.scale_log2 = scale * 1.4426950408889634f;
     a.nqt = (uint32_t)((Sq + 128 * QB - 1) / (128 * QB));
     a.total = (uint32_t)total;
     a.ksplit = 1; a.part = nullptr;
+    a.ldv = ldv;
     float* const ws = workspace_bytes > 0 ? (float*)workspace_dev : nullptr;
-    const int rc = dtype == GSW_F16 ? launch_attn<_Float16>(a, head_dim, QB, (uint32_t)total, ragged, ws, workspace_bytes, (hipStream_t)stream)
-                                    : launch_attn<__bf16>(a, head_dim, QB, (uint32_t)total, ragged, ws, workspace_bytes, (hipStream_t)stream);
+    int rc;
+    if (rowv) rc = dtype == GSW_F16 ? launch_attn_rowv<_Float16>(a, QB, (uint32_t)total, ragged, ws, workspace_bytes, (hipStream_t)stream)
+                                    : launch_attn_rowv<__bf16>(a, QB, (uint32_t)total, ragged, ws, workspace_bytes, (hipStream_t)stream);
+    else rc = dtype == GSW_F16 ? launch_attn<_Float16>(a, head_dim, QB, (uint32_t)total, ragged, ws, workspace_bytes, (hipStream_t)stream)
+                               : launch_attn<__bf16>(a, head_dim, QB, (uint32_t)total, ragged, ws, workspace_bytes, (hipStream_t)stream);
     if (rc != GSW_OK) return rc;
     hipError_t e = hipGetLastError();
     if (e != hipSuccess) { g_last_hip_error = (int)e; return GSW_ERR_HIP; }
     return GSW_OK;
+}
+
+int gsw_attention(const void* q_dev, const void* k_dev, const void* vt_dev, void* out_dev, int B, int H, int head_dim, int Sq, int Sk, int Sk_valid,
+                  int ldq, int ldk, int ldo, float scale, int dtype, void* stream) {
+    return attention_launch(q_dev, k_dev, vt_dev, out_dev, B, H, head_dim, Sq, Sk, Sk_valid, ldq, ldk, 0, ldo, scale, dtype, nullptr, 0, stream, false);
+}
+
+int gsw_attention_ws(const void* q_dev, const void* k_dev, const void* vt_dev, void* out_dev, int B, int H, int head_dim, int Sq, int Sk, int Sk_valid,
+                     int ldq, int ldk, int ldo, float scale, int dtype, void* workspace_dev, int64_t workspace_bytes, void* stream) {
+    return attention_launch(q_dev, k_dev, vt_dev, out_dev, B, H, head_dim, Sq, Sk, Sk_valid, ldq, ldk, 0, ldo, scale, dtype, workspace_dev, workspace_bytes, stream, false);
+}
+
+int gsw_attention_rowv_ws(const void* q_dev, const void* k_dev, const void* v_dev, void* out_dev, int B, int H, int head_dim, int Sq, int Sk, int Sk_valid,
+                          int ldq, int ldk, int ldv, int ldo, float scale, int dtype, void* workspace_dev, int64_t workspace_bytes, void* stream) {
+    return attention_launch(q_dev, k_dev, v_dev, out_dev, B, H, head_dim, Sq, Sk, Sk_valid, ldq, ldk, ldv, ldo, scale, dtype, workspace_dev, workspace_bytes, stream, true);
 }
 
 template <typename T>
diff --git a/a-watermark-for-diffusion-models_amd/graph.py b/a-watermark-for-diffusion-models_amd/graph.py
--- a/a-watermark-for-diffusion-models_amd/graph.py
+++ b/a-watermark-for-diffusion-models_amd/graph.py
@@ -30,7 +30,7 @@
     N.lib().gsw_mm_get_config(C.byref(tr), C.byref(sm))
     return (U.FUSED_KERNELS, U.USE_PF, U.UPSAMPLE_SUBPIXEL, U.CACHE_CONTEXT_KV, U.FUSED_QK, U.FUSED_QKV, U.OWN_ATTENTION, U.OWN_GEMM, U.TEMB_TABLE,
             U.CONV_OUT_DIRECT_MAX_PIXELS, U.CFG_SHARED_PREFIX, pf.FUSE_GN_STATS, pf.GN_FUSED_MAX_WGS, pf.GN_FUSED_MAX_PIXELS, pf.FOLD_LN, pf.FOLD_LN_MIN_ROWS, pf.SPLITK_MAX,
-            pf.SPLITK_BYTES, pf.SMALL_GEMM_MAX_ROWS, pf.ATTN_KEY_SPLIT, U.FOLD_FF_OUT, X.ENABLED, X.PRE_ENABLED, X.GNPROJ_ENABLED,
+            pf.SPLITK_BYTES, pf.SMALL_GEMM_MAX_ROWS, pf.ATTN_KEY_SPLIT, U.FOLD_FF_OUT, U.QKV_ROW_V, U.QKV_ROW_V_MIN_TOKENS, X.ENABLED, X.PRE_ENABLED, X.GNPROJ_ENABLED,
             tr.value, sm.value)
 
 
diff --git a/a-watermark-for-diffusion-models_amd/pf.py b/a-watermark-for-diffusion-models_amd/pf.py
--- a/a-watermark-for-diffusion-models_amd/pf.py
+++ b/a-watermark-for-diffusion-models_amd/pf.py
@@ -699,12 +699,25 @@
     return y
 
 
-def attention(q: torch.Tensor, k: torch.Tensor, vt: torch.Tensor, heads: int, scale: Optional[float] = None,
-              valid_keys: Optional[int] = None, out: Optional[torch.Tensor] = None) -> torch.Tensor:
+def _attn_key_split(B: int, heads: int, d: int, Sq: int, Sk: int, valid_keys: Optional[int]) -> bool:
+    return (ATTN_KEY_SPLIT and d in (40, 64) and Sq % 128 == 0 and Sk % 64 == 0 and Sk // 64 >= 32 and (valid_keys is None or int(valid_keys) == Sk)
+            and (Sq // 128) * B * heads <= 256)
+
+
+def attention_rowv_ok(B: int, heads: int, d: int, Sq: int, Sk: int, valid_keys: Optional[int] = None) -> bool:
+    if d != 64 or Sk % 8 or _attn_key_split(B, heads, d, Sq, Sk, valid_keys):
+        return False
+    return not (Sq % 128 == 0 and Sk % 64 == 0 and Sk // 64 >= 16 and (Sk // 64) % 4)
+
+
+def attention(q: torch.Tensor, k: torch.Tensor, vt: Optional[torch.Tensor], heads: int, scale: Optional[float] = None,
+              valid_keys: Optional[int] = None, out: Optional[torch.Tensor] = None, *, v: Optional[torch.Tensor] = None) -> torch.Tensor:
+    if (v is None) == (vt is None):
+        raise ValueError("attention: give either vt (V transposed) or v= (V row-major), not both and not neither")
     B, Sq, inner = q.shape
     Sk = k.shape[1]
     d = inner // heads
-    assert inner == heads * d and vt.shape == (B, inner, Sk) and k.shape[2] == inner
+    assert inner == heads * d and k.shape[2] == inner and (vt.shape == (B, inner, Sk) if v is None else v.shape == (B, Sk, inner))
 
     def rows(t):
         if t.stride(2) == 1 and t.stride(0) == t.shape[1] * t.stride(1) and t.stride(1) % 8 == 0 and t.data_ptr() % 16 == 0:
@@ -713,8 +726,11 @@
         return t, inner
 
     (q, ldq), (k, ldk) = rows(q), rows(k)
-    vt = vt.contiguous()
-    for t_, nm in ((k, "k"), (vt, "vt")):
+    if v is None:
+        vt = vt.contiguous()
+    else:
+        v, ldv = rows(v)
+    for t_, nm in ((k, "k"), (vt, "vt") if v is None else (v, "v")):
         if t_.dtype != q.dtype or t_.device != q.device:
             raise ValueError(f"attention: {nm} is {t_.dtype} on {t_.device}, q is {q.dtype} on {q.device}")
     if out is None:
@@ -724,13 +740,16 @@
     tm = CONV_TIMER
     with torch.cuda.device(q.device):
         e0 = tm.start() if tm is not None else None
-        ks_ok = (ATTN_KEY_SPLIT and d in (40, 64) and Sq % 128 == 0 and Sk % 64 == 0 and Sk // 64 >= 32 and (valid_keys is None or int(valid_keys) == Sk)
-                 and (Sq // 128) * B * heads <= 256)
+        ks_ok = v is None and _attn_key_split(B, heads, d, Sq, Sk, valid_keys)
         ws = _workspace(q.device) if ks_ok else None
-        N.check(N.lib().gsw_attention_ws(q.data_ptr(), k.data_ptr(), vt.data_ptr(), out.data_ptr(), B, heads, d, Sq, Sk,
-                                         Sk if valid_keys is None else int(valid_keys), ldq, ldk, inner,
-                                         float(scale if scale is not None else d ** -0.5), _dt(q.dtype), 0 if ws is None else ws.data_ptr(),
-                                         0 if ws is None else ws.numel(), _stream_ptr()))
+        sk_valid = Sk if valid_keys is None else int(valid_keys)
+        sc = float(scale if scale is not None else d ** -0.5)
+        if v is None:
+            N.check(N.lib().gsw_attention_ws(q.data_ptr(), k.data_ptr(), vt.data_ptr(), out.data_ptr(), B, heads, d, Sq, Sk, sk_valid, ldq, ldk, inner,
+                                             sc, _dt(q.dtype), 0 if ws is None else ws.data_ptr(), 0 if ws is None else ws.numel(), _stream_ptr()))
+        else:
+            N.check(N.lib().gsw_attention_rowv_ws(q.data_ptr(), k.data_ptr(), v.data_ptr(), out.data_ptr(), B, heads, d, Sq, Sk, sk_valid, ldq, ldk, ldv, inner,
+                                                  sc, _dt(q.dtype), 0, 0, _stream_ptr()))
         if tm is not None:
             tm.stop(e0, ("gsw_attn_fwd_kernel", B, Sq, Sk, heads, d) if tm.by_shape else "gsw_attn_fwd_kernel", 4.0 * B * heads * Sq * (Sk if valid_keys is None else int(valid_keys)) * d,
                     nbytes=2.0 * heads * d * (2 * out.shape[0] * Sq + 2 * B * Sk))
diff --git a/a-watermark-for-diffusion-models_amd/unet.py b/a-watermark-for-diffusion-models_amd/unet.py
--- a/a-watermark-for-diffusion-models_amd/unet.py
+++ b/a-watermark-for-diffusion-models_amd/unet.py
@@ -44,6 +44,9 @@
 FUSED_QK = True
 
 FUSED_QKV = False
+
+QKV_ROW_V = os.environ.get("GSW_QKV_ROW_V", "1") != "0"
+QKV_ROW_V_MIN_TOKENS = 256
 
 OWN_ATTENTION = True
 
@@ -212,6 +215,11 @@
         return pf.cached(self, "_gsw_ln_" + which, ws + (norm.weight, norm.bias),
                          lambda: pf.fold_ln_weights(ws[0].detach() if len(ws) == 1 else torch.cat([w.detach() for w in ws], dim=0), None, norm.weight, norm.bias))
 
+    def _row_v(self, x) -> bool:
+        b, n, _ = x.shape
+        return (QKV_ROW_V and n >= QKV_ROW_V_MIN_TOKENS and self._no_qkv_bias() and n % 8 == 0 and pf.attention_rowv_ok(b, self.heads, self.head_dim, n, n)
+                and _own_gemm_ok(x, self.to_q.in_features, 3 * self.to_q.out_features))
+
     def context_kv(self, src: torch.Tensor):
         store = getattr(src, "_gsw_kv", None)
         if store is None:
@@ -227,7 +235,10 @@
     def forward_ln(self, x, stat, norm: nn.LayerNorm, ctx=None, resid=None, project: bool = True):
         n = x.shape[1]
         inner = self.to_q.out_features
-        if ctx is None:
+        if ctx is None and self._row_v(x):
+            qkv = pf.gemm_ln(x, stat, *self._folded("qkv", norm))
+            o = pf.attention(qkv[..., :inner], qkv[..., inner:2 * inner], None, self.heads, v=qkv[..., 2 * inner:])
+        elif ctx is None:
             qk = pf.gemm_ln(x, stat, *self._folded("qk", norm))
             vt = pf.gemm_ln(x, stat, *self._folded("v", norm), mode="trans", tokens=n)
             o = pf.attention(qk[..., :inner], qk[..., inner:], vt, self.heads)
@@ -286,6 +297,11 @@
         if OWN_ATTENTION and FUSED_KERNELS:
             src, valid = (x, n) if ctx is None else _padded_ctx(ctx)
             if pf.attention_ok(x, self.heads, self.head_dim, n, src.shape[1]):
+                if ctx is None and not (FUSED_QK and FUSED_QKV) and self._row_v(x) and self._wcat("qkv").dtype == x.dtype:
+                    inner = self.to_q.out_features
+                    qkv = pf.gemm(x.contiguous(), self._wcat("qkv"), None)
+                    o = pf.attention(qkv[..., :inner], qkv[..., inner:2 * inner], None, self.heads, v=qkv[..., 2 * inner:])
+                    return _lin(o, self.to_out[0], resid)
                 q, k, vt = self._qkv(x, src, ctx is not None)
                 return _lin(pf.attention(q, k, vt, self.heads, valid_keys=valid), self.to_out[0], resid)
             if pf.half_gpu(x):
diff --git a/include/gswm.h b/include/gswm.h
--- a/include/gswm.h
+++ b/include/gswm.h
@@ -161,6 +161,9 @@
                   int Sk_valid, int ldq, int ldk, int ldo, float scale, int dtype, void* stream);
 int gsw_attention_ws(const void* q_dev, const void* k_dev, const void* vt_dev, void* out_dev, int B, int H, int head_dim, int Sq, int Sk,
                      int Sk_valid, int ldq, int ldk, int ldo, float scale, int dtype, void* workspace_dev, int64_t workspace_bytes, void* stream);
+int gsw_attention_rowv_ws(const void* q_dev, const void* k_dev, const void* v_dev, void* out_dev, int B, int H, int head_dim, int Sq, int Sk,
+                          int Sk_valid, int ldq, int ldk, int ldv, int ldo, float scale, int dtype, void* workspace_dev, int64_t workspace_bytes,
+                          void* stream);
 int gsw_xattn_fused(const void* x_dev, const float* ln_stat_dev, const void* blob_dev, int64_t blob_stride_bytes, const float* v_dev, int64_t v_stride_floats,
                     const int32_t* ctx_index_dev, void* out_dev, float* out_stat_dev, float out_eps, int x_images, int out_images, int tokens, int C, int heads,
                     int dtype, void* stream);
```

New measurement: 8.195 images/s, median of 6. About the same (+0.7%).
